# BenLangmead/bowtie2

Hardware: NVIDIA H100
Metric: Mreads/s (higher is better)
Workload: dtype u64 popcount (FM rank) + s16x2 DPX (DP)

## Files before the change

### bowtie2_b200/csrc/api.cu

```cuda
#include "bt2g_internal.h"
#include "dp_device.cuh"
#include <cstring>
#include <cstdlib>
#include <new>

template <typename OFF> void launch_rank4(const DevEbwt<OFF> &, const uint64_t *, uint64_t, uint64_t *, cudaStream_t);
template <typename OFF> void launch_maplf_range(const DevEbwt<OFF> &, const uint64_t *, const uint64_t *, const uint64_t *, uint64_t, uint64_t *, uint64_t *, uint8_t *, cudaStream_t);
template <typename OFF> void launch_maplf1(const DevEbwt<OFF> &, const uint64_t *, const uint8_t *, uint64_t, uint64_t *, cudaStream_t);
template <typename OFF> void launch_ftab(const DevEbwt<OFF> &, const uint64_t *, uint64_t, uint64_t *, cudaStream_t);
template <typename OFF> void launch_exact_sweep(const DevIndex<OFF> &, const uint8_t *, const uint64_t *, uint64_t, int, int, uint8_t *, uint64_t *, cudaStream_t, unsigned long long * = nullptr);
template <typename OFF> void launch_seed_search(const DevIndex<OFF> &, const uint8_t *, const uint64_t *, uint64_t, int, int, int, int, const int32_t *, const int32_t *, uint64_t *, int32_t *, cudaStream_t, unsigned long long * = nullptr);
template <typename OFF> void launch_seed_search2(const DevIndex<OFF> &, const uint8_t *, const uint64_t *, uint64_t, int, int, int, int, int, const int32_t *, const int32_t *, uint64_t *, int32_t *, uint64_t *, uint32_t *, unsigned long long *, int, cudaStream_t, unsigned long long *);
template <typename OFF> void launch_exact_sweep2(const DevIndex<OFF> &, const uint64_t *, uint64_t, int, int, uint8_t *, uint64_t *, const uint64_t *, const uint32_t *, unsigned long long *, int, cudaStream_t, unsigned long long *, int = 0);
void launch_pack_reads(const uint8_t *, const uint64_t *, uint64_t, int, uint64_t *, uint32_t *, cudaStream_t);
template <typename OFF> void launch_resolve(const DevIndex<OFF> &, const uint64_t *, const uint32_t *, uint64_t, int, uint64_t *, uint64_t *, uint64_t *, uint64_t *, uint8_t *, cudaStream_t, unsigned long long * = nullptr);
template <typename OFF> void launch_resolve2(const DevIndex<OFF> &, const uint64_t *, const uint32_t *, uint64_t, const uint32_t *, int, uint64_t *, uint64_t *, uint64_t *, uint64_t *, uint8_t *, unsigned long long *, int, cudaStream_t, unsigned long long *);
template <typename OFF> void launch_one_mm(const DevIndex<OFF> &, const uint8_t *, const uint8_t *, const uint64_t *, uint64_t, const int32_t *, const uint8_t *, const bt2g_scoring &, int, bt2g_mm_hit *, int32_t *, cudaStream_t);
template <typename OFF> void launch_get_stretch(const DevIndex<OFF> &, const uint64_t *, const int64_t *, const int32_t *, uint64_t, int, uint8_t *, cudaStream_t);
template <typename OFF> void launch_extend(const DevIndex<OFF> &, const uint8_t *, const uint64_t *, uint64_t, int, int, const int32_t *, const int32_t *, const uint64_t *, uint8_t *, cudaStream_t);

template <typename OFF> void launch_ungapped(const DevIndex<OFF> &, const bt2g_scoring &, const uint8_t *, const uint8_t *, const uint64_t *, const bt2g_ungapped_problem *, uint64_t, bt2g_ungapped_result *, uint8_t *, uint32_t, cudaStream_t);
template <typename OFF> void launch_build_ktab(const DevIndex<OFF> &, int, OFF *, cudaStream_t);
template <typename OFF> void launch_build_dense_sa(const DevIndex<OFF> &, int, OFF *, cudaStream_t);
void launch_frame_mate(const bt2g_pe_policy &, const bt2g_mate_anchor *, uint64_t, bt2g_mate_frame *, cudaStream_t);
// ... 489 lines not shown
	BT2G_CUDA_TRY(ctx, cudaStreamSynchronize(ctx->stream));
	return 0;
}

int bt2g_pe_classify(bt2g_ctx *ctx, const bt2g_pe_policy *pol, const int64_t *pairs, uint64_t n, int32_t *out) {
	if(!ctx) return -1;
	if(!pol || !pairs || !out || pol->pol < 1 || pol->pol > 4) { ctx->err = "bt2g_pe_classify: bad argument"; return -1; }
	if(n == 0) return 0;
	BT2G_CUDA_TRY(ctx, cudaSetDevice(ctx->device));
	DBuf dp, dout;
	BT2G_CUDA_TRY(ctx, dp.alloc(n * 48)); BT2G_CUDA_TRY(ctx, dout.alloc(n * 4));
	BT2G_CUDA_TRY(ctx, cudaMemcpyAsync(dp.p, pairs, n * 48, cudaMemcpyHostToDevice, ctx->stream));
	launch_pe_classify(*pol, dp.as<int64_t>(), n, dout.as<int32_t>(), ctx->stream);
	BT2G_CUDA_TRY(ctx, cudaGetLastError());
	BT2G_CUDA_TRY(ctx, cudaMemcpyAsync(out, dout.p, n * 4, cudaMemcpyDeviceToHost, ctx->stream));
	BT2G_CUDA_TRY(ctx, cudaStreamSynchronize(ctx->stream));
	return 0;
}

int bt2g_extend_exact(bt2g_ctx *ctx, const bt2g_reads *reads, const bt2g_seed_plan *plan, const uint64_t *ranges, uint8_t *out) {
	REQUIRE_LOADED(ctx);
	if(!reads || !plan || !ranges || !out || plan->max_seeds <= 0 || plan->seed_len <= 0) return -1;
	uint64_t n = reads->n_reads;
	if(n == 0) return 0;
	DBuf dseq, dqual, doff, dint, doffs, drng, dout;
	int rc = uploadReads(ctx, reads, dseq, dqual, doff, false);
	if(rc) return rc;
	const uint64_t nr = n * 2ull * plan->max_seeds;
	BT2G_CUDA_TRY(ctx, dint.alloc(n * 4)); BT2G_CUDA_TRY(ctx, doffs.alloc(n * 4));
	BT2G_CUDA_TRY(ctx, drng.alloc(nr * 32)); BT2G_CUDA_TRY(ctx, dout.alloc(nr * 2));
	BT2G_CUDA_TRY(ctx, cudaMemcpyAsync(dint.p, plan->interval, n * 4, cudaMemcpyHostToDevice, ctx->stream));
	BT2G_CUDA_TRY(ctx, cudaMemcpyAsync(doffs.p, plan->offset, n * 4, cudaMemcpyHostToDevice, ctx->stream));
	BT2G_CUDA_TRY(ctx, cudaMemcpyAsync(drng.p, ranges, nr * 32, cudaMemcpyHostToDevice, ctx->stream));
	DISPATCH(ctx, launch_extend<uint32_t>(bt2g_dev_index<uint32_t>(ctx), dseq.as<uint8_t>(), doff.as<uint64_t>(), n, plan->seed_len, plan->max_seeds, dint.as<int32_t>(), doffs.as<int32_t>(), drng.as<uint64_t>(), dout.as<uint8_t>(), ctx->stream),
	              launch_extend<uint64_t>(bt2g_dev_index<uint64_t>(ctx), dseq.as<uint8_t>(), doff.as<uint64_t>(), n, plan->seed_len, plan->max_seeds, dint.as<int32_t>(), doffs.as<int32_t>(), drng.as<uint64_t>(), dout.as<uint8_t>(), ctx->stream));
	BT2G_CUDA_TRY(ctx, cudaGetLastError());
	BT2G_CUDA_TRY(ctx, cudaMemcpyAsync(out, dout.p, nr * 2, cudaMemcpyDeviceToHost, ctx->stream));
	BT2G_CUDA_TRY(ctx, cudaStreamSynchronize(ctx->stream));
	return 0;
}

int bt2g_resolve(bt2g_ctx *ctx, const uint64_t *rows, const uint32_t *hitlen, uint64_t n, int rejectStraddle,
                 uint64_t *joined, uint64_t *tidx, uint64_t *textoff, uint64_t *tlen, uint8_t *flags) {
	REQUIRE_LOADED(ctx);
	if(!rows) return -1;
	if(n == 0) return 0;
	DBuf dr, dh, dj, dti, dto, dtl, dfl;
	BT2G_CUDA_TRY(ctx, dr.alloc(n * 8));
	BT2G_CUDA_TRY(ctx, cudaMemcpyAsync(dr.p, rows, n * 8, cudaMemcpyHostToDevice, ctx->stream));
	if(hitlen) { BT2G_CUDA_TRY(ctx, dh.alloc(n * 4)); BT2G_CUDA_TRY(ctx, cudaMemcpyAsync(dh.p, hitlen, n * 4, cudaMemcpyHostToDevice, ctx->stream)); }
	if(joined) BT2G_CUDA_TRY(ctx, dj.alloc(n * 8));
	if(tidx) BT2G_CUDA_TRY(ctx, dti.alloc(n * 8));
	if(textoff) BT2G_CUDA_TRY(ctx, dto.alloc(n * 8));
	if(tlen) BT2G_CUDA_TRY(ctx, dtl.alloc(n * 8));
	if(flags) BT2G_CUDA_TRY(ctx, dfl.alloc(n));
	DBuf dnext;
	BT2G_CUDA_TRY(ctx, dnext.alloc(8));
	int sms = 148; cudaDeviceGetAttribute(&sms, cudaDevAttrMultiProcessorCount, ctx->device);
	DISPATCH(ctx, launch_resolve2<uint32_t>(bt2g_dev_index<uint32_t>(ctx), dr.as<uint64_t>(), dh.as<uint32_t>(), n, nullptr, rejectStraddle, dj.as<uint64_t>(), dti.as<uint64_t>(), dto.as<uint64_t>(), dtl.as<uint64_t>(), dfl.as<uint8_t>(), dnext.as<unsigned long long>(), sms, ctx->stream, nullptr),
	              launch_resolve2<uint64_t>(bt2g_dev_index<uint64_t>(ctx), dr.as<uint64_t>(), dh.as<uint32_t>(), n, nullptr, rejectStraddle, dj.as<uint64_t>(), dti.as<uint64_t>(), dto.as<uint64_t>(), dtl.as<uint64_t>(), dfl.as<uint8_t>(), dnext.as<unsigned long long>(), sms, ctx->stream, nullptr));
	BT2G_CUDA_TRY(ctx, cudaGetLastError());
	if(joined) BT2G_CUDA_TRY(ctx, cudaMemcpyAsync(joined, dj.p, n * 8, cudaMemcpyDeviceToHost, ctx->stream));
	if(tidx) BT2G_CUDA_TRY(ctx, cudaMemcpyAsync(tidx, dti.p, n * 8, cudaMemcpyDeviceToHost, ctx->stream));
	if(textoff) BT2G_CUDA_TRY(ctx, cudaMemcpyAsync(textoff, dto.p, n * 8, cudaMemcpyDeviceToHost, ctx->stream));
	if(tlen) BT2G_CUDA_TRY(ctx, cudaMemcpyAsync(tlen, dtl.p, n * 8, cudaMemcpyDeviceToHost, ctx->stream));
	if(flags) BT2G_CUDA_TRY(ctx, cudaMemcpyAsync(flags, dfl.p, n, cudaMemcpyDeviceToHost, ctx->stream));
	BT2G_CUDA_TRY(ctx, cudaStreamSynchronize(ctx->stream));
	return 0;
}

int bt2g_get_stretch(bt2g_ctx *ctx, const uint64_t *tidx, const int64_t *off, const int32_t *count, uint64_t n,
                     int32_t stride, uint8_t *out) {
	REQUIRE_LOADED(ctx);
	if(!ctx->info.has_ref) { ctx->err = "packed reference (.3/.4) not loaded"; return -1; }
	if(n == 0) return 0;
	DBuf dt, dof, dc, dout;
	BT2G_CUDA_TRY(ctx, dt.alloc(n * 8)); BT2G_CUDA_TRY(ctx, dof.alloc(n * 8)); BT2G_CUDA_TRY(ctx, dc.alloc(n * 4));
	BT2G_CUDA_TRY(ctx, dout.alloc(n * (uint64_t)stride));
	BT2G_CUDA_TRY(ctx, cudaMemcpyAsync(dt.p, tidx, n * 8, cudaMemcpyHostToDevice, ctx->stream));
	BT2G_CUDA_TRY(ctx, cudaMemcpyAsync(dof.p, off, n * 8, cudaMemcpyHostToDevice, ctx->stream));
	BT2G_CUDA_TRY(ctx, cudaMemcpyAsync(dc.p, count, n * 4, cudaMemcpyHostToDevice, ctx->stream));
	BT2G_CUDA_TRY(ctx, cudaMemsetAsync(dout.p, 4, n * (uint64_t)stride, ctx->stream));
	DISPATCH(ctx, launch_get_stretch<uint32_t>(bt2g_dev_index<uint32_t>(ctx), dt.as<uint64_t>(), dof.as<int64_t>(), dc.as<int32_t>(), n, stride, dout.as<uint8_t>(), ctx->stream),
	              launch_get_stretch<uint64_t>(bt2g_dev_index<uint64_t>(ctx), dt.as<uint64_t>(), dof.as<int64_t>(), dc.as<int32_t>(), n, stride, dout.as<uint8_t>(), ctx->stream));
	BT2G_CUDA_TRY(ctx, cudaGetLastError());
	BT2G_CUDA_TRY(ctx, cudaMemcpyAsync(out, dout.p, n * (uint64_t)stride, cudaMemcpyDeviceToHost, ctx->stream));
	BT2G_CUDA_TRY(ctx, cudaStreamSynchronize(ctx->stream));
	return 0;
}

}

template <typename OFF> int launch_dp_e2e(const DevIndex<OFF> &, const bt2g_scoring &, const DpLaunch &, int, cudaStream_t);
template <typename OFF> int launch_dp_local(const DevIndex<OFF> &, const bt2g_scoring &, const DpLaunch &, int, cudaStream_t);

extern "C" {

void bt2g_scoring_default(bt2g_scoring *sc, int local) {
	memset(sc, 0, sizeof(*sc));
	sc->match_bonus = local ? 2 : 0;
	sc->rdgap_const = 5; sc->rdgap_linear = 3; sc->rfgap_const = 5; sc->rfgap_linear = 3;
	sc->gapbar = 4;
	sc->local = local ? 1 : 0;
	for(int q = 0; q < 64; q++) {
		int ii = q < 40 ? q : 40;
		float frac = (float)ii / 40.0f;
		sc->mmpen[q] = (uint8_t)(2 + (int)(frac * (6 - 2)));
		sc->npen[q] = 1;
	}
	sc->nceil_const = 0.0; sc->nceil_linear = (double)0.15f;
}

int bt2g_set_scoring(bt2g_ctx *ctx, const bt2g_scoring *sc) {
	if(!ctx || !sc) return -1;
	if(sc->gapbar < 1) { ctx->err = "gapbar must be >= 1"; return -1; }
	ctx->scoring = *sc;
	return 0;
}

int bt2g_set_extend_mode(bt2g_ctx *ctx, int through_text) {
	if(!ctx) return -1;
	ctx->extendText = through_text ? 1 : 0;
	return 0;
}

int bt2g_set_dp_mode(bt2g_ctx *ctx, int cap) {
	if(!ctx || cap < 0 || cap > 3) return -1;
	ctx->dpModeCap = cap;
	return 0;
}

int bt2g_dp_extend(bt2g_ctx *ctx, const bt2g_reads *reads, const bt2g_dp_problem *probs, uint64_t n,
                   int32_t maxCands, int32_t maxAlns, int32_t maxOps,
                   bt2g_dp_summary *summ, bt2g_dp_cand *cands, bt2g_dp_aln *alns, uint8_t *ops) {
	REQUIRE_LOADED(ctx);
	if(!ctx->info.has_ref) { ctx->err = "packed reference (.3/.4) not loaded"; return -1; }
	if(!reads || !reads->qual || !probs || !summ || !cands || !alns || !ops) { ctx->err = "null argument"; return -1; }
	if(ctx->scoring.gapbar < 1) bt2g_scoring_default(&ctx->scoring, 0);
	if(n == 0) return 0;
	if(maxCands < 1 || maxAlns < 1 || maxOps < 1) return -1;
	int maxCol = 1, maxLen = 1;
	int64_t minMinsc = 0;
	for(uint64_t i = 0; i < n; i++) {
		if(probs[i].minsc < minMinsc) minMinsc = probs[i].minsc;
		int64_t nc = probs[i].refr - probs[i].refl + 1;
		if(nc > maxCol) maxCol = (int)nc;
		if(probs[i].read_idx >= reads->n_reads) { ctx->err = "read_idx out of range"; return -1; }
		int len = (int)(reads->off[probs[i].read_idx + 1] - reads->off[probs[i].read_idx]);
		if(len > maxLen) maxLen = len;
	}
	if(maxLen > 512) { ctx->err = "reads longer than 512 are not supported by the DP kernel"; return -1; }
	maxCol += 1;
	if(maxCol > 8192) { ctx->err = "DP window wider than 8192 columns"; return -1; }
	DBuf dseq, dqual, doff, dprob, dcodes, dlast, dsumm, dcand, daln, dops, draw;
	int rc = uploadReads(ctx, reads, dseq, dqual, doff, true);
	if(rc) return rc;
	DpLaunch L;
	L.n = n; L.nDev = nullptr; L.maxCol = maxCol;
	{
		int sms = 148; cudaDeviceGetAttribute(&sms, cudaDevAttrMultiProcessorCount, ctx->device);
		uint64_t want = (uint64_t)sms * 24;
		L.numSlots = ((n < want ? n : want) + 3) / 4 * 4;
	} L.maxCands = maxCands; L.maxAlns = maxAlns; L.maxOps = maxOps;
	L.packed = ctx->scoring.local ? 0 : dp_kernel_mode(ctx->scoring, minMinsc, maxLen, ctx->dpModeCap);
	L.codeStride = dp_code_stride(maxCol, maxLen, L.packed);
	BT2G_CUDA_TRY(ctx, dprob.alloc(n * sizeof(bt2g_dp_problem)));
	if(L.packed == 3) {
		L.chunk = dp_chunk_problems(L.codeStride, n);
		BT2G_CUDA_TRY(ctx, dcodes.alloc(L.chunk * L.codeStride));
	} else {
		BT2G_CUDA_TRY(ctx, dcodes.alloc(L.numSlots * L.codeStride * (L.packed ? 2 : 1)));
	}
	BT2G_CUDA_TRY(ctx, dlast.alloc(L.numSlots * (uint64_t)maxCol * 4));
	L.maxRaw = maxCands * 4 < 1024 ? 1024 : maxCands * 4;
	BT2G_CUDA_TRY(ctx, draw.alloc(L.numSlots * (uint64_t)L.maxRaw * 8));
	L.rawKeys = draw.as<uint64_t>();
	BT2G_CUDA_TRY(ctx, dsumm.alloc(n * sizeof(bt2g_dp_summary)));
	BT2G_CUDA_TRY(ctx, dcand.alloc(n * (uint64_t)maxCands * sizeof(bt2g_dp_cand)));
	BT2G_CUDA_TRY(ctx, daln.alloc(n * (uint64_t)maxAlns * sizeof(bt2g_dp_aln)));
	BT2G_CUDA_TRY(ctx, dops.alloc(n * (uint64_t)maxAlns * maxOps));
	BT2G_CUDA_TRY(ctx, cudaMemcpyAsync(dprob.p, probs, n * sizeof(bt2g_dp_problem), cudaMemcpyHostToDevice, ctx->stream));
	BT2G_CUDA_TRY(ctx, cudaMemsetAsync(dcand.p, 0, dcand.bytes, ctx->stream));
	BT2G_CUDA_TRY(ctx, cudaMemsetAsync(daln.p, 0, daln.bytes, ctx->stream));
	L.seq = dseq.as<uint8_t>(); L.qual = dqual.as<uint8_t>(); L.roff = doff.as<uint64_t>();
	L.probs = dprob.as<bt2g_dp_problem>(); L.codes = dcodes.as<uint8_t>(); L.lastH = dlast.as<int32_t>();
	L.summ = dsumm.as<bt2g_dp_summary>(); L.cands = dcand.as<bt2g_dp_cand>(); L.alns = daln.as<bt2g_dp_aln>(); L.ops = dops.as<uint8_t>();
	int lrc;
	if(ctx->scoring.local) {
		if(ctx->info.off_size == 4) lrc = launch_dp_local<uint32_t>(bt2g_dev_index<uint32_t>(ctx), ctx->scoring, L, maxLen, ctx->stream);
		else lrc = launch_dp_local<uint64_t>(bt2g_dev_index<uint64_t>(ctx), ctx->scoring, L, maxLen, ctx->stream);
	} else {
		if(ctx->info.off_size == 4) lrc = launch_dp_e2e<uint32_t>(bt2g_dev_index<uint32_t>(ctx), ctx->scoring, L, maxLen, ctx->stream);
		else lrc = launch_dp_e2e<uint64_t>(bt2g_dev_index<uint64_t>(ctx), ctx->scoring, L, maxLen, ctx->stream);
	}
	if(lrc) { ctx->err = "DP launch rejected"; return -1; }
	BT2G_CUDA_TRY(ctx, cudaGetLastError());
	BT2G_CUDA_TRY(ctx, cudaMemcpyAsync(summ, dsumm.p, dsumm.bytes, cudaMemcpyDeviceToHost, ctx->stream));
	BT2G_CUDA_TRY(ctx, cudaMemcpyAsync(cands, dcand.p, dcand.bytes, cudaMemcpyDeviceToHost, ctx->stream));
	BT2G_CUDA_TRY(ctx, cudaMemcpyAsync(alns, daln.p, daln.bytes, cudaMemcpyDeviceToHost, ctx->stream));
	BT2G_CUDA_TRY(ctx, cudaMemcpyAsync(ops, dops.p, dops.bytes, cudaMemcpyDeviceToHost, ctx->stream));
	BT2G_CUDA_TRY(ctx, cudaStreamSynchronize(ctx->stream));
	return 0;
}

}
```

### bowtie2_b200/csrc/dp_device.cuh

```cuda
#pragma once
#include "bt2g_internal.h"
#include <cstdlib>

static inline bool dp_packed_ok(const bt2g_scoring &sc, int64_t minMinsc, int maxLen) {
	return !sc.local && minMinsc >= -8000 && (int64_t)sc.match_bonus * maxLen <= 8000 && sc.match_bonus >= 0;
}

static inline int dp_kernel_mode(const bt2g_scoring &sc, int64_t minMinsc, int maxLen, int cap = 3) {
	if(cap < 0 || cap > 3) cap = 3;
	if(cap == 0 || !dp_packed_ok(sc, minMinsc, maxLen)) return 0;
	const int64_t range = (int64_t)sc.match_bonus * maxLen - (minMinsc - sc.match_bonus - 1);
	return (cap >= 2 && range <= 127) ? (cap >= 3 ? 3 : 2) : 1;
}

static inline int dp_rows_per_lane(int maxLen, int mode) {
	if(mode >= 2) {
		const int rs[7] = {4, 5, 6, 8, 10, 12, 16};
		for(int i = 0; i < 7; i++) if(32 * rs[i] >= maxLen) return rs[i];
		return 0;
	}
	return maxLen <= 128 ? 4 : (maxLen <= 256 ? 8 : (maxLen <= 512 ? 16 : 0));
}
#define DP_BLOCK_RPL 2
static inline uint64_t dp_code_stride(int maxCol, int maxLen, int mode) {
	int R = dp_rows_per_lane(maxLen, mode);
	if(mode == 3) R = (R + DP_BLOCK_RPL - 1) / DP_BLOCK_RPL * DP_BLOCK_RPL;
	const uint64_t steps = (uint64_t)maxCol + (mode == 3 ? 36 : 32);
	return ((steps * 32 * (uint64_t)R) + 255) & ~(uint64_t)255;
}

static inline uint64_t dp_chunk_problems(uint64_t codeStride, uint64_t nMax, uint64_t budget = 6ull << 30) {
	if(const char *e = getenv("BT2G_DP_CHUNK_MB")) { uint64_t v = strtoull(e, nullptr, 10); if(v) budget = v << 20; }
	uint64_t c = budget / (codeStride ? codeStride : 1);
	if(c < 1024) c = 1024;
	if(c > nMax) c = nMax;
	return c ? c : 1;
}

struct DpLaunch {
	const uint8_t  *seq, *qual;
	const uint64_t *roff;
	const bt2g_dp_problem *probs;
	uint64_t        n;
	const uint32_t *nDev;
	uint64_t        numSlots;
	uint8_t        *codes;
	int32_t        *lastH;
	uint64_t       *rawKeys;
	int             maxRaw;
	uint64_t        codeStride;
	int             maxCol;
	int             maxCands, maxAlns, maxOps;
	uint64_t        chunk = 0;
	int             packed = 0;
	cudaEvent_t    *tev = nullptr;
	int             tevCap = 0;
	int            *tevN = nullptr;
	uint32_t        zeroP = 0;
	bt2g_dp_summary *summ;
	bt2g_dp_cand    *cands;
	bt2g_dp_aln     *alns;
	uint8_t         *ops;
};
```

### bowtie2_b200/csrc/dp_kernels.cu

```cuda
#include "fm_device.cuh"
#include "dp_device.cuh"

#define DP_NEG (-(1 << 28))
#define DP_BIG (1 << 20)

__host__ __device__ __forceinline__ size_t dp_smem_per_warp(int maxCol) { return ((size_t)maxCol * 7 + 16 + 15) & ~(size_t)15; }

__device__ __forceinline__ int dp_max(int a, int b) { return a > b ? a : b; }

template <int R>
__device__ __forceinline__ void dp_backtrace_all(const DpLaunch &L, const bt2g_scoring &sc, const bt2g_dp_problem &p, uint64_t w,
                                                 const uint8_t *rs, const uint8_t *rq, int rdlen, const uint8_t *refw,
                                                 uint8_t *codes, bt2g_dp_cand *cands, int ncand, bt2g_dp_summary *summ,
                                                 int lane, bool local) {
	const int rdgapo = sc.rdgap_const + sc.rdgap_linear, rdgape = sc.rdgap_linear;
	const int rfgapo = sc.rfgap_const + sc.rfgap_linear, rfgape = sc.rfgap_linear;
	int SQ = rdlen >> 4; if(SQ == 0) SQ = 1;
	bt2g_dp_aln *alns = L.alns + w * (uint64_t)L.maxAlns;
	uint8_t *ops = L.ops + w * (uint64_t)L.maxAlns * L.maxOps;
	int naln = 0, flags = 0;
	auto cell = [&](int rr, int cc) -> uint8_t * { int k = rr / R; return codes + ((size_t)(cc + k) * 32 + k) * R + (rr - k * R); };
	for(int ci = 0; ci < ncand; ci++) {
		int row = cands[ci].row, col = cands[ci].col;
		const int startRow = row;
// ... 475 lines not shown
	const int rdgapo = sc.rdgap_const + sc.rdgap_linear, rdgape = sc.rdgap_linear;
	const int rfgapo = sc.rfgap_const + sc.rfgap_linear, rfgape = sc.rfgap_linear;
	const int bonus = sc.match_bonus;
	const uint32_t FLOORP = dpx_both(DPX_FLOOR), ONEP = 0x00010001u;
	const uint32_t bonusP = dpx_both(bonus), nrdeP = dpx_both(-rdgape);

	for(uint64_t pw = slot; pw < nPairs; pw += nSlots) {
		uint64_t w[2] = {2 * pw, 2 * pw + 1};
		bool live[2] = {true, w[1] < nProb};
		if(!live[1]) w[1] = w[0];
		bt2g_dp_problem p[2] = {L.probs[w[0]], L.probs[w[1]]};
		const uint8_t *rs[2], *rq[2]; int rdlen[2], ncol[2], floorv[2];
		__syncwarp();
#pragma unroll
		for(int x = 0; x < 2; x++) {
			rs[x] = L.seq + L.roff[p[x].read_idx]; rq[x] = L.qual + L.roff[p[x].read_idx];
			rdlen[x] = (int)(L.roff[p[x].read_idx + 1] - L.roff[p[x].read_idx]);
			ncol[x] = (int)(p[x].refr - p[x].refl + 1);
			floorv[x] = p[x].minsc - bonus - 1;
			if(ncol[x] <= 0 || ncol[x] > L.maxCol || rdlen[x] > 32 * R || rdlen[x] <= 0 ||
			   (int64_t)bonus * rdlen[x] - floorv[x] > 127 || floorv[x] < -DPX_LIMIT) {
				if(live[x] && lane == 0) {
					bt2g_dp_summary *sm = L.summ + w[x];
					sm->found = 0; sm->best = DP_NEG; sm->ncand = 0; sm->naln = 0; sm->flags = BT2G_DP_FLAG_BADSHAPE;
				}
				live[x] = false;
			}
		}
		if(!live[0] && !live[1]) continue;
		if(!live[0]) { p[0] = p[1]; rs[0] = rs[1]; rq[0] = rq[1]; rdlen[0] = rdlen[1]; ncol[0] = ncol[1]; floorv[0] = floorv[1]; w[0] = w[1]; }
		if(!live[1]) { p[1] = p[0]; rs[1] = rs[0]; rq[1] = rq[0]; rdlen[1] = rdlen[0]; ncol[1] = ncol[0]; floorv[1] = floorv[0]; w[1] = w[0]; }
		const int ncolMax = ncol[0] > ncol[1] ? ncol[0] : ncol[1];
#pragma unroll
		for(int x = 0; x < 2; x++) {
			ref_window<OFF>(ix, p[x].tidx, p[x].refl, ncol[x], refw[x], lane);
			for(int k = ncol[x] + lane; k < ncolMax; k += 32) refw[x][k] = 4;
		}
		__syncwarp();

		uint32_t rcP[R], mmpP[R], npnP[R], nrfoP[R], nrfeP[R], nrdoP[R];
#pragma unroll
		for(int r = 0; r < R; r++) {
			int v[2][6];
#pragma unroll
			for(int x = 0; x < 2; x++) {
				const int i = lane * R + r;
				bool bar = true;
				int c = 5, mm = 0, np = 0;
				if(i < rdlen[x]) {
					const int pos = p[x].fw ? i : rdlen[x] - 1 - i;
					c = rs[x][pos];
					c = p[x].fw ? c : (c > 3 ? 4 : 3 - c);
					int q = (int)rq[x][pos] - 33;
					q = q < 0 ? 0 : (q > 63 ? 63 : q);
					np = -(int)sc.npen[q];
					mm = c > 3 ? np : -(int)sc.mmpen[q];
					if(c > 3) c = 5;
					bar = (i < sc.gapbar) || (rdlen[x] - 1 - i < sc.gapbar);
				}
				v[x][0] = c; v[x][1] = mm; v[x][2] = np;
				v[x][3] = bar ? -DPX_BIG : -rfgapo; v[x][4] = bar ? -DPX_BIG : -rfgape; v[x][5] = bar ? -DPX_BIG : -rdgapo;
			}
			rcP[r] = dpx_pack(v[0][0], v[1][0]); mmpP[r] = dpx_pack(v[0][1], v[1][1]); npnP[r] = dpx_pack(v[0][2], v[1][2]);
			nrfoP[r] = dpx_pack(v[0][3], v[1][3]); nrfeP[r] = dpx_pack(v[0][4], v[1][4]); nrdoP[r] = dpx_pack(v[0][5], v[1][5]);
		}
		const int lastLane0 = (rdlen[0] - 1) / R, lastLane1 = (rdlen[1] - 1) / R;
		const int lastLaneMax = lastLane0 > lastLane1 ? lastLane0 : lastLane1;
		const uint32_t nfloorP = dpx_pack(-floorv[0], -floorv[1]);

		uint32_t Hleft[R], Earr[R];
#pragma unroll
		for(int r = 0; r < R; r++) { Hleft[r] = FLOORP; Earr[r] = FLOORP; }
		uint32_t botH = FLOORP, botF = FLOORP, prevInH = FLOORP;
		const int nsteps = ncolMax + lastLaneMax;
		const size_t P4 = (size_t)(L.maxCol + 32) * 128, P1 = (size_t)(L.maxCol + 32) * 32;
		uint8_t *w4A[R / 4 + 1], *w4B[R / 4 + 1], *w1A[R % 4 + 1], *w1B[R % 4 + 1];
#pragma unroll
		for(int g = 0; g < R / 4; g++) { w4A[g] = hb[0] + g * P4 + (size_t)lane * 4; w4B[g] = hb[1] + g * P4 + (size_t)lane * 4; }
#pragma unroll
		for(int g = 0; g < R % 4; g++) { w1A[g] = hb[0] + (R / 4) * P4 + g * P1 + lane; w1B[g] = hb[1] + (R / 4) * P4 + g * P1 + lane; }
		for(int t = 0; t < nsteps; t++) {
			uint32_t inH = __shfl_up_sync(0xffffffffu, botH, 1);
			uint32_t inF = __shfl_up_sync(0xffffffffu, botF, 1);
			if(lane == 0) { inH = FLOORP; inF = FLOORP; }
			const int j = t - lane;
			if(j >= 0 && j < ncolMax && lane <= lastLaneMax) {
				const uint32_t refcP = (uint32_t)refw[0][j] | ((uint32_t)refw[1][j] << 16);
				const uint32_t refNm = ((refcP >> 2) & ONEP) * 0xffffu;
				uint32_t diag = (lane == 0) ? 0u : prevInH;
				uint32_t upH = inH, upF = inF;
				uint32_t hs[DP_RP(R)];
#pragma unroll
				for(int r = R; r < DP_RP(R); r++) hs[r] = 0u;
#pragma unroll
				for(int r = 0; r < R; r++) {
					const uint32_t F = __viaddmax_s16x2(upF, nrfeP[r], __viaddmax_s16x2(upH, nrfoP[r], FLOORP));
					const uint32_t pen = dpx_sel(refNm, npnP[r], mmpP[r]);
					const uint32_t mmask = dpx_ne01(rcP[r], refcP) * 0xffffu;
					const uint32_t Hd = __viaddmax_s16x2(diag, dpx_sel(mmask, pen, bonusP), FLOORP);
					const uint32_t E = Earr[r];
					const uint32_t H = __vimax3_s16x2(Hd, E, F);
					Earr[r] = __viaddmax_s16x2(E, nrdeP, __viaddmax_s16x2(H, nrdoP[r], FLOORP));
					hs[r] = __viaddmax_s16x2(H, nfloorP, 0u);
					diag = Hleft[r]; Hleft[r] = H;
					upH = H; upF = F;
				}
				botH = upH; botF = upF;
				prevInH = inH;
#pragma unroll
				for(int q4 = 0; q4 < R / 4; q4++) {
					const uint32_t t01 = __byte_perm(hs[4 * q4], hs[4 * q4 + 1], 0x6240), t23 = __byte_perm(hs[4 * q4 + 2], hs[4 * q4 + 3], 0x6240);
					*reinterpret_cast<uint32_t *>(w4A[q4]) = __byte_perm(t01, t23, 0x5410);
					*reinterpret_cast<uint32_t *>(w4B[q4]) = __byte_perm(t01, t23, 0x7632);
				}
#pragma unroll
				for(int g = 0; g < R % 4; g++) {
					*w1A[g] = (uint8_t)(hs[(R / 4) * 4 + g] & 0xffu);
					*w1B[g] = (uint8_t)((hs[(R / 4) * 4 + g] >> 16) & 0xffu);
				}
			} else if(j >= ncolMax) {
				botH = FLOORP; botF = FLOORP;
			}
#pragma unroll
			for(int g = 0; g < R / 4; g++) { w4A[g] += 128; w4B[g] += 128; }
#pragma unroll
			for(int g = 0; g < R % 4; g++) { w1A[g] += 32; w1B[g] += 32; }
		}
		__syncwarp();
#pragma unroll
		for(int x = 0; x < 2; x++) {
			if(!live[x]) continue;
			const int lr = rdlen[x] - 1, kk = lr / R;
			for(int j = lane; j < ncol[x]; j += 32)
				lastH[x][j] = (int)hb[x][hb_index<R>(L.maxCol + 32, lr, j)] + floorv[x];
			dp_e2e_tail<R, true>(L, sc, p[x], w[x], rs[x], rq[x], rdlen[x], ncol[x], lastH[x], candCol[x], refw[x], hb[x], L.summ + w[x], lane,
			                     DpHbPlanes<R>{hb[x], L.maxCol + 32});
		}
	}
}

#define DP_BLK_ROWS (32 * DP_BLOCK_RPL)
#define DP_BLK_HEAD 64
#define DP_BLK_MAX (DP_BLK_HEAD / 4)
static_assert(16 * 32 <= DP_BLK_MAX * DP_BLK_ROWS, "the range table must cover reads of 32 x 16 rows");

#define DP_FILL_PAD 64
__host__ __device__ __forceinline__ size_t dp_fill_smem_per_warp(int maxCol, bool offdom) {
	const size_t win = ((size_t)maxCol + 15) & ~(size_t)15;
	return 2 * (win + 2 * DP_FILL_PAD) + DP_QPROF_BYTES(DP_BLOCK_RPL) + win * (offdom ? 4 : 8);
}

template <bool B> struct DpBool { static constexpr bool value = B; };

template <typename OFF, int R, bool OFFDOM>
__global__ void __launch_bounds__(128, 8) k_dp_fill_h(DevIndex<OFF> ix, bt2g_scoring sc, DpLaunch L, uint64_t chunkStart, uint64_t chunkMax) {
	constexpr int RPL = DP_BLOCK_RPL;
	static_assert(RPL == 1 || RPL == 2, "stores are one byte or one u16 per lane and problem");
	extern __shared__ uint8_t smem[];
	const int warpInBlock = threadIdx.x >> 5, lane = threadIdx.x & 31;
	const uint64_t slot = blockIdx.x * (uint64_t)(blockDim.x >> 5) + warpInBlock;
	const uint64_t nSlots = (uint64_t)gridDim.x * (blockDim.x >> 5);
	const uint64_t nAll = L.nDev ? (uint64_t)*L.nDev : L.n;
	if(chunkStart >= nAll) return;
	const uint64_t nProb = (nAll - chunkStart < chunkMax) ? nAll - chunkStart : chunkMax;
	const uint64_t nPairs = (nProb + 1) >> 1;
	const size_t win = ((size_t)L.maxCol + 15) & ~(size_t)15;
	uint8_t *sm0 = smem + (size_t)warpInBlock * dp_fill_smem_per_warp(L.maxCol, OFFDOM);
	uint8_t *refw[2] = {sm0 + DP_FILL_PAD, sm0 + win + 3 * DP_FILL_PAD}; uint8_t *hb[2];
	for(int k = lane; k < 2 * ((int)win + 2 * DP_FILL_PAD); k += 32) sm0[k] = 4;
	uint32_t *qprof = reinterpret_cast<uint32_t *>(sm0 + 2 * (win + 2 * DP_FILL_PAD));
	uint32_t *bnd = reinterpret_cast<uint32_t *>(sm0 + 2 * (win + 2 * DP_FILL_PAD) + DP_QPROF_BYTES(RPL));
	const int rdgapo = sc.rdgap_const + sc.rdgap_linear, rdgape = sc.rdgap_linear;
	const int rfgapo = sc.rfgap_const + sc.rfgap_linear, rfgape = sc.rfgap_linear;
	const int bonus = sc.match_bonus;
	const uint32_t FLOORP = OFFDOM ? L.zeroP : dpx_both(DPX_FLOOR);
	const uint32_t nrdeP = dpx_both(-rdgape);

	for(uint64_t pw = slot; pw < nPairs; pw += nSlots) {
		uint64_t w[2] = {2 * pw, 2 * pw + 1};
		bool live[2] = {true, w[1] < nProb};
		if(!live[1]) w[1] = w[0];
		bt2g_dp_problem p[2] = {L.probs[chunkStart + w[0]], L.probs[chunkStart + w[1]]};
		hb[0] = L.codes + w[0] * L.codeStride; hb[1] = L.codes + w[1] * L.codeStride;
		uint64_t ro[2]; int rdlen[2], ncol[2], floorv[2];
		__syncwarp();
#pragma unroll
		for(int x = 0; x < 2; x++) {
			ro[x] = L.roff[p[x].read_idx];
			rdlen[x] = (int)(L.roff[p[x].read_idx + 1] - L.roff[p[x].read_idx]);
			ncol[x] = (int)(p[x].refr - p[x].refl + 1);
			floorv[x] = p[x].minsc - bonus - 1;
			if(ncol[x] <= 0 || ncol[x] > L.maxCol || rdlen[x] > 32 * R || rdlen[x] <= 0 ||
			   (int64_t)bonus * rdlen[x] - floorv[x] > 127 || floorv[x] < -DPX_LIMIT) {
				if(live[x] && lane == 0) {
					bt2g_dp_summary *sm = L.summ + chunkStart + w[x];
					sm->found = 0; sm->best = DP_NEG; sm->ncand = 0; sm->naln = 0; sm->flags = BT2G_DP_FLAG_BADSHAPE;
				}
				live[x] = false;
			}
		}
		if(!live[0] && !live[1]) continue;
		if(!live[0]) { p[0] = p[1]; ro[0] = ro[1]; rdlen[0] = rdlen[1]; ncol[0] = ncol[1]; floorv[0] = floorv[1]; }
		if(!live[1]) { p[1] = p[0]; ro[1] = ro[0]; rdlen[1] = rdlen[0]; ncol[1] = ncol[0]; floorv[1] = floorv[0]; }
		const int ncolMax = ncol[0] > ncol[1] ? ncol[0] : ncol[1];
#pragma unroll
		for(int x = 0; x < 2; x++) {
			ref_window<OFF>(ix, p[x].tidx, p[x].refl, ncol[x], refw[x], lane);
			for(int k = ncol[x] + lane; k < ncolMax; k += 32) refw[x][k] = 4;
		}
		__syncwarp();
		const int rdMax = rdlen[0] > rdlen[1] ? rdlen[0] : rdlen[1];
		const int nblk = (rdMax + DP_BLK_ROWS - 1) / DP_BLK_ROWS;
		const uint32_t nfloorP = dpx_pack(-floorv[0], -floorv[1]);
		uint32_t off = DP_BLK_HEAD;
		int plo = 0, phi = -1;

		for(int b = 0; b < nblk; b++) {
			int lo = 0, bLast = -1, nst = 0;
			if(OFFDOM && b > 0) {
				int first = -1;
				for(int c0 = plo; c0 <= phi; c0 += 32) {
					const int c = c0 + lane;
					const uint32_t m = __ballot_sync(0xffffffffu, c <= phi && bnd[c] != 0u);
					if(m) { if(first < 0) first = c0 + __ffs(m) - 1; bLast = c0 + 31 - __clz(m); }
				}
				lo = first < 0 ? 0 : first;
			}
			if(!OFFDOM || b == 0 || bLast >= 0) {
				uint32_t nrfoP[RPL], nrfeP[RPL], nrdoP[RPL];
#pragma unroll
				for(int r = 0; r < RPL; r++) {
					int v[2][3];
#pragma unroll
					for(int x = 0; x < 2; x++) {
						const int i = b * DP_BLK_ROWS + lane * RPL + r;
						bool bar = true;
						int c = 5, mm = -DPX_BIG, np = -DPX_BIG;
						if(i < rdlen[x]) {
							const int pos = p[x].fw ? i : rdlen[x] - 1 - i;
							c = L.seq[ro[x] + pos];
							c = p[x].fw ? c : (c > 3 ? 4 : 3 - c);
							int q = (int)L.qual[ro[x] + pos] - 33;
							q = q < 0 ? 0 : (q > 63 ? 63 : q);
							np = -(int)sc.npen[q];
							mm = c > 3 ? np : -(int)sc.mmpen[q];
							if(c > 3) c = 5;
							bar = (i < sc.gapbar) || (rdlen[x] - 1 - i < sc.gapbar);
						}
#pragma unroll
						for(int rf = 0; rf < 5; rf++) {
							const uint32_t pv = (uint32_t)(uint16_t)(int16_t)(rf > 3 ? np : (c == rf ? bonus : mm));
							uint32_t &q = qprof[(rf * RPL + r) * 32 + lane];
							q = x == 0 ? pv : (q | (pv << 16));
						}
						v[x][0] = bar ? -DPX_BIG : -rfgapo; v[x][1] = bar ? -DPX_BIG : -rfgape; v[x][2] = bar ? -DPX_BIG : -rdgapo;
					}
					nrfoP[r] = dpx_pack(v[0][0], v[1][0]); nrfeP[r] = dpx_pack(v[0][1], v[1][1]); nrdoP[r] = dpx_pack(v[0][2], v[1][2]);
				}
				int lastLane = (rdMax - 1 - b * DP_BLK_ROWS) / RPL;
				if(lastLane > 31) lastLane = 31;
				const bool keepBottom = b + 1 < nblk;

				const int nsteps = ncolMax - lo + lastLane;
				const int lim = lane <= lastLane ? ncolMax - lo : 0;
				auto sweep = [&](auto top) -> int {
					constexpr bool TOP = decltype(top)::value;
					constexpr int SG = 4;
					uint32_t Hleft[RPL], Earr[RPL];
#pragma unroll
					for(int r = 0; r < RPL; r++) { Hleft[r] = FLOORP; Earr[r] = FLOORP; }
					uint32_t botH = FLOORP, botF = FLOORP, prevInH = FLOORP;
					uint8_t *dA = hb[0] + off + lane * RPL, *dB = hb[1] + off + lane * RPL;
					for(int t0 = 0; t0 < nsteps; t0 += SG, dA += SG * 32 * RPL, dB += SG * 32 * RPL) {
#pragma unroll
						for(int u = 0; u < SG; u++) {
							const int t = t0 + u;
							uint32_t inH = __shfl_up_sync(0xffffffffu, botH, 1);
							uint32_t inF = __shfl_up_sync(0xffffffffu, botF, 1);
							if(TOP) {
								if(lane == 0) { inH = FLOORP; inF = FLOORP; }
							} else {
								uint32_t bh = FLOORP, bf = FLOORP;
								if(lo + t <= phi) {
									if(OFFDOM) { const uint32_t e = bnd[lo + t]; bh = __byte_perm(e, 0u, 0x4140); bf = __byte_perm(e, 0u, 0x4342); }
									else { const uint2 e = reinterpret_cast<const uint2 *>(bnd)[lo + t]; bh = e.x; bf = e.y; }
								}
								if(lane == 0) { inH = bh; inF = bf; }
							}
							const bool on = (unsigned)(t - lane) < (unsigned)lim;
							if(OFFDOM || on) {
								const int j = lo + t - lane;
								const uint32_t *qa = qprof + (int)refw[0][j] * (RPL * 32) + lane, *qb = qprof + (int)refw[1][j] * (RPL * 32) + lane;
								uint32_t diag = (TOP && lane == 0) ? (OFFDOM ? nfloorP : 0u) : prevInH;
								uint32_t upH = inH, upF = inF;
								uint32_t hs[RPL];
#pragma unroll
								for(int r = 0; r < RPL; r++) {
									const uint32_t F = __viaddmax_s16x2(upF, nrfeP[r], __viaddmax_s16x2(upH, nrfoP[r], FLOORP));
									const uint32_t sP = (qa[r * 32] & 0x0000ffffu) | (qb[r * 32] & 0xffff0000u);
									const uint32_t Hd = __viaddmax_s16x2(diag, sP, FLOORP);
									const uint32_t E = Earr[r];
									const uint32_t H = __vimax3_s16x2(Hd, E, F);
									Earr[r] = __viaddmax_s16x2(E, nrdeP, __viaddmax_s16x2(H, nrdoP[r], FLOORP));
									hs[r] = OFFDOM ? H : __viaddmax_s16x2(H, nfloorP, 0u);
									diag = Hleft[r]; Hleft[r] = H;
									upH = H; upF = F;
								}
								botH = upH; botF = upF;
								prevInH = inH;
								if(OFFDOM || on) {
									if(RPL == 2) {
										const uint32_t w2 = __byte_perm(hs[0], hs[RPL - 1], 0x6240);
										*reinterpret_cast<uint16_t *>(dA + u * 32 * RPL) = (uint16_t)w2;
										*reinterpret_cast<uint16_t *>(dB + u * 32 * RPL) = (uint16_t)(w2 >> 16);
									} else {
										dA[u * 32 * RPL] = (uint8_t)hs[0]; dB[u * 32 * RPL] = (uint8_t)(hs[0] >> 16);
									}
									if(keepBottom && lane == 31 && on) {
										if(OFFDOM) bnd[j] = __byte_perm(botH, botF, 0x6420);
										else reinterpret_cast<uint2 *>(bnd)[j] = make_uint2(botH, botF);
									}
								}
							} else {
								botH = FLOORP; botF = FLOORP;
							}
						}
						if(!TOP && OFFDOM && lo + t0 + SG - 1 >= bLast) {
							uint32_t s = botH | botF | prevInH;
#pragma unroll
							for(int r = 0; r < RPL; r++) s |= Hleft[r] | Earr[r];
							if(!__any_sync(0xffffffffu, t0 + SG - 1 - lane < lim && s != 0u)) return t0 + SG < nsteps ? t0 + SG : nsteps;
						}
					}
					return nsteps;
				};
				nst = b == 0 ? sweep(DpBool<true>()) : sweep(DpBool<false>());
			}
			if(lane == 0) {
				reinterpret_cast<uint32_t *>(hb[0])[b] = (uint32_t)lo | ((uint32_t)nst << 16);
				reinterpret_cast<uint32_t *>(hb[1])[b] = (uint32_t)lo | ((uint32_t)nst << 16);
			}
			off += (uint32_t)nst * 32 * RPL;
			plo = lo; phi = lo + nst - 32;
			if(phi > ncolMax - 1) phi = ncolMax - 1;
			__syncwarp();
		}
	}
}

struct DpHbBlocks {
	uint8_t *hb; const uint2 *tab;
	__device__ __forceinline__ uint8_t *operator()(int rr, int cc) const {
		const int k = (rr % DP_BLK_ROWS) / DP_BLOCK_RPL;
		const uint2 e = tab[rr / DP_BLK_ROWS];
		const int st = cc - (int)(e.x & 0xffffu) + k;
		return (st >= k && st < (int)(e.x >> 16)) ? hb + e.y + ((size_t)st * 32 + k) * DP_BLOCK_RPL + rr % DP_BLOCK_RPL : nullptr;
	}
};

#define DP_TAIL_SMEM_PER_WARP(maxCol, R) (dp_smem_per_warp(maxCol) + DP_PROF_BYTES(R) + DP_BLK_MAX * sizeof(uint2))

template <typename OFF, int R>
__global__ void __launch_bounds__(256) k_dp_tail_h(DevIndex<OFF> ix, bt2g_scoring sc, DpLaunch L, uint64_t chunkStart, uint64_t chunkMax) {
	extern __shared__ uint8_t smem[];
	const int warpInBlock = threadIdx.x >> 5, lane = threadIdx.x & 31;
	const uint64_t nAll = L.nDev ? (uint64_t)*L.nDev : L.n;
	if(chunkStart >= nAll) return;
	const uint64_t nProb = (nAll - chunkStart < chunkMax) ? nAll - chunkStart : chunkMax;
	const size_t perWarp = DP_TAIL_SMEM_PER_WARP(L.maxCol, R);
	int32_t *lastH = reinterpret_cast<int32_t *>(smem + (size_t)warpInBlock * perWarp);
	uint16_t *candCol = reinterpret_cast<uint16_t *>(lastH + L.maxCol);
	uint8_t *refw = reinterpret_cast<uint8_t *>(candCol + L.maxCol);
	uint8_t *prof = smem + (size_t)warpInBlock * perWarp + dp_smem_per_warp(L.maxCol);
	uint2 *tab = reinterpret_cast<uint2 *>(prof + DP_PROF_BYTES(R));
	const int bonus = sc.match_bonus;
	const uint64_t nWarps = (uint64_t)gridDim.x * (blockDim.x >> 5);
	for(uint64_t wl = blockIdx.x * (uint64_t)(blockDim.x >> 5) + warpInBlock; wl < nProb; wl += nWarps) {
		const uint64_t w = chunkStart + wl;
		const bt2g_dp_problem p = L.probs[w];
		const uint8_t *rs = L.seq + L.roff[p.read_idx], *rq = L.qual + L.roff[p.read_idx];
		const int rdlen = (int)(L.roff[p.read_idx + 1] - L.roff[p.read_idx]);
		const int ncol = (int)(p.refr - p.refl + 1);
		const int floorv = p.minsc - bonus - 1;
		__syncwarp();
		if(ncol <= 0 || ncol > L.maxCol || rdlen > 32 * R || rdlen <= 0 || (int64_t)bonus * rdlen - floorv > 127 || floorv < -DPX_LIMIT) continue;
		uint8_t *hb = L.codes + wl * L.codeStride;
		const int nblk = (rdlen + DP_BLK_ROWS - 1) / DP_BLK_ROWS;
		const uint32_t e = lane < nblk ? reinterpret_cast<const uint32_t *>(hb)[lane] : 0u;
		const uint32_t bytes = (e >> 16) * (32 * DP_BLOCK_RPL);
		uint32_t incl = bytes;
#pragma unroll
		for(int o = 1; o < 32; o <<= 1) { const uint32_t v = __shfl_up_sync(0xffffffffu, incl, o); if(lane >= o) incl += v; }
		if(lane < nblk) tab[lane] = make_uint2(e, DP_BLK_HEAD + incl - bytes);
		ref_window<OFF>(ix, p.tidx, p.refl, ncol, refw, lane);
		for(int i = lane; i < rdlen; i += 32) {
			const int pos = p.fw ? i : rdlen - 1 - i;
			int c = rs[pos]; c = p.fw ? c : (c > 3 ? 4 : 3 - c);
			int q = (int)rq[pos] - 33; q = q < 0 ? 0 : (q > 63 ? 63 : q);
			prof[i] = (uint8_t)c; prof[rdlen + i] = sc.mmpen[q]; prof[2 * rdlen + i] = sc.npen[q];
		}
		__syncwarp();
		const DpHbBlocks cell{hb, tab};
		const int lr = rdlen - 1;
		for(int j = lane; j < ncol; j += 32) { const uint8_t *c = cell(lr, j); lastH[j] = (c ? (int)*c : 0) + floorv; }
		dp_e2e_tail<R, true>(L, sc, p, w, rs, rq, rdlen, ncol, lastH, candCol, refw, hb, L.summ + w, lane, cell, prof);
	}
}

template <typename Acc>
__device__ __forceinline__ void dp_backtrace_h(const DpLaunch &L, const bt2g_scoring &sc, const bt2g_dp_problem &p, uint64_t w,
                                               const uint8_t *rs, const uint8_t *rq, int rdlen, const uint8_t *refw,
                                               const Acc &cell, bt2g_dp_cand *cands, int ncand, bt2g_dp_summary *summ, int lane,
                                               const uint8_t *prof) {
	const int rdgapo = sc.rdgap_const + sc.rdgap_linear, rdgape = sc.rdgap_linear;
	const int rfgapo = sc.rfgap_const + sc.rfgap_linear, rfgape = sc.rfgap_linear;
	const int bonus = sc.match_bonus, gapbar = sc.gapbar;
	const int vmax = bonus * rdlen - (p.minsc - bonus - 1);
	bt2g_dp_aln *alns = L.alns + w * (uint64_t)L.maxAlns;
	uint8_t *ops = L.ops + w * (uint64_t)L.maxAlns * L.maxOps;
	int naln = 0, flags = 0;
	bool screened = false;
	auto cellv = [&](int rr, int cc) -> int { const uint8_t *c = cell(rr, cc); return c ? (int)*c : 0; };
	auto rdchar = [&](int rr) -> int { const int pos = p.fw ? rr : rdlen - 1 - rr; int c = rs[pos]; return p.fw ? c : (c > 3 ? 4 : 3 - c); };
	auto rdqual = [&](int rr) -> int { const int pos = p.fw ? rr : rdlen - 1 - rr; int q = (int)rq[pos] - 33; return q < 0 ? 0 : (q > 63 ? 63 : q); };
	auto inCore = [&](int dlo, int dhi) -> bool { return dhi >= p.corel && dlo <= p.corer; };
	for(int ci = 0; ci < ncand; ci++) {
		int row = cands[ci].row, col = cands[ci].col;
		const int startRow = row, origCol = col;
		uint8_t *o = ops + (size_t)naln * L.maxOps;
		const bool room = naln < L.maxAlns;
		int nops = 0, ns = 0, gaps = 0;
		bool fail = false, core = false, done = false, first = true, filtStart = false;
		while(!done && !fail) {
			const int wd = (ci > 0 && first) ? 8 : 32;
			const int rk = row - lane, ck = col - lane;
			const bool in = lane < wd && rk >= 0 && ck >= 0;
			uint8_t *cp = in ? cell(rk, ck) : nullptr;
			const int mine = in ? (cp ? (int)*cp : 0) : 0x80;
			const int v = mine & 0x7f;
			const int vn = __shfl_down_sync(0xffffffffu, v, 1);
			int sck = 0, refc = 4; bool isN = false, isMatch = false;
			if(in) {
				refc = refw[ck];
				if(prof) {
					const int c = prof[rk];
					isN = c > 3 || refc > 3;
					isMatch = !isN && c == refc;
					sck = isN ? -(int)prof[2 * rdlen + rk] : (isMatch ? bonus : -(int)prof[rdlen + rk]);
				} else {
					const int c = rdchar(rk), q = rdqual(rk);
					isN = c > 3 || refc > 3;
					isMatch = !isN && c == refc;
					sck = isN ? -(int)sc.npen[q] : (isMatch ? bonus : -(int)sc.mmpen[q]);
				}
			}
			const bool cont = lane < wd - 1 && !(mine & 0x80) && rk > 0 && ck > 0 && vn > 0 && v == vn + sck;
			const int run = __ffs(~__ballot_sync(0xffffffffu, cont)) - 1;
			if(run > 0) {
				first = false;
				const int diagi = col - row + p.triml;
				if(inCore(diagi, diagi)) core = true;
				if(lane < run) {
					const uint8_t op = (uint8_t)((isMatch ? BT2G_OP_MATCH : BT2G_OP_MM) | (refc << 2));
					if(room && nops + lane < L.maxOps) o[nops + lane] = op;
					if(cp) *cp = (uint8_t)(mine | 0x80);
				}
				ns += __popc(__ballot_sync(0xffffffffu, lane < run && isN));
				nops += run; row -= run; col -= run;
			}
			const int endBits = __shfl_sync(0xffffffffu, mine, run);
			if(run == wd - 1 && !(endBits & 0x80) && row > 0 && col > 0) { __syncwarp(); continue; }
			if(endBits & 0x80) {
				if(first) filtStart = true;
				fail = true; break;
			}
			first = false;
			if(lane == run && cp) *cp = (uint8_t)(mine | 0x80);
			{
				const int diagi = col - row + p.triml;
				if(inCore(diagi, diagi)) core = true;
			}
			if(row == 0) { done = true; break; }
			const int cur = endBits & 0x7f;
			__syncwarp();
			int klen = 0, gapKind = 0;
			if(row >= gapbar && rdlen - 1 - row >= gapbar) {
				for(int k0 = 0; k0 < row; k0 += 32) {
					if(vmax - rfgapo - k0 * rfgape < cur) break;
					const int k = k0 + lane + 1, r2 = row - k;
					bool ok = false;
					if(r2 >= 0 && row - k + 1 >= gapbar && vmax - rfgapo - (k - 1) * rfgape >= cur) {
						const int u = cellv(r2, col) & 0x7f;
						ok = u > 0 && u - rfgapo - (k - 1) * rfgape == cur;
					}
					const uint32_t mk = __ballot_sync(0xffffffffu, ok);
					if(mk) { klen = k0 + __ffs(mk); gapKind = 1; break; }
				}
				if(gapKind == 0) {
					for(int k0 = 0; k0 < col; k0 += 32) {
						if(vmax - rdgapo - k0 * rdgape < cur) break;
						const int k = k0 + lane + 1, c2 = col - k;
						bool ok = false;
						if(c2 >= 0 && vmax - rdgapo - (k - 1) * rdgape >= cur) {
							const int u = cellv(row, c2) & 0x7f;
							ok = u > 0 && u - rdgapo - (k - 1) * rdgape == cur;
						}
						const uint32_t mk = __ballot_sync(0xffffffffu, ok);
						if(mk) { klen = k0 + __ffs(mk); gapKind = 2; break; }
					}
				}
			}
			if(gapKind == 0) { fail = true; break; }
			for(int m0 = 1; m0 < klen && !fail; m0 += 32) {
				const int mth = m0 + lane;
				uint8_t *q2 = nullptr; int b = 0;
				if(mth < klen) { q2 = gapKind == 1 ? cell(row - mth, col) : cell(row, col - mth); b = q2 ? *q2 : 0; }
				const uint32_t vm = __ballot_sync(0xffffffffu, (b & 0x80) != 0);
				const int lim = vm ? __ffs(vm) - 1 : 32;
				if(q2 && lane < lim) *q2 = (uint8_t)(b | 0x80);
				if(vm) fail = true;
			}
			if(fail) break;
			{
				const int d0 = col - row + p.triml, ni = klen - 1;
				if(ni > 0 && (gapKind == 1 ? inCore(d0 + 1, d0 + ni) : inCore(d0 - ni, d0 - 1))) core = true;
			}
			if(room) {
				for(int k = lane; k < klen; k += 32) {
					const int idx = nops + k;
					if(idx < L.maxOps) o[idx] = gapKind == 1 ? (uint8_t)BT2G_OP_REFGAP : (uint8_t)(BT2G_OP_READGAP | (refw[col - k] << 2));
				}
			}
			nops += klen; gaps += klen;
			if(gapKind == 1) row -= klen; else col -= klen;
			__syncwarp();
		}
		if(filtStart) { if(lane == 0) cands[ci].fate = BT2G_CAND_FILT_START; continue; }
		if(!fail) {
			const int c = rdchar(row), refc = refw[col];
			const bool isN = c > 3 || refc > 3;
			ns += isN;
			const uint8_t op = (uint8_t)(((!isN && c == refc) ? BT2G_OP_MATCH : BT2G_OP_MM) | (refc << 2));
			if(!core) fail = true;
			else if(ns > p.nceil) fail = true;
			else {
				if(room && lane == 0 && nops < L.maxOps) o[nops] = op;
				nops++;
			}
		}
		const bool opOverflow = nops > L.maxOps;
		if(fail) { if(lane == 0) cands[ci].fate = BT2G_CAND_FAILED; continue; }
		if(lane == 0) cands[ci].fate = BT2G_CAND_SUCCEEDED;
		if(room) {
			int refns = 0;
			for(int k = col + lane; k <= origCol; k += 32) refns += refw[k] > 3;
			refns = __reduce_add_sync(0xffffffffu, refns);
			if(lane == 0) {
				bt2g_dp_aln &a = alns[naln];
				a.cand_idx = ci; a.score = cands[ci].score; a.ns = ns; a.gaps = gaps; a.col0 = col; a.row0 = row;
				a.trim_beg = 0; a.trim_end = rdlen - 1 - startRow; a.nops = nops;
				a.refns = refns;
			}
			if(opOverflow) flags |= BT2G_DP_FLAG_OPS_OVERFLOW;
		} else {
			flags |= BT2G_DP_FLAG_ALN_OVERFLOW;
		}
		naln++;
		if(naln == 1 && !screened && ci + 1 < ncand) {
			screened = true;
			bool needSeq = false;
			for(int base = ci + 1; base < ncand; base += 32) {
				const int cj = base + lane;
				int verdict = 0;
				if(cj < ncand) {
					int r2 = cands[cj].row, c2 = cands[cj].col;
					int b = cellv(r2, c2);
					if(b & 0x80) verdict = 1;
					else {
						for(int guard = 0; guard < 4 * rdlen + 8; guard++) {
							const int curv = b & 0x7f;
							if(r2 == 0) { verdict = 2; break; }
							if(c2 > 0) {
								const int pb = cellv(r2 - 1, c2 - 1), pv = pb & 0x7f;
								const int rf = refw[c2];
								int c, mm, np;
								if(prof) { c = prof[r2]; mm = prof[rdlen + r2]; np = prof[2 * rdlen + r2]; }
								else { c = rdchar(r2); const int q = rdqual(r2); mm = sc.mmpen[q]; np = sc.npen[q]; }
								const int sc2 = (c > 3 || rf > 3) ? -np : (c == rf ? bonus : -mm);
								if(pv > 0 && curv == pv + sc2) {
									if(pb & 0x80) break;
									r2--; c2--; b = pb;
									continue;
								}
							}
							if(r2 < gapbar || rdlen - 1 - r2 < gapbar) break;
							bool moved = false, dead = false, marked = false;
							for(int k = 1; k <= r2 && r2 - k + 1 >= gapbar && vmax - rfgapo - (k - 1) * rfgape >= curv; k++) {
								const int ub = cellv(r2 - k, c2), u = ub & 0x7f;
								if(u > 0 && u - rfgapo - (k - 1) * rfgape == curv) {
									if(marked || (ub & 0x80)) dead = true; else { r2 -= k; b = ub; moved = true; }
									break;
								}
								marked = marked || (ub & 0x80);
							}
							if(!moved && !dead) {
								marked = false;
								for(int k = 1; k <= c2 && vmax - rdgapo - (k - 1) * rdgape >= curv; k++) {
									const int ub = cellv(r2, c2 - k), u = ub & 0x7f;
									if(u > 0 && u - rdgapo - (k - 1) * rdgape == curv) {
										if(marked || (ub & 0x80)) dead = true; else { c2 -= k; b = ub; moved = true; }
										break;
									}
									marked = marked || (ub & 0x80);
								}
							}
							if(!moved) break;
						}
					}
				}
				if(__any_sync(0xffffffffu, verdict == 2)) { needSeq = true; break; }
				if(cj < ncand) cands[cj].fate = verdict == 1 ? BT2G_CAND_FILT_START : BT2G_CAND_FAILED;
			}
			__syncwarp();
			if(!needSeq) break;
		}
	}
	if(lane == 0) { summ->naln = naln; summ->flags |= flags; }
}

template <typename K>
static unsigned dp_resident_grid(K kernel, int threads, size_t smem, uint64_t numSlots, int warpsPerBlock) {
	int dev = 0, sms = 148, nb = 1;
	cudaGetDevice(&dev);
	cudaDeviceGetAttribute(&sms, cudaDevAttrMultiProcessorCount, dev);
	if(cudaOccupancyMaxActiveBlocksPerMultiprocessor(&nb, kernel, threads, smem) != cudaSuccess || nb < 1) nb = 1;
	uint64_t g = (uint64_t)nb * sms, cap = numSlots / warpsPerBlock;
	return (unsigned)(g < cap ? g : cap);
}

template <typename OFF, int R>
static void launch_dp_e2e_r(const DevIndex<OFF> &ix, const bt2g_scoring &sc, const DpLaunch &L, cudaStream_t st) {
	const int warpsPerBlock = 4;
	if(L.packed == 3) {
		int dev = 0, sms = 148; cudaGetDevice(&dev); cudaDeviceGetAttribute(&sms, cudaDevAttrMultiProcessorCount, dev);
		const size_t smF = (size_t)warpsPerBlock * dp_fill_smem_per_warp(L.maxCol, sc.match_bonus == 0);
		const size_t smT = (size_t)8 * DP_TAIL_SMEM_PER_WARP(L.maxCol, R);
		auto kfill = sc.match_bonus == 0 ? k_dp_fill_h<OFF, R, true> : k_dp_fill_h<OFF, R, false>;
		if(smF > 48 * 1024) cudaFuncSetAttribute(kfill, cudaFuncAttributeMaxDynamicSharedMemorySize, (int)smF);
		if(smT > 48 * 1024) cudaFuncSetAttribute(k_dp_tail_h<OFF, R>, cudaFuncAttributeMaxDynamicSharedMemorySize, (int)smT);
		int nbF = 1, nbT = 1;
		if(cudaOccupancyMaxActiveBlocksPerMultiprocessor(&nbF, kfill, warpsPerBlock * 32, smF) != cudaSuccess || nbF < 1) nbF = 1;
		if(cudaOccupancyMaxActiveBlocksPerMultiprocessor(&nbT, k_dp_tail_h<OFF, R>, 256, smT) != cudaSuccess || nbT < 1) nbT = 1;
		auto mark = [&]() { if(L.tev && L.tevN && *L.tevN < L.tevCap) cudaEventRecord(L.tev[(*L.tevN)++], st); };
		mark();
		for(uint64_t c0 = 0; c0 < L.n; c0 += L.chunk) {
			kfill<<<(unsigned)(nbF * sms), warpsPerBlock * 32, smF, st>>>(ix, sc, L, c0, L.chunk);
			mark();
			k_dp_tail_h<OFF, R><<<(unsigned)(nbT * sms), 256, smT, st>>>(ix, sc, L, c0, L.chunk);
			mark();
		}
	} else if(L.packed == 2) {
		const size_t smem = (size_t)warpsPerBlock * 2 * dp_smem_per_warp(L.maxCol);
		if(smem > 48 * 1024) cudaFuncSetAttribute(k_dp_e2e_h<OFF, R>, cudaFuncAttributeMaxDynamicSharedMemorySize, (int)smem);
		const unsigned grid = dp_resident_grid(k_dp_e2e_h<OFF, R>, warpsPerBlock * 32, smem, L.numSlots, warpsPerBlock);
		k_dp_e2e_h<OFF, R><<<grid, warpsPerBlock * 32, smem, st>>>(ix, sc, L);
	} else if(L.packed) {
		const size_t smem = (size_t)warpsPerBlock * 2 * dp_smem_per_warp(L.maxCol);
		if(smem > 48 * 1024) cudaFuncSetAttribute(k_dp_e2e_x2<OFF, R>, cudaFuncAttributeMaxDynamicSharedMemorySize, (int)smem);
		const unsigned grid = dp_resident_grid(k_dp_e2e_x2<OFF, R>, warpsPerBlock * 32, smem, L.numSlots, warpsPerBlock);
		k_dp_e2e_x2<OFF, R><<<grid, warpsPerBlock * 32, smem, st>>>(ix, sc, L);
	} else {
		const size_t smem = (size_t)warpsPerBlock * dp_smem_per_warp(L.maxCol);
		if(smem > 48 * 1024) cudaFuncSetAttribute(k_dp_e2e<OFF, R>, cudaFuncAttributeMaxDynamicSharedMemorySize, (int)smem);
		const unsigned grid = dp_resident_grid(k_dp_e2e<OFF, R>, warpsPerBlock * 32, smem, L.numSlots, warpsPerBlock);
		k_dp_e2e<OFF, R><<<grid, warpsPerBlock * 32, smem, st>>>(ix, sc, L);
	}
}

template <typename OFF>
int launch_dp_e2e(const DevIndex<OFF> &ix, const bt2g_scoring &sc, const DpLaunch &L, int maxRdLen, cudaStream_t st) {
	if(L.n == 0) return 0;
	switch(dp_rows_per_lane(maxRdLen, L.packed)) {
		case 4: launch_dp_e2e_r<OFF, 4>(ix, sc, L, st); break;
		case 5: launch_dp_e2e_r<OFF, 5>(ix, sc, L, st); break;
		case 6: launch_dp_e2e_r<OFF, 6>(ix, sc, L, st); break;
		case 8: launch_dp_e2e_r<OFF, 8>(ix, sc, L, st); break;
		case 10: launch_dp_e2e_r<OFF, 10>(ix, sc, L, st); break;
		case 12: launch_dp_e2e_r<OFF, 12>(ix, sc, L, st); break;
		case 16: launch_dp_e2e_r<OFF, 16>(ix, sc, L, st); break;
		default: return -1;
	}
	return 0;
}
template int launch_dp_e2e<uint32_t>(const DevIndex<uint32_t> &, const bt2g_scoring &, const DpLaunch &, int, cudaStream_t);
template int launch_dp_e2e<uint64_t>(const DevIndex<uint64_t> &, const bt2g_scoring &, const DpLaunch &, int, cudaStream_t);

template <typename OFF, int R>
__global__ void __launch_bounds__(128) k_dp_local(DevIndex<OFF> ix, bt2g_scoring sc, DpLaunch L) {
	extern __shared__ uint8_t smem[];
	const int warpInBlock = threadIdx.x >> 5, lane = threadIdx.x & 31;
	const uint64_t slot = blockIdx.x * (uint64_t)(blockDim.x >> 5) + warpInBlock;
	const uint64_t nSlots = (uint64_t)gridDim.x * (blockDim.x >> 5);
	const uint64_t nProb = L.nDev ? (uint64_t)*L.nDev : L.n;
	const size_t perWarp = dp_smem_per_warp(L.maxCol);
	int32_t *wsm = reinterpret_cast<int32_t *>(smem + (size_t)warpInBlock * perWarp);
	uint8_t *refw = reinterpret_cast<uint8_t *>(wsm + L.maxCol) + 2 * (size_t)L.maxCol;
	uint8_t *codes = L.codes + slot * L.codeStride;
	uint64_t *raw = L.rawKeys + slot * (uint64_t)L.maxRaw;
	const int rdgapo = sc.rdgap_const + sc.rdgap_linear, rdgape = sc.rdgap_linear;
	const int rfgapo = sc.rfgap_const + sc.rfgap_linear, rfgape = sc.rfgap_linear;
	const int bonus = sc.match_bonus;

	for(uint64_t w = slot; w < nProb; w += nSlots) {
		const bt2g_dp_problem p = L.probs[w];
		const uint8_t *rs = L.seq + L.roff[p.read_idx];
		const uint8_t *rq = L.qual + L.roff[p.read_idx];
		const int rdlen = (int)(L.roff[p.read_idx + 1] - L.roff[p.read_idx]);
		const int ncol = (int)(p.refr - p.refl + 1);
		bt2g_dp_summary *summ = L.summ + w;
		__syncwarp();
		if(ncol <= 0 || ncol + 1 > L.maxCol || rdlen > 32 * R || rdlen <= 0 || bonus <= 0) {
			if(lane == 0) { summ->found = 0; summ->best = DP_NEG; summ->ncand = 0; summ->naln = 0; summ->flags = BT2G_DP_FLAG_BADSHAPE; }
			continue;
		}
		for(int k = lane; k <= ncol; k += 32) refw[k] = (uint8_t)ref_base<OFF>(ix, p.tidx, p.refl + k);
		if(lane == 0) wsm[0] = 0;
		__syncwarp();

		int rc[R + 1], mmp[R], npn[R];
		bool bar[R];
#pragma unroll
		for(int r = 0; r <= R; r++) {
			int i = lane * R + r;
			int c = 6;
			if(i < rdlen) {
				int pos = p.fw ? i : rdlen - 1 - i;
				c = rs[pos];
				c = p.fw ? c : (c > 3 ? 4 : 3 - c);
				if(r < R) {
					int q = (int)rq[pos] - 33;
					q = q < 0 ? 0 : (q > 63 ? 63 : q);
					npn[r] = sc.npen[q];
					mmp[r] = c > 3 ? npn[r] : sc.mmpen[q];
					bar[r] = (i < sc.gapbar) || (rdlen - 1 - i < sc.gapbar);
				}
			} else if(r < R) { mmp[r] = 0; npn[r] = 0; bar[r] = true; }
			rc[r] = c;
		}
		const int lastLane = (rdlen - 1) / R;
		const int minrow = (int)(((int64_t)p.minsc + bonus - 1) / bonus) - 1;

		int Hleft[R], Earr[R], Eprev[R];
#pragma unroll
		for(int r = 0; r < R; r++) { Hleft[r] = 0; Earr[r] = 0; Eprev[r] = 0; }
		int botH = 0, botF = 0, prevInH = 0, lmax = 0;
		const int nsteps = ncol + lastLane;
		for(int t = 0; t < nsteps; t++) {
			int inH = __shfl_up_sync(0xffffffffu, botH, 1);
			int inF = __shfl_up_sync(0xffffffffu, botF, 1);
			if(lane == 0) { inH = 0; inF = 0; }
			const int j = t - lane;
			if(j >= 0 && j < ncol && lane <= lastLane) {
				const int refc = refw[j], refn = refw[j + 1];
				const bool refN = refc > 3;
				int diag = (lane == 0) ? 0 : prevInH;
				int upH = inH, upF = inF;
				uint32_t packed[(R + 3) / 4];
#pragma unroll
				for(int q4 = 0; q4 < (R + 3) / 4; q4++) packed[q4] = 0;
#pragma unroll
				for(int r = 0; r < R; r++) {
					const int i = lane * R + r;
					const int fo = upH - rfgapo, fe = upF - rfgape;
					int F = bar[r] ? 0 : dp_max(dp_max(fo, fe), 0);
					const int fsel = (upH > 0 && fo == F) ? 1 : ((upF > 0 && fe == F) ? 2 : 0);
					int s = (rc[r] == refc && !refN) ? bonus : -mmp[r];
					s = (refN || rc[r] > 3) ? -npn[r] : s;
					const int Hd = diag + s;
					const int E = Earr[r];
					const int H = dp_max(__vimax3_s32(Hd, E, F), 0);
					int hsel = 0;
					if(diag > 0 && H == Hd) hsel = 1;
					else if(!bar[r]) {
						if(upH > 0 && H == fo) hsel = 2;
						else if(upF > 0 && H == fe) hsel = 3;
						else if(Hleft[r] > 0 && H == Hleft[r] - rdgapo) hsel = 4;
						else if(Eprev[r] > 0 && H == Eprev[r] - rdgape) hsel = 5;
					}
					const int esel = (Hleft[r] > 0 && Hleft[r] - rdgapo == E) ? 1 : ((Eprev[r] > 0 && Eprev[r] - rdgape == E) ? 2 : 0);
					const uint32_t code = (uint32_t)(hsel | (esel << 3) | (fsel << 5));
					packed[r >> 2] |= code << ((r & 3) * 8);
					const int eo = bar[r] ? 0 : H - rdgapo, ee = E - rdgape;
					if(i < rdlen && i >= minrow && H >= p.minsc && rc[r] == refc && !(i < rdlen - 1 && rc[r + 1] == refn)) {
						const int pos = atomicAdd(&wsm[0], 1);
						if(pos < L.maxRaw) raw[pos] = ((uint64_t)(uint32_t)H << 32) | ((uint64_t)i << 16) | (uint64_t)j;
					}
					lmax = dp_max(lmax, i < rdlen ? H : 0);
					diag = Hleft[r]; Hleft[r] = H; Eprev[r] = E; Earr[r] = dp_max(dp_max(eo, ee), 0);
					upH = H; upF = F;
				}
				botH = upH; botF = upF;
				prevInH = inH;
				uint8_t *dst = codes + ((size_t)t * 32 + lane) * R;
				if(R == 4) *reinterpret_cast<uint32_t *>(dst) = packed[0];
				else if(R == 8) *reinterpret_cast<uint2 *>(dst) = make_uint2(packed[0], packed[1]);
				else {
#pragma unroll
					for(int q4 = 0; q4 < (R + 3) / 4; q4++) reinterpret_cast<uint32_t *>(dst)[q4] = packed[q4];
				}
			} else if(j >= ncol) {
				botH = 0; botF = 0;
			}
		}
		__syncwarp();
		int best = lmax;
#pragma unroll
		for(int o = 16; o > 0; o >>= 1) best = dp_max(best, __shfl_xor_sync(0xffffffffu, best, o));
		if(lane == 0) { summ->best = best; summ->flags = 0; summ->naln = 0; summ->ncand = 0; summ->found = 0; }
		if(best < p.minsc) continue;
		const int nrawAll = wsm[0];
		const int nraw = nrawAll < L.maxRaw ? nrawAll : L.maxRaw;
		bt2g_dp_cand *cands = L.cands + w * (uint64_t)L.maxCands;
		for(int a0 = 0; a0 < nraw; a0 += 32) {
			const int a = a0 + lane;
			if(a < nraw) {
				const uint64_t key = raw[a];
				int rank = 0;
				for(int k = 0; k < nraw; k++) rank += raw[k] > key;
				if(rank < L.maxCands) {
					cands[rank].score = (int32_t)(key >> 32); cands[rank].row = (int32_t)((key >> 16) & 0xffff);
					cands[rank].col = (int32_t)(key & 0xffff); cands[rank].fate = 0;
				}
			}
		}
		const int ncand = nraw < L.maxCands ? nraw : L.maxCands;
		if(lane == 0) {
			summ->ncand = nrawAll; summ->found = nrawAll > 0;
			if(nrawAll > L.maxCands || nrawAll > L.maxRaw) summ->flags |= BT2G_DP_FLAG_CAND_OVERFLOW;
		}
		__syncwarp();
		dp_backtrace_all<R>(L, sc, p, w, rs, rq, rdlen, refw, codes, cands, ncand, summ, lane, true);
	}
}

template <typename OFF>
// ... 23 lines not shown
```

### bowtie2_b200/csrc/pipeline.cu

```cuda
#include "fm_device.cuh"
#include "dp_device.cuh"
#include "pe_device.cuh"
#include "mapq_device.cuh"
#include <new>
#include <cstring>

template <typename OFF> void launch_exact_sweep(const DevIndex<OFF> &, const uint8_t *, const uint64_t *, uint64_t, int, int, uint8_t *, uint64_t *, cudaStream_t, unsigned long long *);
template <typename OFF> void launch_seed_search(const DevIndex<OFF> &, const uint8_t *, const uint64_t *, uint64_t, int, int, int, int, const int32_t *, const int32_t *, uint64_t *, int32_t *, cudaStream_t, unsigned long long *);
template <typename OFF> void launch_seed_search2(const DevIndex<OFF> &, const uint8_t *, const uint64_t *, uint64_t, int, int, int, int, int, const int32_t *, const int32_t *, uint64_t *, int32_t *, uint64_t *, uint32_t *, unsigned long long *, int, cudaStream_t, unsigned long long *);
template <typename OFF> void launch_exact_sweep2(const DevIndex<OFF> &, const uint64_t *, uint64_t, int, int, uint8_t *, uint64_t *, const uint64_t *, const uint32_t *, unsigned long long *, int, cudaStream_t, unsigned long long *, int = 0);
void launch_pack_reads(const uint8_t *, const uint64_t *, uint64_t, int, uint64_t *, uint32_t *, cudaStream_t);
template <typename OFF> void launch_resolve2(const DevIndex<OFF> &, const uint64_t *, const uint32_t *, uint64_t, const uint32_t *, int, uint64_t *, uint64_t *, uint64_t *, uint64_t *, uint8_t *, unsigned long long *, int, cudaStream_t, unsigned long long *);
template <typename OFF> void launch_resolve(const DevIndex<OFF> &, const uint64_t *, const uint32_t *, uint64_t, int, uint64_t *, uint64_t *, uint64_t *, uint64_t *, uint8_t *, cudaStream_t, unsigned long long *);
template <typename OFF> int launch_dp_e2e(const DevIndex<OFF> &, const bt2g_scoring &, const DpLaunch &, int, cudaStream_t);
template <typename OFF> int launch_dp_local(const DevIndex<OFF> &, const bt2g_scoring &, const DpLaunch &, int, cudaStream_t);

struct PipeBufs {
	uint8_t *seq, *qual; uint64_t *roff;
	int32_t *minscByLen, *nceilByLen, *nceilRawByLen, *ivalByLen, *rdgapsByLen, *rfgapsByLen;
	int32_t *interval, *offset;
	uint8_t *mine; uint64_t *ee;
	uint64_t *ranges; int32_t *nseeds;
	uint64_t *packed; uint32_t *nmask; unsigned long long *nextTask;
	uint64_t *rows; uint32_t *hitlen, *meta;
	uint32_t *nRows, *rowBase, *rowCnt;
	uint64_t *tidx, *textoff, *tlen; uint8_t *rflags;
	bt2g_dp_problem *probs; uint32_t *nProb; int32_t *readProb; int32_t *readNProb;
	uint8_t *codes; int32_t *lastH; uint64_t *rawKeys;
	bt2g_dp_summary *summ; bt2g_dp_cand *cands; bt2g_dp_aln *alns; uint8_t *ops;
	bt2g_read_result *res; uint8_t *resOps;
	unsigned long long *counters;
	uint64_t *probTlen, *resTlen;
	bt2g_dp_problem *mProbs; uint32_t *nMateProb; int32_t *mateOfRead;
	bt2g_dp_summary *mSumm; bt2g_dp_cand *mCands; bt2g_dp_aln *mAlns; uint8_t *mOps;
	bt2g_pair_result *pairs; unsigned long long *mateCells;
};

struct bt2g_pipeline {
	bt2g_ctx *ctx;
	bt2g_pipeline_params prm;
	bt2g_scoring sc;
	uint64_t maxReads, maxBases;
	PipeBufs b;
	std::vector<void *> allocs;
	uint64_t numSlots, codeStride, maxProbs;
	int packed = 0;
	uint64_t dpChunk = 0, mateChunk = 0;
	int maxCol, R, sms = 148;
	cudaEvent_t ev[9], pev[4];
	bool pairsOn = false; bt2g_pe_policy pe{}; int mateMaxCol = 0; uint64_t mateCodeStride = 0;
	bt2g_pair_result *hPairs = nullptr;
	bool evOk = false;
	uint8_t *hSeq = nullptr, *hQual = nullptr; uint64_t *hOff = nullptr;
	bt2g_read_result *hRes = nullptr; uint8_t *hOps = nullptr;
	uint64_t lastN = 0;
	cudaStream_t sIn = nullptr, sOut = nullptr;
	cudaEvent_t evIn[8], evDone[8];
	bool chunkOk = false;
};

#define PIPE_MAX_RAW 8192
#define META_STRAND(m) (((m) >> 31) & 1u)
#define META_EE(m)     (((m) >> 30) & 1u)
#define META_SEED(m)   (((m) >> 16) & 0x3fffu)

__global__ void k_plan(const uint64_t *roff, uint64_t n, const int32_t *ivalByLen, int maxLen, int32_t *interval, int32_t *offset) {
	uint64_t i = blockIdx.x * (uint64_t)blockDim.x + threadIdx.x;
	if(i >= n) return;
	int len = (int)(roff[i + 1] - roff[i]);
	interval[i] = ivalByLen[len > maxLen ? maxLen : len];
	offset[i] = 0;
}

__global__ void k_collect(uint64_t n, const uint64_t *roff, const uint64_t *ee, const uint64_t *ranges, const int32_t *nseeds,
                          int maxSeeds, int seedLen, int rowCap, int rangeMax,
                          uint64_t *rows, uint32_t *hitlen, uint32_t *meta, uint32_t *nRows, uint32_t *rowBase, uint32_t *rowCnt) {
	uint64_t rd = blockIdx.x * (uint64_t)blockDim.x + threadIdx.x;
	if(rd >= n) return;
	const int len = (int)(roff[rd + 1] - roff[rd]);
	const uint64_t *e = ee + rd * 4;
	const int ns = nseeds[rd];
	const int sl = seedLen < len ? seedLen : len;
	const uint64_t *rg = ranges + rd * 2ull * maxSeeds * 4;
	uint64_t eeTot = (e[1] - e[0]) + (e[3] - e[2]);
	int cnt = 0;
	if(eeTot > 0) cnt = eeTot < (uint64_t)rowCap ? (int)eeTot : rowCap;
	else {
		for(int strand = 0; strand < 2; strand++)
			for(int k = 0; k < ns; k++) {
				const uint64_t *q = rg + ((size_t)strand * maxSeeds + k) * 4;
				const uint64_t sz = q[1] - q[0];
				if(sz >= 1 && sz <= (uint64_t)rangeMax) cnt += (int)sz;
			}
		if(cnt > rowCap) cnt = rowCap;
	}
	const uint32_t base = cnt ? atomicAdd(nRows, (uint32_t)cnt) : 0;
	rowBase[rd] = base; rowCnt[rd] = (uint32_t)cnt;
	uint64_t *ro = rows + base;
	uint32_t *ho = hitlen + base, *mo = meta + base;
	int w = 0;
	if(eeTot > 0) {
		for(int strand = 0; strand < 2; strand++)
			for(uint64_t r = e[2 * strand]; r < e[2 * strand + 1] && w < cnt; r++) {
				ro[w] = r; ho[w] = (uint32_t)len; mo[w] = ((uint32_t)strand << 31) | (1u << 30); w++;
			}
	} else {
		for(int sz = 1; sz <= rangeMax && w < cnt; sz++)
			for(int strand = 0; strand < 2 && w < cnt; strand++)
				for(int k = 0; k < ns && w < cnt; k++) {
					const uint64_t *q = rg + ((size_t)strand * maxSeeds + k) * 4;
					if((int)(q[1] - q[0]) != sz) continue;
					for(uint64_t r = q[0]; r < q[1] && w < cnt; r++) {
						ro[w] = r; ho[w] = (uint32_t)sl; mo[w] = ((uint32_t)strand << 31) | ((uint32_t)k << 16); w++;
					}
				}
	}
}

__global__ void k_frame(uint64_t n, const uint64_t *roff, const int32_t *interval, const int32_t *offset,
                        const uint64_t *rows, const uint32_t *hitlen, const uint32_t *meta,
                        const uint64_t *tidx, const uint64_t *textoff, const uint64_t *tlen, const uint8_t *rflags,
                        const uint32_t *rowBase, const uint32_t *rowCnt,
                        int rowCap, int maxLen, int maxhalf, int matchBonus,
                        const int32_t *minscByLen, const int32_t *nceilRawByLen, const int32_t *rdgapsByLen, const int32_t *rfgapsByLen,
                        bt2g_dp_problem *probs, uint32_t *nProb, uint32_t maxProbs, int32_t *readProb, int32_t *readNProb, bt2g_read_result *res,
                        uint64_t *probTlen, uint64_t *resTlen) {
	uint64_t rd = blockIdx.x * (uint64_t)blockDim.x + threadIdx.x;
	if(rd >= n) return;
	const int len = (int)(roff[rd + 1] - roff[rd]);
	const int li = len > maxLen ? maxLen : len;
	bt2g_read_result r;
	r.found = 0; r.score = 0; r.score2 = INT32_MIN; r.fw = 0; r.tidx = 0; r.refoff = 0; r.nops = 0; r.ndp = 0; r.trim_left = 0; r.trim_right = 0; r.mapq = 0; r.pad = 0;
	int np = 0;
	uint64_t seenT[32]; int64_t seenO[32]; uint8_t seenS[32]; int nseen = 0;
	const int minsc = minscByLen[li];
	const uint32_t rb = rowBase[rd], rcnt = rowCnt[rd];
	for(uint32_t i = 0; i < rcnt; i++) {
		uint64_t s = (uint64_t)rb + i;
		uint32_t m = meta[s];
		const bool isEE = META_EE(m) != 0;
		const uint8_t fl = rflags[s];
		if(fl & 2) continue;
		if(isEE && (fl & 1)) continue;
		const int strand = (int)META_STRAND(m);
		int rdoff = 0;
		if(!isEE) {
			int depth = (int)META_SEED(m) * interval[rd] + offset[rd];
			rdoff = strand == 0 ? depth : len - depth - (int)hitlen[s];
		}
		const int64_t refoff = (int64_t)textoff[s] - rdoff;
		bool dup = false;
		for(int k = 0; k < nseen; k++) if(seenT[k] == tidx[s] && seenO[k] == refoff && seenS[k] == strand) { dup = true; break; }
		if(dup) continue;
		if(nseen < 32) { seenT[nseen] = tidx[s]; seenO[nseen] = refoff; seenS[nseen] = (uint8_t)strand; nseen++; }
		if(isEE) {
			if(r.found == 0) { r.found = 2; r.score = len * matchBonus; r.fw = strand == 0; r.tidx = tidx[s]; r.refoff = refoff; resTlen[rd] = tlen[s]; }
			else if(r.score2 == INT32_MIN) r.score2 = len * matchBonus;
			continue;
		}
		int maxgap = rdgapsByLen[li] > rfgapsByLen[li] ? rdgapsByLen[li] : rfgapsByLen[li];
		if(maxgap < 0 || maxgap > maxhalf) maxgap = maxhalf;
		int64_t refl = refoff - 2 * maxgap, refr = refoff + (len - 1) + 2 * maxgap;
		const int64_t reflen = (int64_t)tlen[s];
		int64_t triml = 0, trimr = 0;
		if(refr >= reflen) trimr = refr - (reflen - 1);
		if(refl < 0) triml = -refl;
		if(refr - trimr < refl + triml) continue;
		uint32_t pi = atomicAdd(nProb, 1u);
		if(pi >= maxProbs) { atomicSub(nProb, 1u); r.found |= 0x100; break; }
		bt2g_dp_problem &p = probs[pi];
		p.read_idx = (uint32_t)rd; p.fw = strand == 0; p.tidx = tidx[s];
		p.refl = refl + triml; p.refr = refr - trimr; p.triml = (int32_t)triml;
		p.corel = maxgap; p.corer = 3 * maxgap; p.minsc = minsc; p.nceil = nceilRawByLen[li]; p.reserved = 0;
		readProb[rd * rowCap + np] = (int32_t)pi;
		probTlen[pi] = tlen[s];
		np++;
	}
	readNProb[rd] = np;
	r.ndp = np;
	res[rd] = r;
}
// ... 63 lines not shown
	if((o.found & 0xff) != 0 && o.tidx == a.tidx) {
		const int ea = pe_ref_extent(a, resOps + rd * (size_t)maxOps, alen), eo = pe_ref_extent(o, resOps + od * (size_t)maxOps, olen);
		const int k = anchor1 ? pe_classify(pp, a.refoff, (uint64_t)ea, a.fw != 0, o.refoff, (uint64_t)eo, o.fw != 0)
		                      : pe_classify(pp, o.refoff, (uint64_t)eo, o.fw != 0, a.refoff, (uint64_t)ea, a.fw != 0);
		if(k != 5) return;
	}
	const int li = olen > maxLen ? maxLen : olen;
	bt2g_mate_anchor an;
	an.off = a.refoff; an.reflen = resTlen[rd];
	an.len1 = (uint32_t)(anchor1 ? alen : olen); an.len2 = (uint32_t)(anchor1 ? olen : alen);
	an.maxrdgap = rdgapsByLen[li]; an.maxrfgap = rfgapsByLen[li];
	an.maxalcols = olen + an.maxrdgap;
	an.maxns = nceilRawByLen[li]; an.maxhalf = maxhalf;
	an.is1 = anchor1; an.fw = a.fw != 0; an.pad[0] = an.pad[1] = 0;
	bt2g_mate_frame f;
	pe_frame_anchor(pp, an, f);
	if(f.status != 2) return;
	if(f.refr - f.refl + 1 > mateMaxCol) return;
	const uint32_t pi = atomicAdd(nMateProb, 1u);
	bt2g_dp_problem &q = mProbs[pi];
	q.read_idx = (uint32_t)od; q.fw = f.ofw; q.tidx = a.tidx;
	q.refl = f.refl; q.refr = f.refr; q.triml = (int32_t)f.triml;
	q.corel = (int32_t)f.corel; q.corer = (int32_t)f.corer;
	q.minsc = minscByLen[li]; q.nceil = nceilRawByLen[li]; q.reserved = 0;
	mateOfRead[rd] = (int32_t)pi;
}

__global__ void k_pick_pairs(uint64_t nPairs, const uint64_t *roff, bt2g_read_result *res, uint8_t *resOps, int maxOps, int maxAlns,
                             bt2g_pe_policy pp, const int32_t *mateOfRead, const bt2g_dp_problem *mProbs, const bt2g_dp_summary *mSumm,
                             const bt2g_dp_aln *mAlns, const uint8_t *mOps, bt2g_pair_result *pairs, unsigned long long *mateCells,
                             const int32_t *minscByLen, int maxLen, int matchBonus, int monotone) {
	const uint64_t pr = blockIdx.x * (uint64_t)blockDim.x + threadIdx.x;
	if(pr >= nPairs) return;
	const uint64_t r1 = 2 * pr, r2 = 2 * pr + 1;
	bt2g_read_result a1 = res[r1], a2 = res[r2];
	const int len1 = (int)(roff[r1 + 1] - roff[r1]), len2 = (int)(roff[r2 + 1] - roff[r2]);
	const bool f1 = (a1.found & 0xff) != 0, f2 = (a2.found & 0xff) != 0;
	bt2g_pair_result out;
	out.pair_type = (f1 && f2) ? 2 : ((f1 || f2) ? 3 : 0); out.kind = 5; out.source = 0; out.score_sum = 0; out.fraglen = 0;
	int bestSum = INT32_MIN, bestSrc = -1, bestKind = 5, bestAln = 0;
	int secSum = INT32_MIN;
	auto offer = [&](int sum) { if(sum > bestSum) { secSum = bestSum; bestSum = sum; return true; } if(sum > secSum) secSum = sum; return false; };
	const int e1 = f1 ? pe_ref_extent(a1, resOps + r1 * (size_t)maxOps, len1) : 0;
	const int e2 = f2 ? pe_ref_extent(a2, resOps + r2 * (size_t)maxOps, len2) : 0;
	if(f1 && f2 && a1.tidx == a2.tidx) {
		const int k = pe_classify(pp, a1.refoff, (uint64_t)e1, a1.fw != 0, a2.refoff, (uint64_t)e2, a2.fw != 0);
		if(k != 5) { offer(a1.score + a2.score); bestSrc = 0; bestKind = k; }
	}
	unsigned long long cells = 0;
	for(int src = 1; src <= 2; src++) {
		const uint64_t ra = src == 1 ? r1 : r2;
		const bool fa = src == 1 ? f1 : f2;
		if(!fa) continue;
		const int pi = mateOfRead[ra];
		if(pi < 0) continue;
		const bt2g_dp_problem &q = mProbs[pi];
		cells += (unsigned long long)(src == 1 ? len2 : len1) * (unsigned long long)(q.refr - q.refl + 1);
		const int na = mSumm[pi].naln < maxAlns ? mSumm[pi].naln : maxAlns;
		const bt2g_read_result &an = src == 1 ? a1 : a2;
		const int ea = src == 1 ? e1 : e2;
		for(int k = 0; k < na; k++) {
			const bt2g_dp_aln &al = mAlns[(size_t)pi * maxAlns + k];
			const uint8_t *o = mOps + ((size_t)pi * maxAlns + k) * maxOps;
			int em = 0;
			const int no = al.nops < maxOps ? al.nops : maxOps;
			for(int x = 0; x < no; x++) em += (o[x] & 3) != BT2G_OP_REFGAP;
			const int64_t moff = q.refl + al.col0;
			const int kind = src == 1 ? pe_classify(pp, an.refoff, (uint64_t)ea, an.fw != 0, moff, (uint64_t)em, q.fw != 0)
			                          : pe_classify(pp, moff, (uint64_t)em, q.fw != 0, an.refoff, (uint64_t)ea, an.fw != 0);
			if(kind == 5) continue;
			const int sum = an.score + al.score;
			if(offer(sum)) { bestSrc = src; bestKind = kind; bestAln = k; }
		}
	}
	if(bestSrc > 0) {
		const uint64_t ra = bestSrc == 1 ? r1 : r2, ro = bestSrc == 1 ? r2 : r1;
		const int pi = mateOfRead[ra];
		const bt2g_dp_problem &q = mProbs[pi];
		const bt2g_dp_aln &al = mAlns[(size_t)pi * maxAlns + bestAln];
		bt2g_read_result m = res[ro];
		if((m.found & 0xff) != 0 && m.score > m.score2) m.score2 = m.score;
		m.found = (m.found & ~0xff) | 1; m.score = al.score; m.fw = q.fw; m.tidx = q.tidx; m.refoff = q.refl + al.col0;
		m.nops = al.nops < maxOps ? al.nops : maxOps; m.trim_left = al.trim_beg; m.trim_right = al.trim_end; m.pad = al.refns;
		const uint8_t *src = mOps + ((size_t)pi * maxAlns + bestAln) * maxOps;
		uint8_t *dst = resOps + ro * (size_t)maxOps;
		for(int k = 0; k < m.nops; k++) dst[k] = src[k];
		res[ro] = m;
		if(bestSrc == 1) a2 = m; else a1 = m;
	}
	if(bestSrc >= 0) {
		out.pair_type = 1; out.kind = bestKind; out.source = bestSrc; out.score_sum = bestSum;
		const int ee1 = pe_ref_extent(a1, resOps + r1 * (size_t)maxOps, len1), ee2 = pe_ref_extent(a2, resOps + r2 * (size_t)maxOps, len2);
		const int64_t lo = a1.refoff < a2.refoff ? a1.refoff : a2.refoff;
		const int64_t h1 = a1.refoff + ee1, h2 = a2.refoff + ee2;
		out.fraglen = (h1 > h2 ? h1 : h2) - lo;
		const int l1 = len1 > maxLen ? maxLen : len1, l2 = len2 > maxLen ? maxLen : len2;
		if(f1 && a1.score2 > INT32_MIN / 2 && (long long)a1.score2 + a2.score > secSum) secSum = a1.score2 + a2.score;
		if(f2 && a2.score2 > INT32_MIN / 2 && (long long)a1.score + a2.score2 > secSum) secSum = a1.score + a2.score2;
		if(secSum > bestSum) secSum = bestSum;
		const long long minPair = (long long)minscByLen[l1] + minscByLen[l2];
		const bool hasSec = secSum > INT32_MIN / 2 && secSum >= minPair;
		const int mq = mapq_v2(bestSum, hasSec, hasSec ? secSum : 0, minPair, (long long)(len1 + len2) * matchBonus, monotone != 0);
		res[r1].mapq = mq; res[r2].mapq = mq;
	}
	pairs[pr] = out;
	if(mateCells && cells) atomicAdd(mateCells, cells);
}

template <typename T> static int pipeAlloc(bt2g_pipeline *p, T *&ptr, uint64_t count) {
	void *v = nullptr;
	cudaError_t e = cudaMalloc(&v, (count ? count : 1) * sizeof(T));
	if(e != cudaSuccess) { p->ctx->err = std::string("pipeline cudaMalloc: ") + cudaGetErrorString(e); return -2; }
	p->allocs.push_back(v);
	ptr = (T *)v;
	return 0;
}

template <typename OFF>
static int runStages(bt2g_pipeline *p, const uint8_t *seq, const uint8_t *qual, const uint64_t *roff, uint64_t n, cudaStream_t st, bool count,
                     uint64_t resBase = 0) {
	bt2g_ctx *ctx = p->ctx;
	PipeBufs &b = p->b;
	const bt2g_pipeline_params &q = p->prm;
	DevIndex<OFF> ix = bt2g_dev_index<OFF>(ctx);
	unsigned long long *c = count ? b.counters : nullptr;
	const unsigned T = 128;
	auto grid = [&](uint64_t m) { return (unsigned)((m + T - 1) / T); };
	auto mark = [&](int i) { if(p->evOk) cudaEventRecord(p->ev[i], st); };
	if(count) BT2G_CUDA_TRY(ctx, cudaMemsetAsync(b.counters, 0, 4 * sizeof(unsigned long long), st));
	BT2G_CUDA_TRY(ctx, cudaMemsetAsync(b.nProb, 0, sizeof(uint32_t), st));
	BT2G_CUDA_TRY(ctx, cudaMemsetAsync(b.nRows, 0, sizeof(uint32_t), st));
	mark(0);
	k_plan<<<grid(n), T, 0, st>>>(roff, n, b.ivalByLen, q.max_len, b.interval, b.offset);
	mark(1);
	launch_pack_reads(seq, roff, n, q.max_len, b.packed, b.nmask, st);
	launch_exact_sweep2<OFF>(ix, roff, n, 0, 0, b.mine, b.ee, b.packed, b.nmask, b.nextTask, p->sms, st, c ? c + 0 : nullptr, 1 );
	mark(2);
	launch_seed_search2<OFF>(ix, seq, roff, n, q.max_len, q.seed_len, q.max_seeds, 0, 0, b.interval, b.offset, b.ranges, b.nseeds,
	                         b.packed, b.nmask, b.nextTask, p->sms, st, c ? c + 1 : nullptr);
	mark(3);
	k_collect<<<grid(n), T, 0, st>>>(n, roff, b.ee, b.ranges, b.nseeds, q.max_seeds, q.seed_len, q.row_cap, q.range_max, b.rows, b.hitlen, b.meta,
	                                 b.nRows, b.rowBase, b.rowCnt);
	mark(4);
	launch_resolve2<OFF>(ix, b.rows, b.hitlen, 0, b.nRows, 0, nullptr, b.tidx, b.textoff, b.tlen, b.rflags, b.nextTask, p->sms, st, c ? c + 2 : nullptr);
	mark(5);
	k_frame<<<grid(n), T, 0, st>>>(n, roff, b.interval, b.offset, b.rows, b.hitlen, b.meta, b.tidx, b.textoff, b.tlen, b.rflags,
	                               b.rowBase, b.rowCnt, q.row_cap, q.max_len, q.maxhalf, p->sc.match_bonus,
	                               b.minscByLen, b.nceilRawByLen, b.rdgapsByLen, b.rfgapsByLen,
	                               b.probs, b.nProb, (uint32_t)p->maxProbs, b.readProb, b.readNProb, b.res + resBase, b.probTlen, b.resTlen + resBase);
	DpLaunch L;
	L.seq = seq; L.qual = qual; L.roff = roff; L.probs = b.probs; L.n = p->maxProbs; L.nDev = b.nProb;
	L.rawKeys = b.rawKeys; L.maxRaw = b.rawKeys ? PIPE_MAX_RAW : 0;
	L.numSlots = p->numSlots; L.codes = b.codes; L.lastH = b.lastH; L.codeStride = p->codeStride; L.maxCol = p->maxCol;
	L.maxCands = q.max_cands; L.maxAlns = q.max_alns; L.maxOps = q.max_ops; L.packed = p->packed; L.chunk = p->dpChunk;
	L.summ = b.summ; L.cands = b.cands; L.alns = b.alns; L.ops = b.ops;
	mark(6);
	const int drc = p->sc.local ? launch_dp_local<OFF>(ix, p->sc, L, q.max_len, st) : launch_dp_e2e<OFF>(ix, p->sc, L, q.max_len, st);
	if(drc) { ctx->err = "pipeline: DP launch rejected"; return -1; }
	mark(7);
	k_pick<<<grid(n), T, 0, st>>>(n, q.row_cap, q.max_alns, q.max_ops, b.readProb, b.readNProb, b.probs, b.summ, b.alns, b.ops,
	                              b.res + resBase, b.resOps + resBase * (uint64_t)q.max_ops, c ? c + 3 : nullptr, roff, b.probTlen, b.resTlen + resBase, b.minscByLen, q.max_len, p->sc.match_bonus, p->sc.match_bonus == 0);
	mark(8);
	BT2G_CUDA_TRY(ctx, cudaGetLastError());
	p->lastN = n;
	return 0;
}

template <typename OFF>
static int runPairTail(bt2g_pipeline *p, const uint8_t *seq, const uint8_t *qual, const uint64_t *roff, uint64_t nPairs, cudaStream_t st, bool count,
                       uint64_t resBase = 0) {
	bt2g_ctx *ctx = p->ctx;
	PipeBufs &b = p->b;
	const bt2g_pipeline_params &q = p->prm;
	DevIndex<OFF> ix = bt2g_dev_index<OFF>(ctx);
	const uint64_t n = 2 * nPairs;
	const unsigned T = 128;
	bt2g_read_result *res = b.res + resBase; uint8_t *resOps = b.resOps + resBase * (uint64_t)q.max_ops;
	const uint64_t *resTlen = b.resTlen + resBase; bt2g_pair_result *pairs = b.pairs + resBase / 2;
	BT2G_CUDA_TRY(ctx, cudaMemsetAsync(b.nMateProb, 0, sizeof(uint32_t), st));
	BT2G_CUDA_TRY(ctx, cudaMemsetAsync(b.mateCells, 0, sizeof(unsigned long long), st));
	cudaEventRecord(p->pev[0], st);
	k_frame_mates<<<(unsigned)((n + T - 1) / T), T, 0, st>>>(n, roff, res, resOps, q.max_ops, resTlen, p->pe, q.max_len, q.maxhalf, p->mateMaxCol,
	                                                         b.minscByLen, b.nceilRawByLen, b.rdgapsByLen, b.rfgapsByLen, b.mProbs, b.nMateProb, b.mateOfRead);
	cudaEventRecord(p->pev[1], st);
	DpLaunch L;
	L.seq = seq; L.qual = qual; L.roff = roff; L.probs = b.mProbs; L.n = p->maxReads; L.nDev = b.nMateProb;
	L.rawKeys = nullptr; L.maxRaw = 0;
	L.numSlots = p->numSlots; L.codes = b.codes; L.lastH = nullptr; L.codeStride = p->mateCodeStride; L.maxCol = p->mateMaxCol;
	L.maxCands = q.max_cands; L.maxAlns = q.max_alns; L.maxOps = q.max_ops; L.packed = p->packed; L.chunk = p->mateChunk;
	L.summ = b.mSumm; L.cands = b.mCands; L.alns = b.mAlns; L.ops = b.mOps;
	if(launch_dp_e2e<OFF>(ix, p->sc, L, q.max_len, st)) { ctx->err = "pipeline: mate DP launch rejected"; return -1; }
	cudaEventRecord(p->pev[2], st);
	k_pick_pairs<<<(unsigned)((nPairs + T - 1) / T), T, 0, st>>>(nPairs, roff, res, resOps, q.max_ops, q.max_alns, p->pe, b.mateOfRead, b.mProbs,
	                                                             b.mSumm, b.mAlns, b.mOps, pairs, count ? b.mateCells : nullptr, b.minscByLen, q.max_len, p->sc.match_bonus, p->sc.match_bonus == 0);
	cudaEventRecord(p->pev[3], st);
	BT2G_CUDA_TRY(ctx, cudaGetLastError());
	return 0;
}

extern "C" {

int bt2g_pipeline_create(bt2g_ctx *ctx, const bt2g_pipeline_params *prm, uint64_t maxReads, uint64_t maxBases, bt2g_pipeline **out) {
	if(!ctx || !prm || !out) return -1;
	if(!ctx->loaded) { ctx->err = "no index loaded"; return -1; }
	if(ctx->scoring.gapbar < 1) bt2g_scoring_default(&ctx->scoring, 0);
	if(prm->seed_len > 32) { ctx->err = "pipeline: seed length must be <= 32"; return -1; }
	if(prm->max_len < 1 || prm->max_len > 512 || prm->row_cap < 1 || prm->row_cap > 32 || prm->max_seeds < 1 || prm->max_seeds > 16383) {
		ctx->err = "pipeline: bad parameters"; return -1;
	}
	cudaSetDevice(ctx->device);
	bt2g_pipeline *p = new(std::nothrow) bt2g_pipeline();
	if(!p) return -4;
	p->ctx = ctx; p->prm = *prm; p->sc = ctx->scoring; p->maxReads = maxReads; p->maxBases = maxBases;
	PipeBufs &b = p->b;
	memset(&b, 0, sizeof(b));
	const uint64_t n = maxReads, cap = prm->row_cap, nrowMax = n * cap;
	const uint64_t nprobMax = (prm->max_probs > 0 && (uint64_t)prm->max_probs < nrowMax) ? (uint64_t)prm->max_probs : nrowMax;
	p->maxProbs = nprobMax;
	int rc = 0;
	const int L1 = prm->max_len + 1;
	rc |= pipeAlloc(p, b.seq, maxBases); rc |= pipeAlloc(p, b.qual, maxBases); rc |= pipeAlloc(p, b.roff, n + 1);
	rc |= pipeAlloc(p, b.minscByLen, L1); rc |= pipeAlloc(p, b.nceilByLen, L1); rc |= pipeAlloc(p, b.nceilRawByLen, L1);
	rc |= pipeAlloc(p, b.ivalByLen, L1); rc |= pipeAlloc(p, b.rdgapsByLen, L1); rc |= pipeAlloc(p, b.rfgapsByLen, L1);
	rc |= pipeAlloc(p, b.interval, n); rc |= pipeAlloc(p, b.offset, n);
	rc |= pipeAlloc(p, b.mine, n * 2); rc |= pipeAlloc(p, b.ee, n * 4);
	rc |= pipeAlloc(p, b.ranges, n * 2ull * prm->max_seeds * 4); rc |= pipeAlloc(p, b.nseeds, n);
	rc |= pipeAlloc(p, b.packed, (maxBases >> 5) + n + 2); rc |= pipeAlloc(p, b.nmask, (maxBases >> 5) + n + 2); rc |= pipeAlloc(p, b.nextTask, 1);
	rc |= pipeAlloc(p, b.nRows, 1); rc |= pipeAlloc(p, b.rowBase, n); rc |= pipeAlloc(p, b.rowCnt, n);
	rc |= pipeAlloc(p, b.rows, nrowMax); rc |= pipeAlloc(p, b.hitlen, nrowMax); rc |= pipeAlloc(p, b.meta, nrowMax);
	rc |= pipeAlloc(p, b.tidx, nrowMax); rc |= pipeAlloc(p, b.textoff, nrowMax); rc |= pipeAlloc(p, b.tlen, nrowMax); rc |= pipeAlloc(p, b.rflags, nrowMax);
	rc |= pipeAlloc(p, b.probs, nprobMax); rc |= pipeAlloc(p, b.nProb, 1); rc |= pipeAlloc(p, b.readProb, nrowMax); rc |= pipeAlloc(p, b.readNProb, n);
	p->maxCol = prm->max_len + 4 * prm->maxhalf + 4;
	int sms = 148; cudaDeviceGetAttribute(&sms, cudaDevAttrMultiProcessorCount, ctx->device);
	p->sms = sms;
	p->numSlots = (uint64_t)sms * 24;
	{
		int64_t mn = 0;
		for(int l = 1; l <= prm->max_len; l++) if(prm->minsc_by_len[l] < mn) mn = prm->minsc_by_len[l];
		p->packed = p->sc.local ? 0 : dp_kernel_mode(p->sc, mn, prm->max_len, ctx->dpModeCap);
	}
	p->R = dp_rows_per_lane(prm->max_len, p->packed);
	p->codeStride = dp_code_stride(p->maxCol, prm->max_len, p->packed);
	if(p->packed == 3) {
		p->dpChunk = dp_chunk_problems(p->codeStride, nprobMax);
		rc |= pipeAlloc(p, b.codes, p->dpChunk * p->codeStride);
	} else {
		rc |= pipeAlloc(p, b.codes, p->numSlots * p->codeStride * (p->packed ? 2 : 1));
	} rc |= pipeAlloc(p, b.lastH, p->numSlots * (uint64_t)p->maxCol);
	if(ctx->scoring.local) rc |= pipeAlloc(p, b.rawKeys, p->numSlots * (uint64_t)PIPE_MAX_RAW);
	rc |= pipeAlloc(p, b.summ, nprobMax); rc |= pipeAlloc(p, b.cands, nprobMax * prm->max_cands);
	rc |= pipeAlloc(p, b.alns, nprobMax * prm->max_alns); rc |= pipeAlloc(p, b.ops, nprobMax * prm->max_alns * (uint64_t)prm->max_ops);
	rc |= pipeAlloc(p, b.res, n); rc |= pipeAlloc(p, b.resOps, n * (uint64_t)prm->max_ops);
	rc |= pipeAlloc(p, b.counters, 4);
	rc |= pipeAlloc(p, b.probTlen, nprobMax); rc |= pipeAlloc(p, b.resTlen, n);
	if(rc) { bt2g_pipeline_destroy(p); return -2; }
	cudaError_t e = cudaSuccess;
	auto up = [&](int32_t *dst, const int32_t *src) { if(e == cudaSuccess) e = cudaMemcpy(dst, src, L1 * sizeof(int32_t), cudaMemcpyHostToDevice); };
	up(b.minscByLen, prm->minsc_by_len); up(b.nceilByLen, prm->nceil_by_len); up(b.nceilRawByLen, prm->nceil_raw_by_len);
	up(b.ivalByLen, prm->interval_by_len); up(b.rdgapsByLen, prm->rdgaps_by_len); up(b.rfgapsByLen, prm->rfgaps_by_len);
	if(e == cudaSuccess) e = cudaMemset(b.alns, 0, nprobMax * prm->max_alns * sizeof(bt2g_dp_aln));
	if(e == cudaSuccess) e = cudaMemset(b.cands, 0, nprobMax * prm->max_cands * sizeof(bt2g_dp_cand));
	if(e == cudaSuccess) e = cudaHostAlloc((void **)&p->hSeq, maxBases, cudaHostAllocDefault);
	if(e == cudaSuccess) e = cudaHostAlloc((void **)&p->hQual, maxBases, cudaHostAllocDefault);
	if(e == cudaSuccess) e = cudaHostAlloc((void **)&p->hOff, (n + 1) * 8, cudaHostAllocDefault);
	if(e == cudaSuccess) e = cudaHostAlloc((void **)&p->hRes, n * sizeof(bt2g_read_result), cudaHostAllocDefault);
	if(e == cudaSuccess) e = cudaHostAlloc((void **)&p->hOps, n * (uint64_t)prm->max_ops, cudaHostAllocDefault);
	if(e != cudaSuccess) { ctx->err = std::string("pipeline setup: ") + cudaGetErrorString(e); bt2g_pipeline_destroy(p); return -2; }
	p->evOk = true;
	for(int i = 0; i < 9; i++) if(cudaEventCreate(&p->ev[i]) != cudaSuccess) p->evOk = false;
	p->chunkOk = cudaStreamCreateWithFlags(&p->sIn, cudaStreamNonBlocking) == cudaSuccess &&
	             cudaStreamCreateWithFlags(&p->sOut, cudaStreamNonBlocking) == cudaSuccess;
	for(int i = 0; i < 8 && p->chunkOk; i++)
		p->chunkOk = cudaEventCreateWithFlags(&p->evIn[i], cudaEventDisableTiming) == cudaSuccess &&
		             cudaEventCreateWithFlags(&p->evDone[i], cudaEventDisableTiming) == cudaSuccess;
	p->prm.minsc_by_len = p->prm.nceil_by_len = p->prm.nceil_raw_by_len = p->prm.interval_by_len = p->prm.rdgaps_by_len = p->prm.rfgaps_by_len = nullptr;
	*out = p;
	return 0;
}

void bt2g_pipeline_destroy(bt2g_pipeline *p) {
	if(!p) return;
	cudaSetDevice(p->ctx->device);
	for(void *v : p->allocs) cudaFree(v);
	if(p->evOk) for(int i = 0; i < 9; i++) cudaEventDestroy(p->ev[i]);
	if(p->chunkOk) { for(int i = 0; i < 8; i++) { cudaEventDestroy(p->evIn[i]); cudaEventDestroy(p->evDone[i]); } }
	if(p->sIn) cudaStreamDestroy(p->sIn);
	if(p->sOut) cudaStreamDestroy(p->sOut);
	if(p->hSeq) cudaFreeHost(p->hSeq);
	if(p->hQual) cudaFreeHost(p->hQual);
	if(p->hOff) cudaFreeHost(p->hOff);
	if(p->hRes) cudaFreeHost(p->hRes);
	if(p->hOps) cudaFreeHost(p->hOps);
	if(p->hPairs) cudaFreeHost(p->hPairs);
	if(p->pairsOn) for(int i = 0; i < 4; i++) cudaEventDestroy(p->pev[i]);
	delete p;
}

int bt2g_pipeline_run_dev(bt2g_pipeline *p, const uint8_t *dSeq, const uint8_t *dQual, const uint64_t *dOff,
                          uint64_t nReads, void *stream, int count) {
	if(!p || !dSeq || !dQual || !dOff) return -1;
	if(nReads > p->maxReads) { p->ctx->err = "pipeline: batch larger than max_reads"; return -1; }
	if(nReads == 0) return 0;
	BT2G_CUDA_TRY(p->ctx, cudaSetDevice(p->ctx->device));
	cudaStream_t st = stream ? (cudaStream_t)stream : p->ctx->stream;
	if(p->ctx->info.off_size == 4) return runStages<uint32_t>(p, dSeq, dQual, dOff, nReads, st, count != 0);
	return runStages<uint64_t>(p, dSeq, dQual, dOff, nReads, st, count != 0);
}

int bt2g_pipeline_run_host(bt2g_pipeline *p, const bt2g_reads *reads, bt2g_read_result *res, uint8_t *ops) {
	if(!p || !reads || !reads->qual || !res) return -1;
	bt2g_ctx *ctx = p->ctx;
	const uint64_t n = reads->n_reads;
	if(n > p->maxReads || reads->off[n] > p->maxBases) { ctx->err = "pipeline: batch larger than the pipeline was created for"; return -1; }
	if(n == 0) return 0;
	BT2G_CUDA_TRY(ctx, cudaSetDevice(ctx->device));
	cudaStream_t st = ctx->stream;
	const uint64_t nb = reads->off[n];
	const uint64_t maxOps = (uint64_t)p->prm.max_ops;
	uint64_t chunkMin = 1u << 18;
	if(const char *e = getenv("BT2G_HOST_CHUNK_MIN")) chunkMin = strtoull(e, nullptr, 10);
	const int nChunks = (p->chunkOk && n >= chunkMin && n >= 4) ? 4 : 1;
	if(nChunks == 1) {
		BT2G_CUDA_TRY(ctx, cudaMemcpyAsync(p->b.seq, reads->seq, nb, cudaMemcpyHostToDevice, st));
		BT2G_CUDA_TRY(ctx, cudaMemcpyAsync(p->b.qual, reads->qual, nb, cudaMemcpyHostToDevice, st));
		BT2G_CUDA_TRY(ctx, cudaMemcpyAsync(p->b.roff, reads->off, (n + 1) * 8, cudaMemcpyHostToDevice, st));
		int rc = bt2g_pipeline_run_dev(p, p->b.seq, p->b.qual, p->b.roff, n, st, 0);
		if(rc) return rc;
		BT2G_CUDA_TRY(ctx, cudaMemcpyAsync(res, p->b.res, n * sizeof(bt2g_read_result), cudaMemcpyDeviceToHost, st));
		if(ops) BT2G_CUDA_TRY(ctx, cudaMemcpyAsync(ops, p->b.resOps, n * maxOps, cudaMemcpyDeviceToHost, st));
		BT2G_CUDA_TRY(ctx, cudaStreamSynchronize(st));
		return 0;
	}
	BT2G_CUDA_TRY(ctx, cudaStreamSynchronize(st));
	BT2G_CUDA_TRY(ctx, cudaMemcpyAsync(p->b.roff, reads->off, (n + 1) * 8, cudaMemcpyHostToDevice, p->sIn));
	const uint64_t per = (n + nChunks - 1) / nChunks;
	for(int c = 0; c < nChunks; c++) {
		const uint64_t s0 = c * per, s1 = (s0 + per < n) ? s0 + per : n;
		const uint64_t b0 = reads->off[s0], b1 = reads->off[s1];
		BT2G_CUDA_TRY(ctx, cudaMemcpyAsync(p->b.seq + b0, reads->seq + b0, b1 - b0, cudaMemcpyHostToDevice, p->sIn));
		BT2G_CUDA_TRY(ctx, cudaMemcpyAsync(p->b.qual + b0, reads->qual + b0, b1 - b0, cudaMemcpyHostToDevice, p->sIn));
		BT2G_CUDA_TRY(ctx, cudaEventRecord(p->evIn[c], p->sIn));
	}
	for(int c = 0; c < nChunks; c++) {
		const uint64_t s0 = c * per, s1 = (s0 + per < n) ? s0 + per : n;
		BT2G_CUDA_TRY(ctx, cudaStreamWaitEvent(st, p->evIn[c], 0));
		int rc;
		if(ctx->info.off_size == 4) rc = runStages<uint32_t>(p, p->b.seq, p->b.qual, p->b.roff + s0, s1 - s0, st, false, s0);
		else rc = runStages<uint64_t>(p, p->b.seq, p->b.qual, p->b.roff + s0, s1 - s0, st, false, s0);
		if(rc) return rc;
		BT2G_CUDA_TRY(ctx, cudaEventRecord(p->evDone[c], st));
		BT2G_CUDA_TRY(ctx, cudaStreamWaitEvent(p->sOut, p->evDone[c], 0));
		BT2G_CUDA_TRY(ctx, cudaMemcpyAsync(res + s0, p->b.res + s0, (s1 - s0) * sizeof(bt2g_read_result), cudaMemcpyDeviceToHost, p->sOut));
		if(ops) BT2G_CUDA_TRY(ctx, cudaMemcpyAsync(ops + s0 * maxOps, p->b.resOps + s0 * maxOps, (s1 - s0) * maxOps, cudaMemcpyDeviceToHost, p->sOut));
	}
	BT2G_CUDA_TRY(ctx, cudaStreamSynchronize(p->sOut));
	BT2G_CUDA_TRY(ctx, cudaStreamSynchronize(st));
	p->lastN = n;
	return 0;
}

int bt2g_pipeline_enable_pairs(bt2g_pipeline *p, const bt2g_pe_policy *pol) {
	if(!p || !pol) return -1;
	bt2g_ctx *ctx = p->ctx;
	if(pol->pol < 1 || pol->pol > 4) { ctx->err = "pipeline: bad paired-end policy"; return -1; }
	if(p->sc.local) { ctx->err = "pipeline: paired-end pass is end-to-end only in this build"; return -1; }
	if(p->pairsOn) { p->pe = *pol; return 0; }
	BT2G_CUDA_TRY(ctx, cudaSetDevice(ctx->device));
	PipeBufs &b = p->b;
	const bt2g_pipeline_params &q = p->prm;
	const uint64_t n = p->maxReads;
	uint64_t maxfrag = pol->maxfrag > (uint64_t)q.max_len ? pol->maxfrag : (uint64_t)q.max_len;
	const int maxgap = q.maxhalf > 32 ? q.maxhalf : 32;
	p->mateMaxCol = (int)(maxfrag + q.max_len + 2 * maxgap + 8);
	if(p->mateMaxCol > 8192) { ctx->err = "pipeline: -X too large for the mate-finding workspace"; return -1; }
	p->mateCodeStride = dp_code_stride(p->mateMaxCol, q.max_len, p->packed);
	int rc = 0;
	uint8_t *codes2 = nullptr;
	if(p->packed == 3) {
		p->mateChunk = dp_chunk_problems(p->mateCodeStride, n);
		const uint64_t need = p->mateChunk * p->mateCodeStride, have = p->dpChunk * p->codeStride;
		rc |= pipeAlloc(p, codes2, need > have ? need : have);
	} else {
		rc |= pipeAlloc(p, codes2, p->numSlots * p->mateCodeStride * (p->packed ? 2 : 1));
	}
	rc |= pipeAlloc(p, b.mProbs, n); rc |= pipeAlloc(p, b.nMateProb, 1); rc |= pipeAlloc(p, b.mateOfRead, n);
	rc |= pipeAlloc(p, b.mSumm, n); rc |= pipeAlloc(p, b.mCands, n * q.max_cands);
	rc |= pipeAlloc(p, b.mAlns, n * q.max_alns); rc |= pipeAlloc(p, b.mOps, n * q.max_alns * (uint64_t)q.max_ops);
	rc |= pipeAlloc(p, b.pairs, n / 2 + 1); rc |= pipeAlloc(p, b.mateCells, 1);
	if(rc) return -2;
	b.codes = codes2;
	if(p->packed != 3) p->codeStride = p->mateCodeStride;
	cudaError_t e = cudaMemset(b.mAlns, 0, n * q.max_alns * sizeof(bt2g_dp_aln));
	if(e == cudaSuccess) e = cudaMemset(b.mCands, 0, n * q.max_cands * sizeof(bt2g_dp_cand));
	if(e == cudaSuccess) e = cudaHostAlloc((void **)&p->hPairs, (n / 2 + 1) * sizeof(bt2g_pair_result), cudaHostAllocDefault);
	for(int i = 0; i < 4 && e == cudaSuccess; i++) e = cudaEventCreate(&p->pev[i]);
	if(e != cudaSuccess) { ctx->err = std::string("pipeline pairs setup: ") + cudaGetErrorString(e); return -2; }
	p->pe = *pol; p->pairsOn = true;
	return 0;
}

int bt2g_pipeline_run_paired_dev(bt2g_pipeline *p, const uint8_t *dSeq, const uint8_t *dQual, const uint64_t *dOff,
                                 uint64_t nPairs, void *stream, int count) {
	if(!p || !dSeq || !dQual || !dOff) return -1;
	if(!p->pairsOn) { p->ctx->err = "pipeline: call bt2g_pipeline_enable_pairs first"; return -1; }
	if(2 * nPairs > p->maxReads) { p->ctx->err = "pipeline: batch larger than max_reads"; return -1; }
	if(nPairs == 0) return 0;
// ... 129 lines not shown
```

### bowtie2_b200/csrc/xengine.cu

```cuda
#include <new>
#include <mutex>
#include <map>
#include <cstdio>
#include <cstddef>
#include <chrono>
#include <cstring>
#include <string>
#include <vector>
#include "dp_ungapped_device.cuh"
#include "dp_device.cuh"
#define XE_HD __device__
#include "xengine.cuh"
#include "xengine_shared.h"

template <typename OFF> int launch_dp_e2e(const DevIndex<OFF> &, const bt2g_scoring &, const DpLaunch &, int, cudaStream_t);
template <typename OFF> int launch_dp_local(const DevIndex<OFF> &, const bt2g_scoring &, const DpLaunch &, int, cudaStream_t);
template <typename OFF> void launch_exact_sweep2(const DevIndex<OFF> &, const uint64_t *, uint64_t, int, int, uint8_t *, uint64_t *, const uint64_t *, const uint32_t *, unsigned long long *, int, cudaStream_t, unsigned long long *, int);
void launch_pack_reads(const uint8_t *, const uint64_t *, uint64_t, int, uint64_t *, uint32_t *, cudaStream_t);
template <typename OFF> void launch_one_mm_sel(const DevIndex<OFF> &, const uint8_t *, const uint8_t *, const uint64_t *, uint64_t, const uint32_t *, const int32_t *, const uint8_t *, const bt2g_scoring &, int, bt2g_mm_hit *, int32_t *, cudaStream_t, bool);
template <typename OFF> void launch_seed_search_active(const DevIndex<OFF> &, const uint64_t *, uint64_t, int, int, const int32_t *, const int32_t *, const uint8_t *, uint64_t *, int32_t *, const uint64_t *, const uint32_t *, unsigned long long *, int, cudaStream_t);

extern "C" int bt2g_policy_align(const bt2g_policy_backend *, const bt2g_policy_params *, const bt2g_reads *, const char *const *,
                                 bt2g_read_result *, uint8_t *, uint32_t, bt2g_pair_result *, uint64_t *);

namespace {
using namespace xe;

#define XE_MM_MAXHITS 16
#define XE_TEV 96

struct XQueues {
	uint32_t nDpA, nDpM, nMm, nSeed, nDone, nFallback, nActive, pad1;
	unsigned long long cellsA, cellsM;
};

struct DpOut { bt2g_dp_problem *probs; bt2g_dp_summary *summ; bt2g_dp_cand *cands; bt2g_dp_aln *alns; uint8_t *ops; int maxCands, maxAlns, maxOps; };

struct XDev {
	const uint8_t *seq, *qual; const uint64_t *roff;
	const uint32_t *seeds;
	const uint64_t *packed; const uint32_t *nmask;
	const uint8_t *mine; const uint64_t *ee;
	const bt2g_mm_hit *mmHits; const int32_t *mmCounts;
	uint32_t *mmSel; int32_t *mmMinsc; uint8_t *mmMask;
	const uint64_t *ranges; const int32_t *nseeds; int maxSeeds;
	int32_t *seedInterval, *seedOffset; uint8_t *seedActive;
	DpOut A, M;
	XQueues *q;
	XUnit *units; uint8_t *status; uint64_t nUnits;
	bt2g_read_result *res; uint8_t *resOps; bt2g_pair_result *pairs; uint32_t resMaxOps;
};

template <typename OFF, bool K>
struct DevSvc {
	static constexpr bool kReport = K;
	const DevIndex<OFF> &ix; const bt2g_scoring &sc; const XDev &d;
	__device__ DevSvc(const DevIndex<OFF> &i, const bt2g_scoring &s, const XDev &dd) : ix(i), sc(s), d(dd) {}
	__device__ const uint8_t *codes(int read) const { return d.seq + d.roff[read]; }
	__device__ const uint8_t *quals(int read) const { return d.qual + d.roff[read]; }
	__device__ int rdlen(int read) const { return (int)(d.roff[read + 1] - d.roff[read]); }
	__device__ uint32_t randSeed(int read) const { return d.seeds[read]; }
	__device__ void sweep(int read, int mined[2], uint64_t tb[4]) const {
		mined[0] = d.mine[2 * (size_t)read]; mined[1] = d.mine[2 * (size_t)read + 1];
		for(int j = 0; j < 4; j++) tb[j] = d.ee[4 * (size_t)read + j];
	}
	__device__ int mmMax() const { return XE_MM_MAXHITS; }
	__device__ int mmCount(int slot, int task) const { return d.mmCounts[4 * (size_t)slot + task]; }
	__device__ const bt2g_mm_hit *mmHits(int slot, int task) const { return d.mmHits + (4 * (size_t)slot + task) * XE_MM_MAXHITS; }
	__device__ int nSeeds(int read) const { return d.nseeds[read]; }
	__device__ const uint64_t *seedRange(int read, int strand, int i) const { return d.ranges + (((size_t)read * 2 + strand) * d.maxSeeds + i) * 4; }
	__device__ const DpOut &dq(bool mate) const { return mate ? d.M : d.A; }
	__device__ const bt2g_dp_summary *dpSumm(int slot, bool mate) const { return dq(mate).summ + slot; }
	__device__ const bt2g_dp_cand *dpCands(int slot, bool mate) const { return dq(mate).cands + (size_t)slot * dq(mate).maxCands; }
	__device__ const bt2g_dp_aln *dpAlns(int slot, bool mate) const { return dq(mate).alns + (size_t)slot * dq(mate).maxAlns; }
	__device__ const uint8_t *dpOps(int slot, bool mate, int k) const { const DpOut &o = dq(mate); return o.ops + ((size_t)slot * o.maxAlns + k) * o.maxOps; }
	__device__ int dpMaxAlns() const { return d.A.maxAlns; }
	__device__ bool resolve(uint64_t row, int qlen, bool reject, int64_t &tidx, int64_t &toff, int64_t &tlen) const {
		unsigned nside = 0;
		const uint64_t off = (row & BT2G_ROW_IS_OFFSET) ? (row & ~BT2G_ROW_IS_OFFSET) : get_offset<OFF>(ix, row, nside);
		uint64_t ti, to, tl; bool st;
		const bool ok = joined_to_text<OFF>(ix, (uint64_t)qlen, off, reject, ti, to, tl, st);
		tidx = (int64_t)ti; toff = (int64_t)to; tlen = (int64_t)tl;
		return ok;
	}
	__device__ void extend(int read, bool fw, int rdoff, int seedlen, const uint64_t rng[4], int &nlex, int &nrex) const {
		const int len = rdlen(read);
		uint32_t nl = 0, nr = 0;
		const uint64_t wb = (d.roff[read] >> 5) + (uint64_t)read;
		extend_hit<OFF>(ix, rng, codes(read), len, fw, rdoff, seedlen < len ? seedlen : len, true, true, nl, nr, d.packed + wb, d.nmask + wb);
		nlex = (int)nl; nrex = (int)nr;
	}
	__device__ int ungapped(int read, bool fw, int64_t tidx, int64_t refoff, int64_t tlen, int64_t minsc, bt2g_ungapped_result &r) const {
		bt2g_ungapped_problem p; p.read_idx = (uint32_t)read; p.fw = fw ? 1u : 0u; p.tidx = (uint64_t)tidx; p.refoff = refoff; p.reflen = (uint64_t)tlen;
		p.minsc = (int32_t)minsc; p.ohang = 0;
		ungapped_one<OFF>(ix, sc, codes(read), quals(read), rdlen(read), p, r, nullptr, 0);
		return r.status;
	}
	mutable RefCursor<OFF> refCur;
	__device__ int refChar(int64_t tidx, int64_t off) const { return refCur.get(ix, (uint64_t)tidx, off); }
};

__global__ void k_xe_seeds(const uint8_t *seq, const uint8_t *qual, const uint64_t *roff, uint64_t nReads, const char *names, uint32_t nameStride,
                           int paired, uint32_t seed, uint32_t *out) {
	const uint64_t i = blockIdx.x * (uint64_t)blockDim.x + threadIdx.x;
	if(i >= nReads) return;
	const uint8_t *c = seq + roff[i], *q = qual + roff[i];
	const int len = (int)(roff[i + 1] - roff[i]);
	uint32_t rseed = (seed + 101u) * 59u * 61u * 67u * 71u * 73u * 79u * 83u;
	for(int k = 0; k < len; k++) rseed ^= (uint32_t)c[k] << ((k & 15) << 1);
	for(int k = 0; k < len; k++) rseed ^= (uint32_t)q[k] << ((k & 3) << 3);
	if(names) {
		const char *nm = names + i * (uint64_t)nameStride;
		for(uint32_t k = 0; k < nameStride && nm[k]; k++) { if(nm[k] == '/') break; rseed ^= (uint32_t)(unsigned char)nm[k] << ((k & 3) << 3); }
	} else {
		char buf[24]; int n = 0;
		uint64_t v = paired ? i >> 1 : i;
		char tmp[20]; int t = 0;
		do { tmp[t++] = (char)('0' + v % 10); v /= 10; } while(v);
		buf[n++] = 'r';
		while(t) buf[n++] = tmp[--t];
		for(int k = 0; k < n; k++) rseed ^= (uint32_t)(unsigned char)buf[k] << ((k & 3) << 3);
	}
	out[i] = rseed;
}

__global__ void k_xe_reset(XUnit *units, uint8_t *status, uint64_t nUnits, int paired) {
	const uint64_t i = blockIdx.x * (uint64_t)blockDim.x + threadIdx.x;
	if(i >= nUnits) return;
	x_unit_reset(units[i], (uint32_t)i, paired != 0);
	status[i] = 0;
}

__device__ __forceinline__ uint32_t agg_inc(uint32_t *ctr) {
	const unsigned act = __activemask();
	const unsigned peers = __match_any_sync(act, (unsigned long long)ctr);
	const int lane = threadIdx.x & 31, leader = __ffs(peers) - 1;
	uint32_t base = 0;
	if(lane == leader) base = atomicAdd(ctr, (uint32_t)__popc(peers));
	base = __shfl_sync(peers, base, leader);
	return base + (uint32_t)__popc(peers & ((1u << lane) - 1u));
}

template <typename OFF, int MINB, bool K>
__global__ void __launch_bounds__(128, MINB) k_xe_step(DevIndex<OFF> ix, bt2g_scoring sc, XParams P, XDev d, const uint32_t *activeIn, uint32_t *activeOut,
                                                       uint32_t nAct, int spread) {
	const uint64_t tt = blockIdx.x * (uint64_t)blockDim.x + threadIdx.x;
	const uint64_t t = tt >> spread;
	const bool valid = t < nAct && (tt & ((1u << spread) - 1u)) == 0;
	const uint64_t i = valid ? (activeIn ? activeIn[t] : t) : 0;
	int r = XR_DONE;
	if(valid) {
		XUnit &u = d.units[i];
		DevSvc<OFF, K> svc(ix, sc, d);
		r = x_step(P, u, svc);
		switch(r) {
		case XR_DP: case XR_DP_MATE: {
			const bool mate = r == XR_DP_MATE;
			const uint32_t slot = agg_inc(mate ? &d.q->nDpM : &d.q->nDpA);
			(mate ? d.M : d.A).probs[slot] = u.rqProb;
			u.dpSlot = (int32_t)slot;
			const unsigned long long cells = (unsigned long long)svc.rdlen((int)u.rqProb.read_idx) * (unsigned long long)(u.rqProb.refr - u.rqProb.refl + 1);
			atomicAdd(mate ? &d.q->cellsM : &d.q->cellsA, cells);
			break; }
		case XR_ONE_MM: {
			const uint32_t slot = agg_inc(&d.q->nMm);
			d.mmSel[slot] = (uint32_t)u.rqRead; d.mmMinsc[slot] = u.rqMinsc; d.mmMask[slot] = (uint8_t)((u.rqNofw ? 0 : 1) | (u.rqNorc ? 0 : 2));
			u.dpSlot = (int32_t)slot;
			break; }
		case XR_SEED:
			d.seedActive[u.rqRead] = 1; d.seedInterval[u.rqRead] = u.rqInterval; d.seedOffset[u.rqRead] = u.rqOffset;
			agg_inc(&d.q->nSeed);
			break;
		case XR_DONE: {
			d.status[i] = 1;
			agg_inc(&d.q->nDone);
			if(K) break;
			const uint64_t r0 = u.paired ? 2 * i : i; const int nr = u.paired ? 2 : 1;
			for(int k = 0; k < nr; k++) x_fill_result(u, k, svc.codes((int)(r0 + k)), d.res[r0 + k], d.resOps + (r0 + k) * (uint64_t)d.resMaxOps, d.resMaxOps);
			if(u.paired) { bt2g_pair_result pr; pr.pair_type = u.pairType; pr.kind = u.pairKind; pr.source = 0; pr.score_sum = (int32_t)u.scoreSum; pr.fraglen = u.fraglen; d.pairs[i] = pr; }
			break; }
		default:
			d.status[i] = 2;
			agg_inc(&d.q->nFallback);
			break;
		}
	}
	__syncwarp();
	const bool cont = valid && (r == XR_DP || r == XR_DP_MATE || r == XR_ONE_MM || r == XR_SEED);
	const unsigned m = __ballot_sync(0xffffffffu, cont);
	if(m) {
		const int lane = threadIdx.x & 31, leader = __ffs(m) - 1;
		uint32_t base = 0;
		if(lane == leader) base = atomicAdd(&d.q->nActive, (uint32_t)__popc(m));
		base = __shfl_sync(0xffffffffu, base, leader);
		if(cont) activeOut[base + (uint32_t)__popc(m & ((1u << lane) - 1u))] = (uint32_t)i;
	}
}

__global__ void __launch_bounds__(128) k_xe_report(XParams P, const XUnit *units, const uint8_t *status, uint64_t nUnits, const uint8_t *seq,
                                                   const uint64_t *roff, uint32_t maxPer, bt2g_read_result *res, uint8_t *ops, uint32_t maxOps,
                                                   bt2g_pair_result *pairs, uint32_t *nEntries, uint32_t *truncated) {
	const uint64_t w = (blockIdx.x * (uint64_t)blockDim.x + threadIdx.x) >> 5;
	const int lane = threadIdx.x & 31;
	if(w >= nUnits || status[w] != 1) return;
	const XUnit &u = units[w];
	const int n = x_report_count(u, P), nw = n < (int)maxPer ? n : (int)maxPer;
	if(lane == 0) {
		nEntries[w] = (uint32_t)nw;
		if(n > (int)maxPer && maxPer > 1) atomicOr(truncated, 1u);
	}
	const int per = u.paired ? 2 : 1;
	const uint64_t r0 = w * (uint64_t)per;
	const uint8_t *c0 = seq + roff[r0], *c1 = u.paired ? seq + roff[r0 + 1] : nullptr;
	for(int e = lane; e < (nw > 1 ? nw : 1); e += 32) {
		const uint64_t ent = w * (uint64_t)maxPer + (uint64_t)e;
		x_report_entry(u, P, e, c0, c1, res + ent * per, ops + ent * per * (uint64_t)maxOps, maxOps, u.paired ? pairs + ent : nullptr);
	}
}

struct DpWork {
	DpOut o{}; uint8_t *codes = nullptr; int32_t *lastH = nullptr; uint64_t *rawKeys = nullptr;
	int maxCol = 0, packed = 0, maxRaw = 0; uint64_t codeStride = 0, chunk = 0, numSlots = 0;
};

}

struct bt2g_xengine {
	bt2g_ctx *ctx = nullptr;
	bt2g_policy_params pp{};
	bt2g_scoring sc{};
	XParams P{}; XTables T;
	uint64_t maxUnits = 0, maxReads = 0, maxBases = 0; int maxLen = 0; uint32_t maxOps = 0;
	std::vector<void *> allocs;
	int32_t *dTabs = nullptr;
	XDev d{};
	DpWork A, M;
	uint64_t *packed = nullptr; uint32_t *nmask = nullptr; unsigned long long *nextTask = nullptr;
	uint32_t *active[2] = {nullptr, nullptr};
	uint8_t *dSeq = nullptr, *dQual = nullptr; uint64_t *dOff = nullptr; char *dNames = nullptr; uint32_t nameStrideCap = 0;
	XQueues *hq = nullptr;
	uint8_t *hStatus = nullptr;
	int sms = 148;
	cudaStream_t stream = nullptr;
	cudaStream_t streamHi = nullptr;
	bool ownStreams = false;
	int debug = 0;
	int bigSpread = 0;
	int stepOcc = 4;
	uint64_t stats[8] = {0, 0, 0, 0, 0, 0, 0, 0};
	float stageMs[12] = {0, 0, 0, 0, 0, 0, 0, 0, 0, 0, 0, 0};
	cudaEvent_t tev[2][XE_TEV]; int tevN[2] = {0, 0};
	cudaEvent_t evJoin = nullptr; int dpSideBySide = 1;
	uint64_t launches = 0;
	uint32_t maxPer = 0;
	bt2g_read_result *kRes = nullptr; uint8_t *kOps = nullptr; bt2g_pair_result *kPairs = nullptr; uint32_t *kN = nullptr, *kTrunc = nullptr;
	cudaEvent_t ev[8] = {nullptr, nullptr, nullptr, nullptr, nullptr, nullptr, nullptr, nullptr};
};

namespace {

template <typename T> int xalloc(bt2g_xengine *e, T *&ptr, uint64_t count) {
	void *v = nullptr;
	const cudaError_t err = cudaMalloc(&v, (count ? count : 1) * sizeof(T));
	if(err != cudaSuccess) { e->ctx->err = std::string("xengine cudaMalloc: ") + cudaGetErrorString(err); return -2; }
	e->allocs.push_back(v);
	ptr = (T *)v;
	return 0;
}

int setupDp(bt2g_xengine *e, DpWork &w, int maxCol, uint64_t cap, int maxCands, int maxAlns) {
	const bt2g_scoring &sc = e->sc;
	int64_t mn = 0;
	for(int l = 1; l <= e->maxLen; l++) if(e->T.minsc[l] < mn) mn = e->T.minsc[l];
	w.maxCol = maxCol + 1;
	w.packed = sc.local ? 0 : dp_kernel_mode(sc, mn, e->maxLen, e->ctx->dpModeCap);
	w.codeStride = dp_code_stride(w.maxCol, e->maxLen, w.packed);
	w.numSlots = (uint64_t)e->sms * 24;
	int rc = 0;
	if(w.packed == 3) { w.chunk = dp_chunk_problems(w.codeStride, cap, 3ull << 30); rc |= xalloc(e, w.codes, w.chunk * w.codeStride); }
	else rc |= xalloc(e, w.codes, w.numSlots * w.codeStride * (w.packed ? 2 : 1));
	rc |= xalloc(e, w.lastH, w.numSlots * (uint64_t)w.maxCol);
	w.maxRaw = maxCands * 4 < 1024 ? 1024 : maxCands * 4;
	if(sc.local) rc |= xalloc(e, w.rawKeys, w.numSlots * (uint64_t)w.maxRaw);
	w.o.maxCands = maxCands; w.o.maxAlns = maxAlns; w.o.maxOps = e->maxLen + 80;
	rc |= xalloc(e, w.o.probs, cap); rc |= xalloc(e, w.o.summ, cap); rc |= xalloc(e, w.o.cands, cap * (uint64_t)maxCands);
	rc |= xalloc(e, w.o.alns, cap * (uint64_t)maxAlns); rc |= xalloc(e, w.o.ops, cap * (uint64_t)maxAlns * w.o.maxOps);
	return rc;
}

template <typename OFF>
int launchDp(bt2g_xengine *e, const DpWork &w, uint64_t n, cudaStream_t st) {
	if(n == 0) return 0;
	DpLaunch L;
	L.seq = e->d.seq; L.qual = e->d.qual; L.roff = e->d.roff; L.probs = w.o.probs; L.n = n; L.nDev = nullptr;
	L.numSlots = w.numSlots; L.codes = w.codes; L.lastH = w.lastH; L.rawKeys = w.rawKeys; L.maxRaw = w.rawKeys ? w.maxRaw : 0;
	L.codeStride = w.codeStride; L.maxCol = w.maxCol; L.maxCands = w.o.maxCands; L.maxAlns = w.o.maxAlns; L.maxOps = w.o.maxOps;
	L.chunk = w.chunk; L.packed = w.packed;
	{ const int qi = &w == &e->M ? 1 : 0; e->tevN[qi] = 0; L.tev = e->tev[qi]; L.tevCap = XE_TEV; L.tevN = &e->tevN[qi]; }
	L.summ = w.o.summ; L.cands = w.o.cands; L.alns = w.o.alns; L.ops = w.o.ops;
	const DevIndex<OFF> ix = bt2g_dev_index<OFF>(e->ctx);
	e->launches += (!e->sc.local && w.packed == 3) ? 2 * ((n + w.chunk - 1) / w.chunk) : 1;
	return e->sc.local ? launch_dp_local<OFF>(ix, e->sc, L, e->maxLen, st) : launch_dp_e2e<OFF>(ix, e->sc, L, e->maxLen, st);
}

template <typename OFF>
int runBatch(bt2g_xengine *e, uint64_t nReads, const char *dNames, uint32_t nameStride, cudaStream_t st0) {
	cudaStream_t st = st0;
	bt2g_ctx *ctx = e->ctx;
	const bool paired = e->P.paired != 0;
	const uint64_t nUnits = paired ? nReads / 2 : nReads;
	const DevIndex<OFF> ix = bt2g_dev_index<OFF>(ctx);
	XDev &d = e->d;
	d.nUnits = nUnits;
	d.packed = e->packed; d.nmask = e->nmask;
	const unsigned T = 128;
	auto grid = [&](uint64_t m, unsigned t) { return (unsigned)((m + t - 1) / t); };
	for(int k = 0; k < 8; k++) e->stats[k] = 0;
	for(int k = 0; k < 12; k++) e->stageMs[k] = 0.f;
	e->tevN[0] = e->tevN[1] = 0;
	e->launches = 4;
	cudaEvent_t *ev = e->ev;
	auto lap = [&](int a, int b, int stage) { float ms = 0.f; if(cudaEventElapsedTime(&ms, ev[a], ev[b]) == cudaSuccess) e->stageMs[stage] += ms; };
	cudaEventRecord(ev[7], st);
	k_xe_seeds<<<grid(nReads, T), T, 0, st>>>(d.seq, d.qual, d.roff, nReads, dNames, nameStride, paired ? 1 : 0, e->P.seed, const_cast<uint32_t *>(d.seeds));
	k_xe_reset<<<grid(nUnits, T), T, 0, st>>>(d.units, d.status, nUnits, paired ? 1 : 0);
	launch_pack_reads(d.seq, d.roff, nReads, e->maxLen, e->packed, e->nmask, st);
	launch_exact_sweep2<OFF>(ix, d.roff, nReads, 0, 0, const_cast<uint8_t *>(d.mine), const_cast<uint64_t *>(d.ee), e->packed, e->nmask, e->nextTask, e->sms, st, nullptr,
	                         ix.extText ? 2 : 0 );
	BT2G_CUDA_TRY(ctx, cudaMemsetAsync(d.seedActive, 0, nReads, st));
	BT2G_CUDA_TRY(ctx, cudaGetLastError());
	uint64_t done = 0;
	uint32_t nActive = 0;
	cudaEventRecord(ev[0], st);
	for(uint64_t wave = 0;; wave++) {
		BT2G_CUDA_TRY(ctx, cudaMemsetAsync(d.q, 0, sizeof(XQueues), st));
		{
			const uint32_t nAct = wave == 0 ? (uint32_t)nUnits : nActive;
			const uint32_t *in = wave == 0 ? nullptr : e->active[wave & 1];
			uint32_t *out = e->active[(wave + 1) & 1];
			const int spread = (uint64_t)nAct * 32 <= (uint64_t)e->sms * 2048 * 4 ? 5 : e->bigSpread;
			const uint64_t nThr = (uint64_t)nAct << spread;
			if(e->maxPer) k_xe_step<OFF, 4, true><<<grid(nThr, 128), 128, 0, st>>>(ix, e->sc, e->P, d, in, out, nAct, spread);
			else if(e->stepOcc >= 8) k_xe_step<OFF, 8, false><<<grid(nThr, 128), 128, 0, st>>>(ix, e->sc, e->P, d, in, out, nAct, spread);
			else if(e->stepOcc >= 6) k_xe_step<OFF, 6, false><<<grid(nThr, 128), 128, 0, st>>>(ix, e->sc, e->P, d, in, out, nAct, spread);
			else k_xe_step<OFF, 4, false><<<grid(nThr, 128), 128, 0, st>>>(ix, e->sc, e->P, d, in, out, nAct, spread);
		}
		cudaEventRecord(ev[1], st);
		e->launches++;
		BT2G_CUDA_TRY(ctx, cudaMemcpyAsync(e->hq, d.q, sizeof(XQueues), cudaMemcpyDeviceToHost, st));
		BT2G_CUDA_TRY(ctx, cudaStreamSynchronize(st));
		if(wave == 0) lap(7, 0, 0); else { lap(2, 3, 2); lap(3, 4, 3); lap(4, 5, 4); lap(5, 0, 5); }
		for(int qi = 0; qi < 2; qi++) {
			for(int k = 0; k + 1 < e->tevN[qi]; k++) { float ms = 0.f; if(cudaEventElapsedTime(&ms, e->tev[qi][k], e->tev[qi][k + 1]) == cudaSuccess) e->stageMs[8 + (k & 1)] += ms; }
			e->tevN[qi] = 0;
		}
		lap(0, 1, 1);
		const XQueues q = *e->hq;
		if(e->debug) {
			float ms = 0.f; cudaEventElapsedTime(&ms, ev[0], ev[1]);
			fprintf(stderr, "[xengine] wave %llu: step %.3f ms; done %u fallback %u | dpA %u dpM %u mm %u seed %u\n", (unsigned long long)wave, ms, q.nDone, q.nFallback,
			        q.nDpA, q.nDpM, q.nMm, q.nSeed);
		}
		e->stats[0]++; e->stats[1] += q.nFallback; e->stats[2] += q.nDpA; e->stats[3] += q.nDpM; e->stats[4] += q.cellsA; e->stats[5] += q.cellsM;
		e->stats[6] += q.nMm; e->stats[7] += q.nSeed;
		e->launches += (q.nMm ? 1 : 0) + (q.nSeed ? 1 : 0);
		done += q.nDone + q.nFallback;
		nActive = q.nActive;
		if(done >= nUnits) break;
		if(e->ownStreams) st = (uint64_t)nActive * 32 <= (uint64_t)e->sms * 2048 * 4 ? e->streamHi : e->stream;
		if(q.nDpA + q.nDpM + q.nMm + q.nSeed == 0) { ctx->err = "xengine: units neither finished nor waiting"; return -5; }
		cudaEventRecord(ev[2], st);
		if(q.nMm) launch_one_mm_sel<OFF>(ix, d.seq, d.qual, d.roff, q.nMm, d.mmSel, d.mmMinsc, d.mmMask, e->sc, XE_MM_MAXHITS, const_cast<bt2g_mm_hit *>(d.mmHits), const_cast<int32_t *>(d.mmCounts), st,
		                                      ix.extText != 0);
		cudaEventRecord(ev[3], st);
		if(q.nSeed) {
			launch_seed_search_active<OFF>(ix, d.roff, nReads, e->P.seedLen, d.maxSeeds, d.seedInterval, d.seedOffset, d.seedActive, const_cast<uint64_t *>(d.ranges),
			                               const_cast<int32_t *>(d.nseeds), e->packed, e->nmask, e->nextTask, e->sms, st);
			BT2G_CUDA_TRY(ctx, cudaMemsetAsync(d.seedActive, 0, nReads, st));
		}
		cudaEventRecord(ev[4], st);
		const bool sideBySide = e->ownStreams && e->dpSideBySide && q.nDpA && q.nDpM && (uint64_t)(q.nDpA + q.nDpM) * 16 <= (uint64_t)e->sms * 2048;
		cudaStream_t stM = sideBySide ? (st == e->stream ? e->streamHi : e->stream) : st;
		if(launchDp<OFF>(e, e->A, q.nDpA, st)) { ctx->err = "xengine: DP launch rejected"; return -1; }
		cudaEventRecord(ev[5], st);
		if(launchDp<OFF>(e, e->M, q.nDpM, stM)) { ctx->err = "xengine: DP launch rejected"; return -1; }
		if(sideBySide) { cudaEventRecord(e->evJoin, stM); cudaStreamWaitEvent(st, e->evJoin, 0); }
		cudaEventRecord(ev[0], st);
		BT2G_CUDA_TRY(ctx, cudaGetLastError());
	}
	lap(7, 1, 7);
	return 0;
}

}

static int createEngine(bt2g_ctx *ctx, const bt2g_policy_params *pp, uint64_t maxUnits, uint32_t maxLen, uint32_t maxPer, bt2g_xengine **out) {
	BT2G_CUDA_TRY(ctx, cudaSetDevice(ctx->device));
	if(maxPer) {
		const uint64_t per = pp->paired ? 2 : 1, ents = maxUnits * (uint64_t)maxPer;
		const uint64_t need = ents * per * (sizeof(bt2g_read_result) + maxLen + 80) + (pp->paired ? ents * sizeof(bt2g_pair_result) : 0) + maxUnits * 4;
		size_t freeB = 0, totalB = 0;
		BT2G_CUDA_TRY(ctx, cudaMemGetInfo(&freeB, &totalB));
		if(need > freeB) {
			char msg[200];
			snprintf(msg, sizeof msg, "xengine: the -k / -a report arrays (%.2f GiB for %llu units x %u entries) do not fit the device's free memory (%.2f GiB)",
			         need / 1073741824.0, (unsigned long long)maxUnits, maxPer, freeB / 1073741824.0);
			ctx->err = msg;
			return -2;
		}
	}
	bt2g_xengine *e = new(std::nothrow) bt2g_xengine();
	if(!e) return -4;
	e->ctx = ctx; e->pp = *pp; e->maxLen = (int)maxLen; e->maxUnits = maxUnits;
	e->maxReads = pp->paired ? 2 * maxUnits : maxUnits; e->maxBases = e->maxReads * (uint64_t)maxLen;
	e->maxOps = maxLen + 80;
	cudaDeviceGetAttribute(&e->sms, cudaDevAttrMultiProcessorCount, ctx->device);
	if(const char *o = getenv("BT2G_XE_OCC")) e->stepOcc = atoi(o);
	if(getenv("BT2G_XE_DEBUG")) e->debug = 1;
	if(const char *o = getenv("BT2G_XE_DP_SERIAL")) e->dpSideBySide = atoi(o) ? 0 : 1;
	if(const char *o = getenv("BT2G_XE_SPREAD")) { e->bigSpread = atoi(o); if(e->bigSpread < 0 || e->bigSpread > 5) e->bigSpread = 0; }
	scoringFromParams(pp, &e->sc);
	ctx->scoring = e->sc;
	buildParams(pp, ctx->info.off_size, (int)maxLen, e->P, e->T);
	int rc = 0;
	const uint64_t nR = e->maxReads, nU = maxUnits;
	rc |= xalloc(e, e->dTabs, 4ull * (maxLen + 1));
	XDev &d = e->d;
	rc |= xalloc(e, e->dSeq, e->maxBases); rc |= xalloc(e, e->dQual, e->maxBases); rc |= xalloc(e, e->dOff, nR + 1);
	uint32_t *seeds; uint8_t *mine; uint64_t *ee;
	rc |= xalloc(e, seeds, nR); rc |= xalloc(e, mine, nR * 2); rc |= xalloc(e, ee, nR * 4);
	d.seeds = seeds; d.mine = mine; d.ee = ee;
	bt2g_mm_hit *mmHits; int32_t *mmCounts;
	rc |= xalloc(e, mmHits, nU * 4 * XE_MM_MAXHITS); rc |= xalloc(e, mmCounts, nU * 4);
	d.mmHits = mmHits; d.mmCounts = mmCounts;
	rc |= xalloc(e, d.mmSel, nU); rc |= xalloc(e, d.mmMinsc, nU); rc |= xalloc(e, d.mmMask, nU);
	{
		int minIval = 1 << 30;
		for(int l = 1; l <= (int)maxLen; l++) { minIval = std::min(minIval, std::min(e->T.ivalOne[l], e->T.ivalBoth[l])); }
		int ms = 1 + ((int)maxLen - std::min<int>(pp->seed_len, (int)maxLen)) / std::max(1, minIval) + 1;
		if(ms > XE_MAX_SEEDS) ms = XE_MAX_SEEDS + 1;
		d.maxSeeds = ms;
	}
	uint64_t *ranges; int32_t *nseeds;
	rc |= xalloc(e, ranges, nR * 2ull * d.maxSeeds * 4); rc |= xalloc(e, nseeds, nR);
	d.ranges = ranges; d.nseeds = nseeds;
	rc |= xalloc(e, d.seedInterval, nR); rc |= xalloc(e, d.seedOffset, nR); rc |= xalloc(e, d.seedActive, nR);
	rc |= xalloc(e, e->packed, (e->maxBases >> 5) + nR + 2); rc |= xalloc(e, e->nmask, (e->maxBases >> 5) + nR + 2); rc |= xalloc(e, e->nextTask, 1);
	rc |= xalloc(e, d.q, 1); rc |= xalloc(e, d.units, nU); rc |= xalloc(e, d.status, nU);
	rc |= xalloc(e, e->active[0], nU); rc |= xalloc(e, e->active[1], nU);
	if(maxPer) {
		const uint64_t ents = nU * (uint64_t)maxPer, rows = ents * (pp->paired ? 2 : 1);
		e->maxPer = maxPer;
		rc |= xalloc(e, e->kRes, rows); rc |= xalloc(e, e->kOps, rows * (uint64_t)e->maxOps); rc |= xalloc(e, e->kN, nU); rc |= xalloc(e, e->kTrunc, 1);
		if(pp->paired) rc |= xalloc(e, e->kPairs, ents);
		d.res = nullptr; d.resOps = nullptr; d.pairs = nullptr;
	} else {
		rc |= xalloc(e, d.res, nR); rc |= xalloc(e, d.resOps, nR * (uint64_t)e->maxOps); rc |= xalloc(e, d.pairs, nU);
	}
	d.resMaxOps = e->maxOps;
	if(!rc) {
		const int maxColA = (int)maxLen + 4 * 15 + 4;
		int gapMax = 15;
		for(int l = 1; l <= (int)maxLen; l++) { gapMax = std::max(gapMax, std::max(e->P.maxReadGaps(e->T.minsc[l], l), e->P.maxRefGaps(e->T.minsc[l], l))); }
		if(gapMax > 512) gapMax = 512;
		const uint64_t maxfrag = std::max<uint64_t>(pp->pe.maxfrag, maxLen);
		int maxColM = (int)std::min<uint64_t>(maxfrag + 2ull * maxLen + 2ull * gapMax + 16, 8000);
		const int maxCands = e->sc.local ? 16384 : 256, maxAlns = e->sc.local ? 32 : 8;
		rc |= setupDp(e, e->A, maxColA, nU, maxCands, maxAlns);
		if(pp->paired) rc |= setupDp(e, e->M, maxColM, nU, maxCands, maxAlns);
		else e->M = e->A;
		d.A = e->A.o; d.M = e->M.o;
	}
	cudaError_t err = cudaSuccess;
	if(!rc) {
		std::vector<int32_t> tabs(4ull * (maxLen + 1));
		for(uint32_t l = 0; l <= maxLen; l++) { tabs[l] = e->T.minsc[l]; tabs[(maxLen + 1) + l] = e->T.nceilRaw[l]; tabs[2 * (maxLen + 1) + l] = e->T.ivalOne[l]; tabs[3 * (maxLen + 1) + l] = e->T.ivalBoth[l]; }
		err = cudaMemcpy(e->dTabs, tabs.data(), tabs.size() * 4, cudaMemcpyHostToDevice);
		e->P.minscTab = e->dTabs; e->P.nceilRawTab = e->dTabs + (maxLen + 1); e->P.ivalOneTab = e->dTabs + 2 * (maxLen + 1); e->P.ivalBothTab = e->dTabs + 3 * (maxLen + 1);
		if(err == cudaSuccess) err = cudaHostAlloc((void **)&e->hq, sizeof(XQueues), cudaHostAllocDefault);
		if(err == cudaSuccess) err = cudaHostAlloc((void **)&e->hStatus, nU, cudaHostAllocDefault);
		for(int k = 0; k < 8 && err == cudaSuccess; k++) err = cudaEventCreate(&e->ev[k]);
		for(int k = 0; k < 2 * XE_TEV && err == cudaSuccess; k++) err = cudaEventCreate(&e->tev[k / XE_TEV][k % XE_TEV]);
		if(err == cudaSuccess) err = cudaEventCreateWithFlags(&e->evJoin, cudaEventDisableTiming);
		if(err == cudaSuccess) err = cudaStreamCreateWithFlags(&e->stream, cudaStreamNonBlocking);
		if(err == cudaSuccess) { int lo = 0, hi = 0; cudaDeviceGetStreamPriorityRange(&lo, &hi); err = cudaStreamCreateWithPriority(&e->streamHi, cudaStreamNonBlocking, hi); }
	}
	if(rc || err != cudaSuccess) {
		if(err != cudaSuccess) ctx->err = std::string("xengine setup: ") + cudaGetErrorString(err);
		bt2g_xengine_destroy(e);
		return -2;
	}
	*out = e;
	return 0;
}

static int checkCreate(bt2g_ctx *ctx, const bt2g_policy_params *pp, uint64_t maxUnits, uint32_t maxLen, bt2g_xengine **out) {
	if(!ctx || !pp || !out || maxUnits == 0 || maxLen == 0) return -1;
	*out = nullptr;
	if(!ctx->loaded) { ctx->err = "no index loaded"; return -1; }
	if(!ctx->info.has_bw || !ctx->info.has_ref) { ctx->err = "xengine: needs the mirror index and the packed reference"; return -1; }
	if(maxLen > XE_MAX_LEN) { ctx->err = "xengine: reads longer than 512 are not supported"; return -1; }
	return 0;
}

extern "C" {

int bt2g_xengine_create(bt2g_ctx *ctx, const bt2g_policy_params *pp, uint64_t maxUnits, uint32_t maxLen, bt2g_xengine **out) {
	if(const int rc = checkCreate(ctx, pp, maxUnits, maxLen, out)) return rc;
	if(pp->all_hits || pp->khits > 1) { ctx->err = "xengine: -k / -a are served by bt2g_policy_align_k"; return -1; }
	return createEngine(ctx, pp, maxUnits, maxLen, 0, out);
}

int bt2g_xengine_create_k(bt2g_ctx *ctx, const bt2g_policy_params *pp, uint64_t maxUnits, uint32_t maxLen, uint32_t maxPerUnit, bt2g_xengine **out) {
	if(const int rc = checkCreate(ctx, pp, maxUnits, maxLen, out)) return rc;
	if(maxPerUnit == 0) { ctx->err = "xengine: max_per_unit must be at least 1"; return -1; }
	return createEngine(ctx, pp, maxUnits, maxLen, maxPerUnit, out);
}

void bt2g_xengine_destroy(bt2g_xengine *e) {
	if(!e) return;
	cudaSetDevice(e->ctx->device);
	for(void *v : e->allocs) cudaFree(v);
	if(e->hq) cudaFreeHost(e->hq);
	if(e->hStatus) cudaFreeHost(e->hStatus);
	for(int k = 0; k < 8; k++) if(e->ev[k]) cudaEventDestroy(e->ev[k]);
	for(int k = 0; k < 2 * XE_TEV; k++) if(e->tev[k / XE_TEV][k % XE_TEV]) cudaEventDestroy(e->tev[k / XE_TEV][k % XE_TEV]);
	if(e->evJoin) cudaEventDestroy(e->evJoin);
	if(e->stream) cudaStreamDestroy(e->stream);
	if(e->streamHi) cudaStreamDestroy(e->streamHi);
	delete e;
}

}

static int finishK(bt2g_xengine *e, cudaStream_t st, bool truncated) {
	bt2g_ctx *ctx = e->ctx;
	uint32_t t = 0;
	BT2G_CUDA_TRY(ctx, cudaMemcpyAsync(&t, e->kTrunc, 4, cudaMemcpyDeviceToHost, st));
	BT2G_CUDA_TRY(ctx, cudaStreamSynchronize(st));
	return truncated || t ? 1 : 0;
}

extern "C" {

int bt2g_xengine_run_dev(bt2g_xengine *e, const uint8_t *dSeq, const uint8_t *dQual, const uint64_t *dOff, uint64_t nReads,
                         const char *dNames, uint32_t nameStride, void *stream, uint64_t *stats) {
	if(!e || !dSeq || !dQual || !dOff) return -1;
	bt2g_ctx *ctx = e->ctx;
	if(nReads > e->maxReads || (e->P.paired && (nReads & 1))) { ctx->err = "xengine: batch larger than the engine was created for"; return -1; }
	if(nReads == 0) return 0;
	BT2G_CUDA_TRY(ctx, cudaSetDevice(ctx->device));
	cudaStream_t st = stream ? (cudaStream_t)stream : e->stream;
	e->ownStreams = stream == nullptr;
	ctx->scoring = e->sc;
	e->d.seq = dSeq; e->d.qual = dQual; e->d.roff = dOff;
	const int rc = ctx->info.off_size == 4 ? runBatch<uint32_t>(e, nReads, dNames, nameStride, st) : runBatch<uint64_t>(e, nReads, dNames, nameStride, st);
	if(rc) return rc;
	bool truncated = false;
	if(e->maxPer) {
		const uint64_t nUnits = e->P.paired ? nReads / 2 : nReads;
		BT2G_CUDA_TRY(ctx, cudaMemsetAsync(e->kTrunc, 0, 4, st));
		k_xe_report<<<(unsigned)((nUnits * 32 + 127) / 128), 128, 0, st>>>(e->P, e->d.units, e->d.status, nUnits, dSeq, dOff, e->maxPer, e->kRes, e->kOps, e->maxOps,
		                                                                   e->kPairs, e->kN, e->kTrunc);
		BT2G_CUDA_TRY(ctx, cudaGetLastError());
		e->launches++;
	}
	if(e->stats[1]) {
		static std::mutex fbMutex;
		std::lock_guard<std::mutex> fbLock(fbMutex);
		const auto tFb = std::chrono::steady_clock::now();
		const bool paired = e->P.paired != 0;
		const uint64_t nUnits = paired ? nReads / 2 : nReads, per = paired ? 2 : 1;
		BT2G_CUDA_TRY(ctx, cudaMemcpyAsync(e->hStatus, e->d.status, nUnits, cudaMemcpyDeviceToHost, st));
		std::vector<uint64_t> off(nReads + 1);
		BT2G_CUDA_TRY(ctx, cudaMemcpyAsync(off.data(), dOff, (nReads + 1) * 8, cudaMemcpyDeviceToHost, st));
		BT2G_CUDA_TRY(ctx, cudaStreamSynchronize(st));
		std::vector<uint64_t> ids;
		for(uint64_t i = 0; i < nUnits; i++) if(e->hStatus[i] == 2) ids.push_back(i);
		if(getenv("BT2G_XE_DEBUG")) {
			std::map<uint32_t, uint64_t> hist;
			for(uint64_t id : ids) { uint32_t ln = 0; cudaMemcpy(&ln, reinterpret_cast<const char *>(e->d.units + id) + offsetof(XUnit, fbLine), 4, cudaMemcpyDeviceToHost); hist[ln]++; }
			fprintf(stderr, "[xengine] %zu fallback units of %llu; by xengine.cuh line:", ids.size(), (unsigned long long)nUnits);
			for(auto &kv : hist) fprintf(stderr, " %u:%llu", kv.first, (unsigned long long)kv.second);
			fprintf(stderr, "\n");
		}
		std::vector<uint8_t> seq, qual; std::vector<uint64_t> soff{0}; std::vector<char> names; std::vector<const char *> nptr;
		for(uint64_t id : ids) for(uint64_t k = 0; k < per; k++) {
			const uint64_t r = id * per + k, a = off[r], b = off[r + 1];
			const size_t o = seq.size();
			seq.resize(o + (b - a)); qual.resize(o + (b - a));
			BT2G_CUDA_TRY(ctx, cudaMemcpy(seq.data() + o, dSeq + a, b - a, cudaMemcpyDeviceToHost));
			BT2G_CUDA_TRY(ctx, cudaMemcpy(qual.data() + o, dQual + a, b - a, cudaMemcpyDeviceToHost));
			soff.push_back(seq.size());
		}
		const uint32_t ns = dNames ? nameStride : 24;
		names.assign(ids.size() * per * (size_t)ns, 0);
		for(size_t j = 0; j < ids.size() * per; j++) {
			const uint64_t r = ids[j / per] * per + (j % per);
			if(dNames) { BT2G_CUDA_TRY(ctx, cudaMemcpy(names.data() + j * ns, dNames + r * (uint64_t)nameStride, nameStride, cudaMemcpyDeviceToHost)); names[j * ns + ns - 1] = 0; }
			else snprintf(names.data() + j * ns, ns, "r%llu", (unsigned long long)(paired ? r >> 1 : r));
		}
		for(size_t j = 0; j < ids.size() * per; j++) nptr.push_back(names.data() + j * ns);
		bt2g_reads sub; sub.n_reads = ids.size() * per; sub.seq = seq.data(); sub.qual = qual.data(); sub.off = soff.data();
		if(e->maxPer) {
			const uint64_t mp = e->maxPer, rowsU = mp * per;
			std::vector<bt2g_read_result> res(ids.size() * rowsU); std::vector<uint8_t> ops(res.size() * (size_t)e->maxOps);
			std::vector<bt2g_pair_result> prs(paired ? ids.size() * mp : 0); std::vector<uint32_t> cnt(ids.size());
			bt2g_policy_backend be; bt2g_policy_backend_gpu(ctx, &be);
			bt2g_policy_params pp = e->pp; pp.host_threads = 8;
			const int rc2 = paired ? bt2g_policy_align_pairs_k(&be, &pp, &sub, nptr.data(), e->maxPer, res.data(), ops.data(), e->maxOps, prs.data(), cnt.data(), nullptr)
			                       : bt2g_policy_align_k(&be, &pp, &sub, nptr.data(), e->maxPer, res.data(), ops.data(), e->maxOps, cnt.data(), nullptr);
			if(rc2 < 0) { ctx->err = "xengine: fallback engine failed"; return rc2; }
			truncated = truncated || rc2 == 1;
			for(size_t j = 0; j < ids.size(); j++) {
				const uint64_t r0 = ids[j] * rowsU;
				BT2G_CUDA_TRY(ctx, cudaMemcpy(e->kRes + r0, res.data() + j * rowsU, rowsU * sizeof(bt2g_read_result), cudaMemcpyHostToDevice));
				BT2G_CUDA_TRY(ctx, cudaMemcpy(e->kOps + r0 * (uint64_t)e->maxOps, ops.data() + j * rowsU * (size_t)e->maxOps, rowsU * (size_t)e->maxOps, cudaMemcpyHostToDevice));
				if(paired) BT2G_CUDA_TRY(ctx, cudaMemcpy(e->kPairs + ids[j] * mp, prs.data() + j * mp, mp * sizeof(bt2g_pair_result), cudaMemcpyHostToDevice));
				BT2G_CUDA_TRY(ctx, cudaMemcpy(e->kN + ids[j], cnt.data() + j, 4, cudaMemcpyHostToDevice));
			}
			e->stageMs[6] = std::chrono::duration<float, std::milli>(std::chrono::steady_clock::now() - tFb).count();
			if(stats) for(int k = 0; k < 8; k++) stats[k] = e->stats[k];
			return finishK(e, st, truncated);
		}
		std::vector<bt2g_read_result> res(sub.n_reads); std::vector<uint8_t> ops(sub.n_reads * (size_t)e->maxOps); std::vector<bt2g_pair_result> prs(ids.size());
		bt2g_policy_backend be; bt2g_policy_backend_gpu(ctx, &be);
		bt2g_policy_params pp = e->pp; pp.host_threads = 8;
		const int rc2 = bt2g_policy_align(&be, &pp, &sub, nptr.data(), res.data(), ops.data(), e->maxOps, paired ? prs.data() : nullptr, nullptr);
		if(rc2 < 0) { ctx->err = "xengine: fallback engine failed"; return rc2; }
		for(size_t j = 0; j < ids.size(); j++) {
			const uint64_t r0 = ids[j] * per;
			BT2G_CUDA_TRY(ctx, cudaMemcpy(e->d.res + r0, res.data() + j * per, per * sizeof(bt2g_read_result), cudaMemcpyHostToDevice));
			BT2G_CUDA_TRY(ctx, cudaMemcpy(e->d.resOps + r0 * (uint64_t)e->maxOps, ops.data() + j * per * (size_t)e->maxOps, per * (size_t)e->maxOps, cudaMemcpyHostToDevice));
			if(paired) BT2G_CUDA_TRY(ctx, cudaMemcpy(e->d.pairs + ids[j], prs.data() + j, sizeof(bt2g_pair_result), cudaMemcpyHostToDevice));
		}
		e->stageMs[6] = std::chrono::duration<float, std::milli>(std::chrono::steady_clock::now() - tFb).count();
	}
	if(stats) for(int k = 0; k < 8; k++) stats[k] = e->stats[k];
	return e->maxPer ? finishK(e, st, truncated) : 0;
}

int bt2g_xengine_streams(bt2g_xengine *e, void **stream, void **stream_hi) {
	if(!e) return -1;
	if(stream) *stream = (void *)e->stream;
	if(stream_hi) *stream_hi = (void *)e->streamHi;
	return 0;
}

int bt2g_xengine_stage_ms(bt2g_xengine *e, float *ms, uint64_t *launches) {
	if(!e || !ms) return -1;
	for(int k = 0; k < 10; k++) ms[k] = e->stageMs[k];
	if(launches) *launches = e->launches;
	return 0;
}

int bt2g_xengine_results_dev(bt2g_xengine *e, bt2g_read_result **res, uint8_t **ops, uint32_t *maxOps, bt2g_pair_result **pairs) {
	if(!e) return -1;
	if(res) *res = e->d.res;
	if(ops) *ops = e->d.resOps;
	if(maxOps) *maxOps = e->maxOps;
	if(pairs) *pairs = e->d.pairs;
	return 0;
}

}

static int runHost(bt2g_xengine *e, const bt2g_reads *reads, const char *names, uint32_t nameStride, uint64_t *stats) {
	bt2g_ctx *ctx = e->ctx;
	const uint64_t n = reads->n_reads;
	if(n > e->maxReads || reads->off[n] > e->maxBases) { ctx->err = "xengine: batch larger than the engine was created for"; return -1; }
	if(n == 0) return 2;
	for(uint64_t i = 0; i < n; i++)
		if(reads->off[i + 1] - reads->off[i] > (uint64_t)e->maxLen) { ctx->err = "xengine: a read is longer than the max_len the engine was created for"; return -1; }
	BT2G_CUDA_TRY(ctx, cudaSetDevice(ctx->device));
	cudaStream_t st = e->stream;
	const uint64_t nb = reads->off[n];
	BT2G_CUDA_TRY(ctx, cudaMemcpyAsync(e->dSeq, reads->seq, nb, cudaMemcpyHostToDevice, st));
	BT2G_CUDA_TRY(ctx, cudaMemcpyAsync(e->dQual, reads->qual, nb, cudaMemcpyHostToDevice, st));
	BT2G_CUDA_TRY(ctx, cudaMemcpyAsync(e->dOff, reads->off, (n + 1) * 8, cudaMemcpyHostToDevice, st));
	char *dn = nullptr;
	if(names) {
		if((uint64_t)nameStride * n > (uint64_t)e->nameStrideCap * e->maxReads || !e->dNames) {
// ... 63 lines not shown
```

Baseline: 2.722.

## Use atomic work-stealing in DP fill/tail kernels and ping-pong chunks across two streams

The DP fill and tail kernels now fetch work per warp from an atomic task counter instead of a static grid-stride assignment. This balances load when problem costs vary. Chunked DP is resized evenly and alternated between two streams with separate code buffers, so one chunk's tail can overlap the next chunk's fill. The cost is extra memsets, an atomic per task, event fork/join, and half the code buffer per stream, which means more chunks.

After: 2.805 (median of 6 runs). 3.0% higher.

```diff
diff --git a/bowtie2_b200/csrc/api.cu b/bowtie2_b200/csrc/api.cu
--- a/bowtie2_b200/csrc/api.cu
+++ b/bowtie2_b200/csrc/api.cu
@@ -665,7 +665,7 @@
 	if(maxLen > 512) { ctx->err = "reads longer than 512 are not supported by the DP kernel"; return -1; }
 	maxCol += 1;
 	if(maxCol > 8192) { ctx->err = "DP window wider than 8192 columns"; return -1; }
-	DBuf dseq, dqual, doff, dprob, dcodes, dlast, dsumm, dcand, daln, dops, draw;
+	DBuf dseq, dqual, doff, dprob, dcodes, dlast, dsumm, dcand, daln, dops, draw, dctr;
 	int rc = uploadReads(ctx, reads, dseq, dqual, doff, true);
 	if(rc) return rc;
 	DpLaunch L;
@@ -681,6 +681,8 @@
 	if(L.packed == 3) {
 		L.chunk = dp_chunk_problems(L.codeStride, n);
 		BT2G_CUDA_TRY(ctx, dcodes.alloc(L.chunk * L.codeStride));
+		BT2G_CUDA_TRY(ctx, dctr.alloc(4 * sizeof(uint32_t)));
+		L.taskCtr = dctr.as<uint32_t>();
 	} else {
 		BT2G_CUDA_TRY(ctx, dcodes.alloc(L.numSlots * L.codeStride * (L.packed ? 2 : 1)));
 	}
diff --git a/bowtie2_b200/csrc/dp_device.cuh b/bowtie2_b200/csrc/dp_device.cuh
--- a/bowtie2_b200/csrc/dp_device.cuh
+++ b/bowtie2_b200/csrc/dp_device.cuh
@@ -37,6 +37,14 @@
 	return c ? c : 1;
 }
 
+static inline uint64_t dp_chunk_size(uint64_t n, uint64_t cap, uint64_t round) {
+	if(cap < 1) cap = 1;
+	const uint64_t k = (n + cap - 1) / cap;
+	uint64_t c = k ? (n + k - 1) / k : cap;
+	if(round) { const uint64_t r = (c + round - 1) / round * round; if(r <= cap) c = r; }
+	return c ? c : 1;
+}
+
 struct DpLaunch {
 	const uint8_t  *seq, *qual;
 	const uint64_t *roff;
@@ -53,6 +61,10 @@
 	int             maxCands, maxAlns, maxOps;
 	uint64_t        chunk = 0;
 	int             packed = 0;
+	uint32_t       *taskCtr = nullptr;
+	cudaStream_t    st2 = nullptr;
+	cudaEvent_t     evFork = nullptr, evJoin = nullptr;
+	uint64_t       *nChunks = nullptr;
 	cudaEvent_t    *tev = nullptr;
 	int             tevCap = 0;
 	int            *tevN = nullptr;
diff --git a/bowtie2_b200/csrc/dp_kernels.cu b/bowtie2_b200/csrc/dp_kernels.cu
--- a/bowtie2_b200/csrc/dp_kernels.cu
+++ b/bowtie2_b200/csrc/dp_kernels.cu
@@ -651,14 +651,19 @@
 
 template <bool B> struct DpBool { static constexpr bool value = B; };
 
+__device__ __forceinline__ uint64_t dp_next_task(uint32_t *next, int lane) {
+	uint32_t t = 0;
+	if(lane == 0) t = atomicAdd(next, 1u);
+	return __shfl_sync(0xffffffffu, t, 0);
+}
+
 template <typename OFF, int R, bool OFFDOM>
-__global__ void __launch_bounds__(128, 8) k_dp_fill_h(DevIndex<OFF> ix, bt2g_scoring sc, DpLaunch L, uint64_t chunkStart, uint64_t chunkMax) {
+__global__ void __launch_bounds__(128, 8) k_dp_fill_h(DevIndex<OFF> ix, bt2g_scoring sc, DpLaunch L, uint64_t chunkStart, uint64_t chunkMax,
+                                                      uint32_t *next) {
 	constexpr int RPL = DP_BLOCK_RPL;
 	static_assert(RPL == 1 || RPL == 2, "stores are one byte or one u16 per lane and problem");
 	extern __shared__ uint8_t smem[];
 	const int warpInBlock = threadIdx.x >> 5, lane = threadIdx.x & 31;
-	const uint64_t slot = blockIdx.x * (uint64_t)(blockDim.x >> 5) + warpInBlock;
-	const uint64_t nSlots = (uint64_t)gridDim.x * (blockDim.x >> 5);
 	const uint64_t nAll = L.nDev ? (uint64_t)*L.nDev : L.n;
 	if(chunkStart >= nAll) return;
 	const uint64_t nProb = (nAll - chunkStart < chunkMax) ? nAll - chunkStart : chunkMax;
@@ -675,7 +680,7 @@
 	const uint32_t FLOORP = OFFDOM ? L.zeroP : dpx_both(DPX_FLOOR);
 	const uint32_t nrdeP = dpx_both(-rdgape);
 
-	for(uint64_t pw = slot; pw < nPairs; pw += nSlots) {
+	for(uint64_t pw = dp_next_task(next, lane); pw < nPairs; pw = dp_next_task(next, lane)) {
 		uint64_t w[2] = {2 * pw, 2 * pw + 1};
 		bool live[2] = {true, w[1] < nProb};
 		if(!live[1]) w[1] = w[0];
@@ -860,7 +865,8 @@
 #define DP_TAIL_SMEM_PER_WARP(maxCol, R) (dp_smem_per_warp(maxCol) + DP_PROF_BYTES(R) + DP_BLK_MAX * sizeof(uint2))
 
 template <typename OFF, int R>
-__global__ void __launch_bounds__(256) k_dp_tail_h(DevIndex<OFF> ix, bt2g_scoring sc, DpLaunch L, uint64_t chunkStart, uint64_t chunkMax) {
+__global__ void __launch_bounds__(256) k_dp_tail_h(DevIndex<OFF> ix, bt2g_scoring sc, DpLaunch L, uint64_t chunkStart, uint64_t chunkMax,
+                                                   uint32_t *next) {
 	extern __shared__ uint8_t smem[];
 	const int warpInBlock = threadIdx.x >> 5, lane = threadIdx.x & 31;
 	const uint64_t nAll = L.nDev ? (uint64_t)*L.nDev : L.n;
@@ -873,8 +879,7 @@
 	uint8_t *prof = smem + (size_t)warpInBlock * perWarp + dp_smem_per_warp(L.maxCol);
 	uint2 *tab = reinterpret_cast<uint2 *>(prof + DP_PROF_BYTES(R));
 	const int bonus = sc.match_bonus;
-	const uint64_t nWarps = (uint64_t)gridDim.x * (blockDim.x >> 5);
-	for(uint64_t wl = blockIdx.x * (uint64_t)(blockDim.x >> 5) + warpInBlock; wl < nProb; wl += nWarps) {
+	for(uint64_t wl = dp_next_task(next, lane); wl < nProb; wl = dp_next_task(next, lane)) {
 		const uint64_t w = chunkStart + wl;
 		const bt2g_dp_problem p = L.probs[w];
 		const uint8_t *rs = L.seq + L.roff[p.read_idx], *rq = L.qual + L.roff[p.read_idx];
@@ -1138,9 +1143,10 @@
 }
 
 template <typename OFF, int R>
-static void launch_dp_e2e_r(const DevIndex<OFF> &ix, const bt2g_scoring &sc, const DpLaunch &L, cudaStream_t st) {
+static int launch_dp_e2e_r(const DevIndex<OFF> &ix, const bt2g_scoring &sc, const DpLaunch &L, cudaStream_t st) {
 	const int warpsPerBlock = 4;
 	if(L.packed == 3) {
+		if(!L.taskCtr) return -1;
 		int dev = 0, sms = 148; cudaGetDevice(&dev); cudaDeviceGetAttribute(&sms, cudaDevAttrMultiProcessorCount, dev);
 		const size_t smF = (size_t)warpsPerBlock * dp_fill_smem_per_warp(L.maxCol, sc.match_bonus == 0);
 		const size_t smT = (size_t)8 * DP_TAIL_SMEM_PER_WARP(L.maxCol, R);
@@ -1150,14 +1156,29 @@
 		int nbF = 1, nbT = 1;
 		if(cudaOccupancyMaxActiveBlocksPerMultiprocessor(&nbF, kfill, warpsPerBlock * 32, smF) != cudaSuccess || nbF < 1) nbF = 1;
 		if(cudaOccupancyMaxActiveBlocksPerMultiprocessor(&nbT, k_dp_tail_h<OFF, R>, 256, smT) != cudaSuccess || nbT < 1) nbT = 1;
-		auto mark = [&]() { if(L.tev && L.tevN && *L.tevN < L.tevCap) cudaEventRecord(L.tev[(*L.tevN)++], st); };
-		mark();
-		for(uint64_t c0 = 0; c0 < L.n; c0 += L.chunk) {
-			kfill<<<(unsigned)(nbF * sms), warpsPerBlock * 32, smF, st>>>(ix, sc, L, c0, L.chunk);
-			mark();
-			k_dp_tail_h<OFF, R><<<(unsigned)(nbT * sms), 256, smT, st>>>(ix, sc, L, c0, L.chunk);
-			mark();
-		}
+		const int halves = (L.st2 && L.chunk >= 2) ? 2 : 1;
+		const uint64_t cap = L.chunk / halves;
+		const uint64_t c = dp_chunk_size(L.n, cap, 2ull * warpsPerBlock * nbF * sms);
+		cudaStream_t ss[2] = {st, L.st2};
+		if(halves == 2) { cudaEventRecord(L.evFork, st); cudaStreamWaitEvent(L.st2, L.evFork, 0); }
+		auto mark = [&](cudaStream_t s, int k) { cudaEventRecord(L.tev[*L.tevN + k], s); };
+		uint64_t k = 0;
+		for(uint64_t c0 = 0; c0 < L.n; c0 += c, k++) {
+			const int h = (int)(k % halves);
+			cudaStream_t s = ss[h];
+			DpLaunch Lc = L;
+			Lc.codes = L.codes + (uint64_t)h * cap * L.codeStride;
+			uint32_t *ctr = L.taskCtr + 2 * h;
+			cudaMemsetAsync(ctr, 0, 2 * sizeof(uint32_t), s);
+			const bool timed = L.tev && L.tevN && *L.tevN + 3 <= L.tevCap;
+			if(timed) mark(s, 0);
+			kfill<<<(unsigned)(nbF * sms), warpsPerBlock * 32, smF, s>>>(ix, sc, Lc, c0, c, ctr);
+			if(timed) mark(s, 1);
+			k_dp_tail_h<OFF, R><<<(unsigned)(nbT * sms), 256, smT, s>>>(ix, sc, Lc, c0, c, ctr + 1);
+			if(timed) { mark(s, 2); *L.tevN += 3; }
+		}
+		if(halves == 2 && k > 1) { cudaEventRecord(L.evJoin, L.st2); cudaStreamWaitEvent(st, L.evJoin, 0); }
+		if(L.nChunks) *L.nChunks = k;
 	} else if(L.packed == 2) {
 		const size_t smem = (size_t)warpsPerBlock * 2 * dp_smem_per_warp(L.maxCol);
 		if(smem > 48 * 1024) cudaFuncSetAttribute(k_dp_e2e_h<OFF, R>, cudaFuncAttributeMaxDynamicSharedMemorySize, (int)smem);
@@ -1174,22 +1195,22 @@
 		const unsigned grid = dp_resident_grid(k_dp_e2e<OFF, R>, warpsPerBlock * 32, smem, L.numSlots, warpsPerBlock);
 		k_dp_e2e<OFF, R><<<grid, warpsPerBlock * 32, smem, st>>>(ix, sc, L);
 	}
+	return 0;
 }
 
 template <typename OFF>
 int launch_dp_e2e(const DevIndex<OFF> &ix, const bt2g_scoring &sc, const DpLaunch &L, int maxRdLen, cudaStream_t st) {
 	if(L.n == 0) return 0;
 	switch(dp_rows_per_lane(maxRdLen, L.packed)) {
-		case 4: launch_dp_e2e_r<OFF, 4>(ix, sc, L, st); break;
-		case 5: launch_dp_e2e_r<OFF, 5>(ix, sc, L, st); break;
-		case 6: launch_dp_e2e_r<OFF, 6>(ix, sc, L, st); break;
-		case 8: launch_dp_e2e_r<OFF, 8>(ix, sc, L, st); break;
-		case 10: launch_dp_e2e_r<OFF, 10>(ix, sc, L, st); break;
-		case 12: launch_dp_e2e_r<OFF, 12>(ix, sc, L, st); break;
-		case 16: launch_dp_e2e_r<OFF, 16>(ix, sc, L, st); break;
+		case 4: return launch_dp_e2e_r<OFF, 4>(ix, sc, L, st);
+		case 5: return launch_dp_e2e_r<OFF, 5>(ix, sc, L, st);
+		case 6: return launch_dp_e2e_r<OFF, 6>(ix, sc, L, st);
+		case 8: return launch_dp_e2e_r<OFF, 8>(ix, sc, L, st);
+		case 10: return launch_dp_e2e_r<OFF, 10>(ix, sc, L, st);
+		case 12: return launch_dp_e2e_r<OFF, 12>(ix, sc, L, st);
+		case 16: return launch_dp_e2e_r<OFF, 16>(ix, sc, L, st);
 		default: return -1;
 	}
-	return 0;
 }
 template int launch_dp_e2e<uint32_t>(const DevIndex<uint32_t> &, const bt2g_scoring &, const DpLaunch &, int, cudaStream_t);
 template int launch_dp_e2e<uint64_t>(const DevIndex<uint64_t> &, const bt2g_scoring &, const DpLaunch &, int, cudaStream_t);
diff --git a/bowtie2_b200/csrc/pipeline.cu b/bowtie2_b200/csrc/pipeline.cu
--- a/bowtie2_b200/csrc/pipeline.cu
+++ b/bowtie2_b200/csrc/pipeline.cu
@@ -26,7 +26,7 @@
 	uint32_t *nRows, *rowBase, *rowCnt;
 	uint64_t *tidx, *textoff, *tlen; uint8_t *rflags;
 	bt2g_dp_problem *probs; uint32_t *nProb; int32_t *readProb; int32_t *readNProb;
-	uint8_t *codes; int32_t *lastH; uint64_t *rawKeys;
+	uint8_t *codes; int32_t *lastH; uint64_t *rawKeys; uint32_t *dpTasks;
 	bt2g_dp_summary *summ; bt2g_dp_cand *cands; bt2g_dp_aln *alns; uint8_t *ops;
 	bt2g_read_result *res; uint8_t *resOps;
 	unsigned long long *counters;
@@ -396,7 +396,7 @@
 	L.seq = seq; L.qual = qual; L.roff = roff; L.probs = b.probs; L.n = p->maxProbs; L.nDev = b.nProb;
 	L.rawKeys = b.rawKeys; L.maxRaw = b.rawKeys ? PIPE_MAX_RAW : 0;
 	L.numSlots = p->numSlots; L.codes = b.codes; L.lastH = b.lastH; L.codeStride = p->codeStride; L.maxCol = p->maxCol;
-	L.maxCands = q.max_cands; L.maxAlns = q.max_alns; L.maxOps = q.max_ops; L.packed = p->packed; L.chunk = p->dpChunk;
+	L.maxCands = q.max_cands; L.maxAlns = q.max_alns; L.maxOps = q.max_ops; L.packed = p->packed; L.chunk = p->dpChunk; L.taskCtr = b.dpTasks;
 	L.summ = b.summ; L.cands = b.cands; L.alns = b.alns; L.ops = b.ops;
 	mark(6);
 	const int drc = p->sc.local ? launch_dp_local<OFF>(ix, p->sc, L, q.max_len, st) : launch_dp_e2e<OFF>(ix, p->sc, L, q.max_len, st);
@@ -431,7 +431,7 @@
 	L.seq = seq; L.qual = qual; L.roff = roff; L.probs = b.mProbs; L.n = p->maxReads; L.nDev = b.nMateProb;
 	L.rawKeys = nullptr; L.maxRaw = 0;
 	L.numSlots = p->numSlots; L.codes = b.codes; L.lastH = nullptr; L.codeStride = p->mateCodeStride; L.maxCol = p->mateMaxCol;
-	L.maxCands = q.max_cands; L.maxAlns = q.max_alns; L.maxOps = q.max_ops; L.packed = p->packed; L.chunk = p->mateChunk;
+	L.maxCands = q.max_cands; L.maxAlns = q.max_alns; L.maxOps = q.max_ops; L.packed = p->packed; L.chunk = p->mateChunk; L.taskCtr = b.dpTasks;
 	L.summ = b.mSumm; L.cands = b.mCands; L.alns = b.mAlns; L.ops = b.mOps;
 	if(launch_dp_e2e<OFF>(ix, p->sc, L, q.max_len, st)) { ctx->err = "pipeline: mate DP launch rejected"; return -1; }
 	cudaEventRecord(p->pev[2], st);
@@ -495,7 +495,7 @@
 	rc |= pipeAlloc(p, b.summ, nprobMax); rc |= pipeAlloc(p, b.cands, nprobMax * prm->max_cands);
 	rc |= pipeAlloc(p, b.alns, nprobMax * prm->max_alns); rc |= pipeAlloc(p, b.ops, nprobMax * prm->max_alns * (uint64_t)prm->max_ops);
 	rc |= pipeAlloc(p, b.res, n); rc |= pipeAlloc(p, b.resOps, n * (uint64_t)prm->max_ops);
-	rc |= pipeAlloc(p, b.counters, 4);
+	rc |= pipeAlloc(p, b.counters, 4); rc |= pipeAlloc(p, b.dpTasks, 4);
 	rc |= pipeAlloc(p, b.probTlen, nprobMax); rc |= pipeAlloc(p, b.resTlen, n);
 	if(rc) { bt2g_pipeline_destroy(p); return -2; }
 	cudaError_t e = cudaSuccess;
diff --git a/bowtie2_b200/csrc/xengine.cu b/bowtie2_b200/csrc/xengine.cu
--- a/bowtie2_b200/csrc/xengine.cu
+++ b/bowtie2_b200/csrc/xengine.cu
@@ -27,7 +27,7 @@
 using namespace xe;
 
 #define XE_MM_MAXHITS 16
-#define XE_TEV 96
+#define XE_TEV 192
 
 struct XQueues {
 	uint32_t nDpA, nDpM, nMm, nSeed, nDone, nFallback, nActive, pad1;
@@ -219,7 +219,7 @@
 }
 
 struct DpWork {
-	DpOut o{}; uint8_t *codes = nullptr; int32_t *lastH = nullptr; uint64_t *rawKeys = nullptr;
+	DpOut o{}; uint8_t *codes = nullptr; int32_t *lastH = nullptr; uint64_t *rawKeys = nullptr; uint32_t *tasks = nullptr;
 	int maxCol = 0, packed = 0, maxRaw = 0; uint64_t codeStride = 0, chunk = 0, numSlots = 0;
 };
 
@@ -251,6 +251,8 @@
 	float stageMs[12] = {0, 0, 0, 0, 0, 0, 0, 0, 0, 0, 0, 0};
 	cudaEvent_t tev[2][XE_TEV]; int tevN[2] = {0, 0};
 	cudaEvent_t evJoin = nullptr; int dpSideBySide = 1;
+	cudaEvent_t evFork = nullptr;
+	cudaStream_t streamDp = nullptr;
 	uint64_t launches = 0;
 	uint32_t maxPer = 0;
 	bt2g_read_result *kRes = nullptr; uint8_t *kOps = nullptr; bt2g_pair_result *kPairs = nullptr; uint32_t *kN = nullptr, *kTrunc = nullptr;
@@ -277,7 +279,10 @@
 	w.codeStride = dp_code_stride(w.maxCol, e->maxLen, w.packed);
 	w.numSlots = (uint64_t)e->sms * 24;
 	int rc = 0;
-	if(w.packed == 3) { w.chunk = dp_chunk_problems(w.codeStride, cap, 3ull << 30); rc |= xalloc(e, w.codes, w.chunk * w.codeStride); }
+	if(w.packed == 3) {
+		w.chunk = dp_chunk_problems(w.codeStride, cap, 3ull << 30);
+		rc |= xalloc(e, w.codes, w.chunk * w.codeStride); rc |= xalloc(e, w.tasks, 4);
+	}
 	else rc |= xalloc(e, w.codes, w.numSlots * w.codeStride * (w.packed ? 2 : 1));
 	rc |= xalloc(e, w.lastH, w.numSlots * (uint64_t)w.maxCol);
 	w.maxRaw = maxCands * 4 < 1024 ? 1024 : maxCands * 4;
@@ -289,18 +294,21 @@
 }
 
 template <typename OFF>
-int launchDp(bt2g_xengine *e, const DpWork &w, uint64_t n, cudaStream_t st) {
+int launchDp(bt2g_xengine *e, const DpWork &w, uint64_t n, cudaStream_t st, cudaStream_t st2) {
 	if(n == 0) return 0;
 	DpLaunch L;
 	L.seq = e->d.seq; L.qual = e->d.qual; L.roff = e->d.roff; L.probs = w.o.probs; L.n = n; L.nDev = nullptr;
 	L.numSlots = w.numSlots; L.codes = w.codes; L.lastH = w.lastH; L.rawKeys = w.rawKeys; L.maxRaw = w.rawKeys ? w.maxRaw : 0;
 	L.codeStride = w.codeStride; L.maxCol = w.maxCol; L.maxCands = w.o.maxCands; L.maxAlns = w.o.maxAlns; L.maxOps = w.o.maxOps;
-	L.chunk = w.chunk; L.packed = w.packed;
+	L.chunk = w.chunk; L.packed = w.packed; L.taskCtr = w.tasks;
+	L.st2 = st2; L.evFork = e->evFork; L.evJoin = e->evJoin;
+	uint64_t chunks = 0; L.nChunks = &chunks;
 	{ const int qi = &w == &e->M ? 1 : 0; e->tevN[qi] = 0; L.tev = e->tev[qi]; L.tevCap = XE_TEV; L.tevN = &e->tevN[qi]; }
 	L.summ = w.o.summ; L.cands = w.o.cands; L.alns = w.o.alns; L.ops = w.o.ops;
 	const DevIndex<OFF> ix = bt2g_dev_index<OFF>(e->ctx);
-	e->launches += (!e->sc.local && w.packed == 3) ? 2 * ((n + w.chunk - 1) / w.chunk) : 1;
-	return e->sc.local ? launch_dp_local<OFF>(ix, e->sc, L, e->maxLen, st) : launch_dp_e2e<OFF>(ix, e->sc, L, e->maxLen, st);
+	const int rc = e->sc.local ? launch_dp_local<OFF>(ix, e->sc, L, e->maxLen, st) : launch_dp_e2e<OFF>(ix, e->sc, L, e->maxLen, st);
+	e->launches += (!e->sc.local && w.packed == 3) ? 2 * chunks : 1;
+	return rc;
 }
 
 template <typename OFF>
@@ -351,7 +359,10 @@
 		BT2G_CUDA_TRY(ctx, cudaStreamSynchronize(st));
 		if(wave == 0) lap(7, 0, 0); else { lap(2, 3, 2); lap(3, 4, 3); lap(4, 5, 4); lap(5, 0, 5); }
 		for(int qi = 0; qi < 2; qi++) {
-			for(int k = 0; k + 1 < e->tevN[qi]; k++) { float ms = 0.f; if(cudaEventElapsedTime(&ms, e->tev[qi][k], e->tev[qi][k + 1]) == cudaSuccess) e->stageMs[8 + (k & 1)] += ms; }
+			for(int k = 0; k + 1 < e->tevN[qi]; k++) {
+				if(k % 3 == 2) continue;
+				float ms = 0.f; if(cudaEventElapsedTime(&ms, e->tev[qi][k], e->tev[qi][k + 1]) == cudaSuccess) e->stageMs[8 + k % 3] += ms;
+			}
 			e->tevN[qi] = 0;
 		}
 		lap(0, 1, 1);
@@ -381,9 +392,10 @@
 		cudaEventRecord(ev[4], st);
 		const bool sideBySide = e->ownStreams && e->dpSideBySide && q.nDpA && q.nDpM && (uint64_t)(q.nDpA + q.nDpM) * 16 <= (uint64_t)e->sms * 2048;
 		cudaStream_t stM = sideBySide ? (st == e->stream ? e->streamHi : e->stream) : st;
-		if(launchDp<OFF>(e, e->A, q.nDpA, st)) { ctx->err = "xengine: DP launch rejected"; return -1; }
+		cudaStream_t st2 = (e->ownStreams && !sideBySide) ? (st == e->stream ? e->streamDp : e->stream) : nullptr;
+		if(launchDp<OFF>(e, e->A, q.nDpA, st, st2)) { ctx->err = "xengine: DP launch rejected"; return -1; }
 		cudaEventRecord(ev[5], st);
-		if(launchDp<OFF>(e, e->M, q.nDpM, stM)) { ctx->err = "xengine: DP launch rejected"; return -1; }
+		if(launchDp<OFF>(e, e->M, q.nDpM, stM, st2)) { ctx->err = "xengine: DP launch rejected"; return -1; }
 		if(sideBySide) { cudaEventRecord(e->evJoin, stM); cudaStreamWaitEvent(st, e->evJoin, 0); }
 		cudaEventRecord(ev[0], st);
 		BT2G_CUDA_TRY(ctx, cudaGetLastError());
@@ -482,8 +494,10 @@
 		for(int k = 0; k < 8 && err == cudaSuccess; k++) err = cudaEventCreate(&e->ev[k]);
 		for(int k = 0; k < 2 * XE_TEV && err == cudaSuccess; k++) err = cudaEventCreate(&e->tev[k / XE_TEV][k % XE_TEV]);
 		if(err == cudaSuccess) err = cudaEventCreateWithFlags(&e->evJoin, cudaEventDisableTiming);
+		if(err == cudaSuccess) err = cudaEventCreateWithFlags(&e->evFork, cudaEventDisableTiming);
 		if(err == cudaSuccess) err = cudaStreamCreateWithFlags(&e->stream, cudaStreamNonBlocking);
 		if(err == cudaSuccess) { int lo = 0, hi = 0; cudaDeviceGetStreamPriorityRange(&lo, &hi); err = cudaStreamCreateWithPriority(&e->streamHi, cudaStreamNonBlocking, hi); }
+		if(err == cudaSuccess) err = cudaStreamCreateWithFlags(&e->streamDp, cudaStreamNonBlocking);
 	}
 	if(rc || err != cudaSuccess) {
 		if(err != cudaSuccess) ctx->err = std::string("xengine setup: ") + cudaGetErrorString(err);
@@ -526,8 +540,10 @@
 	for(int k = 0; k < 8; k++) if(e->ev[k]) cudaEventDestroy(e->ev[k]);
 	for(int k = 0; k < 2 * XE_TEV; k++) if(e->tev[k / XE_TEV][k % XE_TEV]) cudaEventDestroy(e->tev[k / XE_TEV][k % XE_TEV]);
 	if(e->evJoin) cudaEventDestroy(e->evJoin);
+	if(e->evFork) cudaEventDestroy(e->evFork);
 	if(e->stream) cudaStreamDestroy(e->stream);
 	if(e->streamHi) cudaStreamDestroy(e->streamHi);
+	if(e->streamDp) cudaStreamDestroy(e->streamDp);
 	delete e;
 }
 
```
